# mims-harvard/G-Meta

Hardware: AMD Instinct MI355X
Metric: meta-tasks/sec (inner-loop fwd+bwd) at task_num=32 (higher is better)
Workload: dtype f32

## Files before the change

g-meta_amd/_lib.py:

```python
import ctypes as C
import os

HERE = os.path.dirname(os.path.abspath(__file__))
LIB_PATH = os.environ.get('GMETA_HIP_LIB') or os.path.join(HERE, 'libgmeta_hip.so')

GM_MAX_GCN = 4
(F_SUB_OFF, F_SET_SUB_OFF, F_PARENT, F_GRAPH, F_INDPTR, F_INDICES, F_INDPTR_T, F_INDICES_T, F_CENTRE, F_NORM,
 F_FEAT_ROW, F_NORM_SRC, F_NORM_CENTRE, F_EDGE_W, F_EDGE_W_T, F_HOP, F_NORM_E1, F_EDGE_CENTRE_T, F_OBS_CENTRE, F_OBS_E1) = range(20)
LINK_SYMMETRIC = 2
LINK_MASK_TARGET = 4
NEG_MODES = {'uniform': 0, 'two_hop': 1}
PAIR_MASK_TARGET = 1
PROP_SELF_LOOPS = 1
PROP_OPS = {'hadamard': 0, 'abs_diff': 1}
DIST_UNREACHED = 255


class Seed(C.Structure):
    _fields_ = [('graph', C.c_int32), ('i', C.c_int32), ('j', C.c_int32)]


class Model(C.Structure):
    _fields_ = [('n_gcn', C.c_int32), ('dims', C.c_int32 * (GM_MAX_GCN + 1)), ('n_out', C.c_int32), ('link_pred', C.c_int32)]

# ... 12 lines not shown
    'gm_store_weighted': (i32, [vp]),
    'gm_batch_weighted': (i32, [vp]),
    'gm_store_destroy': (None, [vp]),
    'gm_store_negative_pairs': (i32, [vp, i32, i64, u64, i32, vp, i64, vp, vp, vp]),
    'gm_store_has_edges': (i32, [vp, i32, vp, i64, vp, vp]),
    'gm_store_pair_scores': (i32, [vp, i32, vp, i64, i32, vp, vp]),
    'gm_store_pair_walks': (i32, [vp, i32, vp, i64, i32, vp, vp]),
    'gm_store_rooted_pagerank': (i32, [vp, i32, vp, i64, C.c_float, i32, vp, vp]),
    'gm_store_pair_pagerank': (i32, [vp, i32, vp, i64, i32, C.c_float, i32, vp, vp]),
    'gm_store_pagerank_candidates': (i32, [vp, i32, vp, i64, i32, C.c_float, i32, vp, vp, vp, vp]),
    'gm_store_node_distances': (i32, [vp, i32, vp, i64, i32, vp, vp]),
    'gm_store_pair_distance': (i32, [vp, i32, vp, i64, i32, i32, vp, vp]),
    'gm_store_pair_distance_profile': (i32, [vp, i32, vp, i64, i32, i32, vp, vp]),
    'gm_store_sketch_build': (i32, [vp, i32, i32, i32, i32, u64, vp, vp]),
    'gm_sketch_dims': (i32, [vp, vp, vp, vp, vp, vp]),
    'gm_sketch_registers': (i32, [vp, i32, vp, i64, vp, vp, vp]),
    'gm_sketch_pair_counts': (i32, [vp, vp, i64, vp, vp, vp]),
    'gm_sketch_destroy': (None, [vp]),
    'gm_store_propagate_build': (i32, [vp, i32, i32, i32, vp, vp]),
    'gm_prop_dims': (i32, [vp, vp, vp, vp, vp, vp]),
    'gm_prop_rows': (i32, [vp, i32, vp, i64, vp, vp]),
    'gm_prop_pair_features': (i32, [vp, vp, i64, i32, vp, vp]),
    'gm_prop_destroy': (None, [vp]),
    'gm_store_neighbour_degrees': (i32, [vp, i32, vp, vp]),
    'gm_store_pair_candidates': (i32, [vp, i32, vp, i64, i32, i32, vp, vp, vp, vp]),
    'gm_extract': (C.c_int, [vp, vp, i32, vp, i32, i32, i32, u64, i32, vp, vp]),
    'gm_extract_pair': (C.c_int, [vp, vp, i32, vp, i32, vp, i32, vp, i32, i32, i32, u64, i32, vp, vp, vp]),
    'gm_batch_from_nodes': (C.c_int, [vp, vp, i32, vp, i32, vp, vp, i32, vp, vp]),
    'gm_set_hop_labels': (None, [i32]),
    'gm_get_hop_labels': (i32, []),
    'gm_batch_hop_labels': (i32, [vp]),
    'gm_batch_mask_target': (i32, [vp]),
    'gm_batch_concat': (C.c_int, [vp, i32, vp, vp]),
    'gm_batch_destroy': (None, [vp]),
    'gm_batch_prepare_cone': (C.c_int, [vp, i32, vp]),
    'gm_batch_prepare_cone_pair': (C.c_int, [vp, vp, i32, vp]),
    'gm_batch_cone_dims': (C.c_int, [vp, i32, vp, vp, vp]),
    'gm_batch_cone_read': (C.c_int, [vp, i32, i32, i32, vp, i64]),
    'gm_batch_dims': (C.c_int, [vp, vp, vp, vp, vp, vp]),
    'gm_batch_read': (C.c_int, [vp, i32, vp, i64]),
    'gm_batch_device_ptr': (C.c_int, [vp, i32, vp]),
    'gm_batch_source_rows': (C.c_int, [vp, vp]),
    'gm_batch_e1_source_rows': (C.c_int, [vp, vp]),
    'gm_gather_features': (C.c_int, [vp, vp, vp]),
    'gm_aggregate': (C.c_int, [vp, i32, i32, vp, i32, vp, vp, vp, vp]),
    'gm_aggregate_bytes': (i64, [vp, i32]),
    'gm_model_param_count': (i64, [vp]),
    'gm_gcn_ws_bytes': (i64, [vp, vp]),
    'gm_gcn_forward': (C.c_int, [vp, vp, vp, i64, vp, vp, vp, vp, i64, vp]),
    'gm_gcn_backward': (C.c_int, [vp, vp, vp, i64, vp, vp, vp, vp, i64, vp, i64, vp]),
    'gm_dense_update': (C.c_int, [vp, vp, i32, vp, i64, i32, vp, i32, vp]),
    'gm_dense_gemm': (C.c_int, [vp, vp, i64, i32, vp, i64, i32, i32, vp, i64, vp, vp, vp, i64, i32, vp, vp, vp, vp, vp, i32, vp, vp]),
    'gm_dense_fused_gemm': (C.c_int, [vp, i32, vp, i64, i32, vp, i64, vp, i64, vp, i64, i32, vp, i64, vp, vp, vp, i64, i32, vp, vp, vp, i32, vp, vp]),
    'gm_dense_wgrad_fused': (C.c_int, [vp, i32, vp, i64, i32, vp, i64, vp, i64, i32, vp, vp, vp, i64, vp, i64, i32, vp]),
    'gm_dense_aggregate': (C.c_int, [vp, i32, i32, vp, i64, i32, i32, vp, vp, i32, vp, i64, i32, vp, vp, vp, i32, vp, i64, i32, i32, i32, i32, i32, vp, vp, vp]),
    'gm_dense_agg_info': (C.c_int, [vp, i32, vp]),
    'gm_dense_obs_lists': (C.c_int, [vp, vp, vp]),
    'gm_dense_fuse_counts': (C.c_int, [vp, vp]),
    'gm_dense_agg_table': (C.c_int, [vp, i32, i32, vp, i64, vp]),
    'gm_dense_dz_centre': (C.c_int, [vp, vp, i32, vp, i64, i32, vp, vp]),
    'gm_dense_wgrad_centre': (C.c_int, [vp, vp, i32, vp, i32, vp, i64, vp, i64, vp]),
    'gm_dense_agg_centre_t': (C.c_int, [vp, vp, i32, vp, vp, i32, vp]),
    'gm_dense_wgrad_e1': (C.c_int, [vp, vp, i32, vp, i32, vp, i64, vp, i64, vp]),
    'gm_dense_wgrad': (C.c_int, [vp, vp, i64, i32, vp, i64, i32, vp, vp, i64, vp, i64, vp, i64, i32, vp, vp, i64, C.c_float, vp, vp, vp, vp]),
    'gm_proto_loss_spt': (C.c_int, [vp, vp, i32, vp, i32, vp, vp, vp, vp, vp]),
    'gm_proto_loss_qry': (C.c_int, [vp, vp, i32, vp, vp, i32, vp, vp, vp, vp, vp]),
    'gm_dense_head_loss': (C.c_int, [vp, vp, i32, i32, i32, i32, vp, i64, i64, i64, vp, vp, i32, i32, vp, i32, vp, vp, vp, vp, vp, vp, vp, vp, i32, vp, i64, vp, vp,
                                     vp, vp, i64, C.c_float, vp, i32, vp, vp]),
    'gm_set_ragged_classes': (None, [i32]),
    'gm_get_ragged_classes': (i32, []),
    'gm_set_readout': (None, [i32]),
    'gm_get_readout': (i32, []),
    'gm_meta_ws_bytes': (i64, [vp, vp, vp, vp]),
    'gm_meta_out_floats': (i64, [vp, vp, vp]),
    'gm_meta_step': (C.c_int, [vp, vp, vp, vp, vp, vp, vp, vp, i64, vp, i64, vp]),
    'gm_adapt_ws_bytes': (i64, [vp, vp, vp]),
    'gm_meta_adapt': (C.c_int, [vp, vp, vp, vp, vp, vp, i64, vp, i32, vp, i64, vp]),
    'gm_predict_ws_bytes': (i64, [vp, vp, vp]),
    'gm_proto_predict': (C.c_int, [vp, vp, vp, vp, i64, vp, vp, i32, vp, vp, vp, vp, i64, vp]),
    'gm_meta_finish': (C.c_int, [vp, i64, i32, vp, vp, vp]),
    'gm_meta_finish_adam': (C.c_int, [vp, i64, i32, vp, vp, vp, vp, vp, i32, C.c_float, C.c_float, C.c_float, C.c_float, vp, vp, vp]),
    'gm_set_gemm_mode': (None, [i32]),
    'gm_get_gemm_mode': (i32, []),
    'gm_get_split_pieces': (i32, []),
    'gm_set_split_pieces': (None, [i32]),
    'gm_set_tuning': (C.c_int, [C.c_char_p, i32]),
    'gm_get_tuning': (i32, [C.c_char_p]),
    'gm_tuning_epoch': (i32, []),
    'gm_set_fuse_agg': (None, [i32]),
    'gm_get_fuse_agg': (i32, []),
    'gm_profile_enable': (None, [i32]),
    'gm_profile_aggregate': (C.c_int, [vp, vp, vp]),
    'gm_profile_read': (C.c_int, [i32, vp, vp, vp]),
    'gm_profile_read_launches': (C.c_int, [i32, vp, vp, i32]),
}
PROBE_PROTOTYPES = {
    'gm_debug_stamp': (C.c_int, [vp, vp]),
    'gm_stream_debug': (C.c_int, [i32, vp, i32]),
    'gm_head_loss_debug': (C.c_int, [i32, vp]),
}

LATER_EXPORTS = {'gm_dense_obs_lists'}

_lib = None


def lib():
    global _lib
    if _lib is None:
        if not os.path.exists(LIB_PATH):
            raise RuntimeError('gmeta_amd: %s is missing -- run `python -c "import __graft_entry__ as g; g.build()"` '
                               '(hipcc --offload-arch=gfx950).  There is no CPU fallback.' % LIB_PATH)
        l = C.CDLL(LIB_PATH)
        for name, (res, args) in PROTOTYPES.items():
            if name in LATER_EXPORTS and os.environ.get('GMETA_HIP_LIB') and not hasattr(l, name):
                continue
            fn = getattr(l, name)
            fn.restype, fn.argtypes = res, args
        for name, (res, args) in PROBE_PROTOTYPES.items():
            if hasattr(l, name):
                fn = getattr(l, name)
                fn.restype, fn.argtypes = res, args
        _lib = l
    return _lib


def check(rc, what=''):
    if rc != 0:
        msg = lib().gm_last_error().decode('utf-8', 'replace')
        exc = ValueError if rc == -1 else RuntimeError
        raise exc('%s failed (code %d): %s' % (what or 'libgmeta_hip', rc, msg))


def require_gpu():
    import torch
    if not torch.cuda.is_available():
        raise RuntimeError('gmeta_amd needs an AMD GPU (gfx950); torch.cuda.is_available() is False and there is no CPU fallback')


def stream_ptr():
    import torch
    return C.c_void_p(torch.cuda.current_stream().cuda_stream)


def ptr(t):
    if t is None:
        return C.c_void_p(0)
    if hasattr(t, 'data_ptr'):
        return C.c_void_p(t.data_ptr())
    return C.c_void_p(t.ctypes.data)


READOUT_CENTRE, READOUT_MEAN = 0, 1
READOUTS = {'centre': READOUT_CENTRE, 'mean': READOUT_MEAN}

# ... 56 lines not shown
```

g-meta_amd/csrc/common.hip:

```cpp
#include <stdarg.h>
#include <stdlib.h>
#include <atomic>
#include <chrono>
#include <map>
#include <mutex>
#include <set>
#include <utility>
#include "gm_internal.h"

static thread_local char g_err[512] = "";

void gm_set_error(const char* fmt, ...) {
    va_list ap;
    va_start(ap, fmt);
    vsnprintf(g_err, sizeof(g_err), fmt, ap);
    va_end(ap);
}

extern "C" const char* gm_last_error(void) { return g_err; }
extern "C" int gm_version(void) { return 100; }

static void pool_keep_memory() {
    static thread_local int done_for = -1;
    int dev = 0;
// ... 261 lines not shown
    if (total_ms) *total_ms = tot;
    if (launches) *launches = c.launches;
    if (work) *work = c.work;
    return GM_OK;
}
extern "C" int gm_profile_read_launches(int32_t category, double* ms, int64_t* work, int32_t cap) {
    GM_REQUIRE(category >= 0 && category < GM_PROF_CATS && ms && work && cap >= 0, GM_EINVAL, "profile_read_launches: bad arguments");
    ProfCat& c = g_prof[category];
    int n = 0;
    for (size_t k = 0; k + 1 < c.used + 1 && k < c.used && n < cap; k += 2, ++n) {
        GM_HIP(hipEventSynchronize(c.ev[k + 1]));
        float t = 0;
        GM_HIP(hipEventElapsedTime(&t, c.ev[k], c.ev[k + 1]));
        ms[n] = t; work[n] = k / 2 < c.works.size() ? c.works[k / 2] : 0;
    }
    return n;
}
extern "C" int gm_profile_aggregate(double* total_ms, int64_t* launches, int64_t* algorithmic_bytes) {
    return gm_profile_read(GM_PROF_AGG, total_ms, launches, algorithmic_bytes);
}

#ifdef GM_PROBES
__global__ void k_debug_stamp(unsigned long long* out) { *out = wall_clock64(); }
extern "C" int gm_debug_stamp(void* out, void* stream) {
    GM_REQUIRE(out, GM_EINVAL, "debug_stamp: NULL argument");
    hipLaunchKernelGGL(k_debug_stamp, dim3(1), dim3(1), 0, (hipStream_t)stream, (unsigned long long*)out);
    GM_HIP(hipGetLastError());
    return GM_OK;
}
#endif

static gm_knobs g_knobs;
static std::once_flag g_knobs_once;
const gm_knobs& gm_knob() {
    gm_knobs& k = g_knobs;
    std::call_once(g_knobs_once, [] {
        gm_knobs& k = g_knobs;
        auto env = [](const char* name, int dflt) { const char* e = getenv(name); return e ? atoi(e) : dflt; };
        k.timing = env("GM_TIMING", 0);
        const char* gm = getenv("GM_GEMM_MODE");
        k.gemm_mode = (gm && (!strcmp(gm, "split") || !strcmp(gm, "1"))) ? 1 : (gm && (!strcmp(gm, "f32") || !strcmp(gm, "0"))) ? 0 : -1;
        k.gemm_split_min_tiles = env("GM_GEMM_SPLIT_MIN_TILES", -1);
        k.centre_store = env("GM_CENTRE_STORE", 2);
        k.dead_rows = env("GM_DEAD_ROWS", 4);
        k.fuse_agg = env("GM_FUSE_AGG", 1);
        k.fuse_diff = env("GM_FUSE_DIFF", 2);
        k.extract_pref16 = env("GM_EXTRACT_PREF16", 1);
        k.head_stage = env("GM_HEAD_STAGE", 1);
        k.head_threads = env("GM_HEAD_THREADS", 0);
        k.query_streams = env("GM_QUERY_STREAMS", 0);
        k.agg_mid_list = env("GM_AGG_MID_LIST", 1);
        k.agg_mid_win = env("GM_AGG_MID_WIN", 0);
        k.agg_obs_list = env("GM_AGG_OBS_LIST", 1);
        k.split_pieces = env("GM_SPLIT_PIECES", 3);
        k.split16_min_rows = env("GM_SPLIT16_MIN_ROWS", 65536);
        k.wgrad_split_min_chunks = env("GM_WGRAD_SPLIT_MIN_CHUNKS", -1);
        k.agg_stream = env("GM_AGG_STREAM", 1);
        k.agg_stream_min_rows = env("GM_AGG_STREAM_MIN_ROWS", 100000);
        k.neg_round = env("GM_NEG_ROUND", 0);
        k.pair_lanes = env("GM_PAIR_LANES", 0);
        k.cand_round = env("GM_CAND_ROUND", 0);
        k.cand_bitmap = env("GM_CAND_BITMAP", 0);
        k.walk_chunk = env("GM_WALK_CHUNK", 0);
        k.walk_lanes = env("GM_WALK_LANES", 0);
        k.ppr_chunk = env("GM_PPR_CHUNK", 0);
        k.ppr_cols = env("GM_PPR_COLS", 0);
        k.dist_chunk = env("GM_DIST_CHUNK", 0);
        k.dist_cols = env("GM_DIST_COLS", 0);
        k.dist_plane_kib = env("GM_DIST_PLANE_KIB", 0);
        k.sketch_chunk = env("GM_SKETCH_CHUNK", 0);
        k.sketch_mib = env("GM_SKETCH_MIB", 0);
        k.prop_chunk = env("GM_PROP_CHUNK", 0);
        k.prop_mib = env("GM_PROP_MIB", 0);
    });
    return k;
}

static std::atomic<int> g_tuning_epoch{0};
extern "C" int32_t gm_tuning_epoch(void) { return g_tuning_epoch.load(std::memory_order_relaxed); }
static int gm_knobs::* gm_find_knob(const char* name) {
    (void)gm_knob();
    static const struct { const char* name; int gm_knobs::*field; } tab[] = {
        {"GM_GEMM_SPLIT_MIN_TILES", &gm_knobs::gemm_split_min_tiles}, {"GM_CENTRE_STORE", &gm_knobs::centre_store}, {"GM_DEAD_ROWS", &gm_knobs::dead_rows},
        {"GM_HEAD_STAGE", &gm_knobs::head_stage}, {"GM_HEAD_THREADS", &gm_knobs::head_threads}, {"GM_QUERY_STREAMS", &gm_knobs::query_streams}, {"GM_AGG_MID_LIST", &gm_knobs::agg_mid_list}, {"GM_AGG_MID_WIN", &gm_knobs::agg_mid_win}, {"GM_AGG_OBS_LIST", &gm_knobs::agg_obs_list}, {"GM_AGG_STREAM", &gm_knobs::agg_stream}, {"GM_AGG_STREAM_MIN_ROWS", &gm_knobs::agg_stream_min_rows},
        {"GM_SPLIT16_MIN_ROWS", &gm_knobs::split16_min_rows}, {"GM_WGRAD_SPLIT_MIN_CHUNKS", &gm_knobs::wgrad_split_min_chunks}, {"GM_TIMING", &gm_knobs::timing},
        {"GM_FUSE_DIFF", &gm_knobs::fuse_diff}, {"GM_EXTRACT_PREF16", &gm_knobs::extract_pref16},
        {"neg_round", &gm_knobs::neg_round}, {"GM_NEG_ROUND", &gm_knobs::neg_round},
        {"pair_lanes", &gm_knobs::pair_lanes}, {"GM_PAIR_LANES", &gm_knobs::pair_lanes},
        {"cand_round", &gm_knobs::cand_round}, {"GM_CAND_ROUND", &gm_knobs::cand_round},
        {"cand_bitmap", &gm_knobs::cand_bitmap}, {"GM_CAND_BITMAP", &gm_knobs::cand_bitmap},
        {"walk_chunk", &gm_knobs::walk_chunk}, {"GM_WALK_CHUNK", &gm_knobs::walk_chunk},
        {"walk_lanes", &gm_knobs::walk_lanes}, {"GM_WALK_LANES", &gm_knobs::walk_lanes},
        {"ppr_chunk", &gm_knobs::ppr_chunk}, {"GM_PPR_CHUNK", &gm_knobs::ppr_chunk},
        {"ppr_cols", &gm_knobs::ppr_cols}, {"GM_PPR_COLS", &gm_knobs::ppr_cols},
        {"dist_chunk", &gm_knobs::dist_chunk}, {"GM_DIST_CHUNK", &gm_knobs::dist_chunk},
        {"dist_cols", &gm_knobs::dist_cols}, {"GM_DIST_COLS", &gm_knobs::dist_cols},
        {"dist_plane_kib", &gm_knobs::dist_plane_kib}, {"GM_DIST_PLANE_KIB", &gm_knobs::dist_plane_kib},
        {"sketch_chunk", &gm_knobs::sketch_chunk}, {"GM_SKETCH_CHUNK", &gm_knobs::sketch_chunk},
        {"sketch_mib", &gm_knobs::sketch_mib}, {"GM_SKETCH_MIB", &gm_knobs::sketch_mib},
        {"prop_chunk", &gm_knobs::prop_chunk}, {"GM_PROP_CHUNK", &gm_knobs::prop_chunk},
        {"prop_mib", &gm_knobs::prop_mib}, {"GM_PROP_MIB", &gm_knobs::prop_mib},
    };
    for (const auto& e : tab)
        if (!strcmp(name, e.name)) return e.field;
    return nullptr;
}
extern "C" int gm_set_tuning(const char* name, int32_t value) {
    GM_REQUIRE(name, GM_EINVAL, "set_tuning: NULL name");
    int gm_knobs::* f = gm_find_knob(name);
    GM_REQUIRE(f, GM_EINVAL, "set_tuning: unknown or start-up-only knob %s", name);
    g_knobs.*f = value; g_tuning_epoch.fetch_add(1, std::memory_order_relaxed);
    return GM_OK;
}
extern "C" int32_t gm_get_tuning(const char* name) {
    int gm_knobs::* f = name ? gm_find_knob(name) : nullptr;
    return f ? g_knobs.*f : 0;
}

int gm_heavy_deg() { return 64; }
int gm_heavy_deg_for(int64_t rows, int64_t edges) {
    return edges <= 8 * rows ? 32 : 64;
}

static std::mutex g_dev_mu;

int gm_num_cus() {
    static std::map<int, int> cus;
    int dev = 0;
    if (hipGetDevice(&dev) != hipSuccess) { (void)hipGetLastError(); return 256; }
    std::lock_guard<std::mutex> lk(g_dev_mu);
    auto it = cus.find(dev);
    if (it != cus.end()) return it->second;
    int n = 0;
    if (hipDeviceGetAttribute(&n, hipDeviceAttributeMultiprocessorCount, dev) != hipSuccess || n <= 0) { (void)hipGetLastError(); n = 256; }
    cus[dev] = n;
    return n;
}
// ... 12 lines not shown
```

g-meta_amd/csrc/dense_exports.hip:

```cpp
#include <algorithm>
#include "gm_internal.h"

static int set_row_amax(const gm_batch* b, const float* x, int64_t ldx, int cols, unsigned* slots, hipStream_t st) {
    int rc = GM_OK;
    for (int t0 = 0; rc == GM_OK && t0 < b->sets; t0 += 8) {
        const int segs = std::min(8, b->sets - t0);
        int64_t xo[8], xn[8];
        for (int i = 0; i < segs; ++i) {
            const int64_t r0 = b->h_set_row_off[t0 + i], nr = b->h_set_row_off[t0 + i + 1] - r0;
            xo[i] = r0 * ldx; xn[i] = nr > 0 ? (nr - 1) * ldx + cols : 0;
        }
        rc = gm_amax_segs(x, xo, xn, segs, slots + (int64_t)t0 * GM_BOUND_PAD, GM_BOUND_PAD, st);
    }
    return rc;
}

extern "C" int gm_dense_update(const gm_batch_t* b, const float* x, int32_t K, const float* W, int64_t w_stride, int32_t N, float* out, int32_t mode,
                               void* stream) {
    GM_REQUIRE(b && x && W && out && K >= 1 && N >= 1, GM_EINVAL, "dense_update: bad arguments");
    hipStream_t st = (hipStream_t)stream;
    gm_gemm_args g{};
    g.A = x; g.lda = K; g.B = W; g.b_stride = w_stride; g.C = out; g.ldc = N; g.K = K; g.N = N;
    g.tiles = b->d_tiles; g.n_tiles = b->n_tiles; g.rows = b->rows;
    uint16_t* planes = nullptr; unsigned* slots = nullptr;
// ... 13 lines not shown
            g.np = 2; g.a_bound = gm_no_bound(); g.a_bound.amax = slots; g.b_bound = wb;
        }
        if (rc == GM_OK) rc = gm_split_weights(W, w_stride, 0, K, N, 0, sets, planes, st, mode == 2 ? 2 : 3, wb);
        if (rc != GM_OK) { gm_dev_free(planes, st); if (slots) gm_dev_free(slots, st); return rc; }
        g.Bsplit = planes; g.bsplit_stride = w_stride ? (int64_t)3 * K * N : 0;
    }
    const int rc = gm_launch_gemm_nn(g, st);
    if (planes) gm_dev_free(planes, st);
    if (slots) gm_dev_free(slots, st);
    gm_batch_mark_use(b, st);
    return rc;
}

extern "C" int gm_dense_gemm(const gm_batch_t* b, const float* x, int64_t ldx, int32_t K, const float* W, int64_t w_stride, int32_t trans_w, int32_t N,
                             float* out, int64_t ldc, const float* s, const float* s_keep, const float* bias, int64_t bias_stride, int32_t relu,
                             uint8_t* relu_bits, const float* mask_h, const uint8_t* mask_b, float* zero_out, uint32_t* amax_out, int32_t mode,
                             int32_t* launched, void* stream) {
    GM_REQUIRE(b && x && W && out && K >= 1 && N >= 1 && ldx >= K && ldc >= N && mode >= -1 && mode <= 2 && !(mask_h && mask_b), GM_EINVAL,
               "dense_gemm: bad arguments");
    GM_REQUIRE(!amax_out || mode == 2, GM_EINVAL, "dense_gemm: amax_out is an output of the two-piece kernels (mode 2)");
    hipStream_t st = (hipStream_t)stream;
    const int sets = b->sets;
    gm_gemm_args g{};
    g.A = x; g.lda = ldx; g.B = W; g.b_stride = w_stride; g.transB = trans_w ? 1 : 0; g.C = out; g.ldc = ldc; g.K = K; g.N = N;
    g.row_scale = s; g.row_scale_keep = s_keep; g.n_keep = b->rows; g.bias = bias; g.bias_stride = bias_stride; g.relu = relu ? 1 : 0;
    g.relu_bits = relu_bits; g.mask_h = mask_h; g.mask_b = mask_b; g.zero_out = zero_out;
    g.tiles = b->d_tiles; g.n_tiles = b->n_tiles; g.rows = b->rows; g.launched = launched;
    uint16_t* planes = nullptr; unsigned* slots = nullptr;
    int rc = GM_OK;
    if (mode == 1 || mode == 2 || (mode < 0 && gm_gemm_split_ok(b->n_tiles, K, N))) {
        GM_REQUIRE(!mask_h && !mask_b, GM_EINVAL, "dense_gemm: the split kernels take no relu' mask");
        GM_REQUIRE((N == 256 || N == 128) && K % 16 == 0 && K >= 32, GM_EINVAL, "dense_gemm: the split kernels need N = 128 or 256 and K a multiple of 16 (>= 32)");
        const int wsets = w_stride ? sets : 1;
        rc = gm_alloc(&planes, (size_t)wsets * 3 * K * N, st);
        gm_bound wb = gm_no_bound();
        if (rc == GM_OK && mode == 2) {
            rc = gm_alloc(&slots, (size_t)(sets + wsets) * GM_BOUND_PAD, st);
            if (rc == GM_OK && hipMemsetAsync(slots, 0, sizeof(unsigned) * (sets + wsets) * GM_BOUND_PAD, st) != hipSuccess) { gm_set_error("dense_gemm: memset failed"); rc = GM_EHIP; }
            if (rc == GM_OK) rc = set_row_amax(b, x, ldx, K, slots, st);
            if (rc == GM_OK) rc = gm_amax(W, w_stride, 0, (int64_t)K * N, wsets, slots + (int64_t)sets * GM_BOUND_PAD, GM_BOUND_PAD, st);
            wb.amax = slots + (int64_t)sets * GM_BOUND_PAD; wb.stride = w_stride ? GM_BOUND_PAD : 0;
            g.np = 2; g.a_bound = gm_no_bound(); g.a_bound.amax = slots; g.a_bound.stride = GM_BOUND_PAD; g.b_bound = wb; g.amax_out = amax_out;
        }
        if (rc == GM_OK) rc = gm_split_weights(W, w_stride, 0, K, N, trans_w ? 1 : 0, wsets, planes, st, mode == 2 ? 2 : 3, wb);
        g.Bsplit = planes; g.bsplit_stride = w_stride ? (int64_t)3 * K * N : 0;
    }
    if (rc == GM_OK) rc = gm_launch_gemm_nn(g, st);
    if (planes) gm_dev_free(planes, st);
    if (slots) gm_dev_free(slots, st);
    gm_batch_mark_use(b, st);
    return rc;
}

extern "C" int gm_dense_fused_gemm(const gm_batch_t* b, int32_t table, const float* x, int64_t ldx, int32_t K, const float* zside, int64_t ldz,
                                   const float* zfull, int64_t ldzf, const float* W, int64_t w_stride, int32_t N, float* out, int64_t ldc, const float* s,
                                   const float* s_keep, const float* bias, int64_t bias_stride, int32_t relu, uint8_t* relu_bits, float* zero_out,
                                   uint32_t* amax_out, int32_t mode, int32_t* launched, void* stream) {
    GM_REQUIRE(b && W && out && zside && K >= 1 && N >= 1 && ldz >= K && ldc >= N && (mode == 1 || mode == 2) && (table == 0 || table == 1), GM_EINVAL,
               "dense_fused_gemm: bad arguments");
    GM_REQUIRE(b->d_fuse2 && b->d_fuse2_feat, GM_EINVAL, "dense_fused_gemm: the batch carries no source tables");
    GM_REQUIRE(table == 1 || (x && ldx >= K), GM_EINVAL, "dense_fused_gemm: table 0 needs x and ldx >= K");
    GM_REQUIRE(table == 0 || (b->feat && (K == b->feat_dim || K == b->feat_ld)), GM_EINVAL, "dense_fused_gemm: table 1 needs K == feat_dim (%d)", b->feat_dim);
    GM_REQUIRE(!amax_out || mode == 2, GM_EINVAL, "dense_fused_gemm: amax_out is an output of the two-piece kernels (mode 2)");
    GM_REQUIRE(mode != 2 || (zfull && ldzf >= K), GM_EINVAL, "dense_fused_gemm: mode 2 takes its A bounds over a fully aggregated Z (zfull)");
    GM_REQUIRE((N == 256 || N == 128) && K % 16 == 0 && K >= 32, GM_EINVAL, "dense_fused_gemm: the split kernels need N = 128 or 256 and K a multiple of 16 (>= 32)");
    hipStream_t st = (hipStream_t)stream;
    const int sets = b->sets, wsets = w_stride ? sets : 1;
    gm_gemm_args g{};
    g.B = W; g.b_stride = w_stride; g.C = out; g.ldc = ldc; g.K = K; g.N = N;
    g.row_scale = s; g.row_scale_keep = s_keep; g.n_keep = b->rows; g.bias = bias; g.bias_stride = bias_stride; g.relu = relu ? 1 : 0;
    g.relu_bits = relu_bits; g.zero_out = zero_out;
    g.tiles = b->d_tiles; g.n_tiles = b->n_tiles; g.rows = b->rows; g.launched = launched;
    g.zside = zside; g.ldz = ldz;
    if (table == 1) { g.A = b->feat; g.lda = b->feat_ld; g.fuse2 = b->d_fuse2_feat; }
    else { g.A = x; g.lda = ldx; g.fuse2 = b->d_fuse2; }
    uint16_t* planes = nullptr; unsigned* slots = nullptr;
    int rc = gm_alloc(&planes, (size_t)wsets * 3 * K * N, st);
    gm_bound wb = gm_no_bound();
    if (rc == GM_OK && mode == 2) {
        rc = gm_alloc(&slots, (size_t)(sets + wsets) * GM_BOUND_PAD, st);
        if (rc == GM_OK && hipMemsetAsync(slots, 0, sizeof(unsigned) * (sets + wsets) * GM_BOUND_PAD, st) != hipSuccess) { gm_set_error("dense_fused_gemm: memset failed"); rc = GM_EHIP; }
        if (rc == GM_OK) rc = set_row_amax(b, zfull, ldzf, K, slots, st);
        if (rc == GM_OK) rc = gm_amax(W, w_stride, 0, (int64_t)K * N, wsets, slots + (int64_t)sets * GM_BOUND_PAD, GM_BOUND_PAD, st);
        wb.amax = slots + (int64_t)sets * GM_BOUND_PAD; wb.stride = w_stride ? GM_BOUND_PAD : 0;
        g.np = 2; g.a_bound = gm_no_bound(); g.a_bound.amax = slots; g.a_bound.stride = GM_BOUND_PAD; g.b_bound = wb; g.amax_out = amax_out;
    }
    if (rc == GM_OK) rc = gm_split_weights(W, w_stride, 0, K, N, 0, wsets, planes, st, mode == 2 ? 2 : 3, wb);
    g.Bsplit = planes; g.bsplit_stride = w_stride ? (int64_t)3 * K * N : 0;
    if (rc == GM_OK) rc = gm_launch_gemm_nn(g, st);
    if (planes) gm_dev_free(planes, st);
    if (slots) gm_dev_free(slots, st);
    gm_batch_mark_use(b, st);
    return rc;
}

extern "C" int gm_dense_dz_centre(const gm_batch_t* b, const float* dQ, int32_t K, const float* W, int64_t w_stride, int32_t N, float* T, void* stream) {
    GM_REQUIRE(b && dQ && W && T && b->d_dq_tab, GM_EINVAL, "dense_dz_centre: bad arguments");
    GM_REQUIRE((N == 256 || N == 128) && K % 16 == 0 && K >= 64, GM_EINVAL, "dense_dz_centre: the fused split kernel needs N = 128 or 256 and K a multiple of 16 (>= 64)");
    hipStream_t st = (hipStream_t)stream;
    const int wsets = w_stride ? b->sets : 1;
    uint16_t* planes = nullptr;
    GM_TRY(gm_alloc(&planes, (size_t)wsets * 3 * K * N, st));
    gm_gemm_args g{};
    g.A = dQ; g.lda = K; g.B = W; g.b_stride = w_stride; g.transB = 1; g.C = T; g.ldc = N; g.K = K; g.N = N;
    g.row_scale = b->d_norm; g.tiles = b->d_tiles; g.n_tiles = b->n_tiles; g.rows = b->rows;
    g.fuse2 = b->d_dq_tab; g.zside = dQ; g.ldz = K;
    int rc = gm_split_weights(W, w_stride, 0, K, N, 1, wsets, planes, st, 3, gm_no_bound());
    g.Bsplit = planes; g.bsplit_stride = w_stride ? (int64_t)3 * K * N : 0; g.np = 3;
    if (rc == GM_OK) rc = gm_launch_gemm_nn(g, st);
    gm_dev_free(planes, st);
    gm_batch_mark_use(b, st);
    return rc;
}
static int dense_wgrad_keep(const gm_batch_t* b, const float* keep, const float* x, int32_t Kx, const float* dQ, int32_t N, float* dW, int64_t dw_stride, float* db,
                            int64_t db_stride, void* stream) {
    GM_REQUIRE(b && x && dQ && dW && db && keep, GM_EINVAL, "dense_wgrad_centre / _e1: bad arguments");
    const int64_t KN = (int64_t)Kx * N;
    GM_REQUIRE(b->sets == 1 || (dw_stride >= KN && db_stride >= N), GM_EINVAL, "dense_wgrad_centre / _e1: per-set outputs overlap");
    hipStream_t st = (hipStream_t)stream;
    gm_wgrad_args w{};
    w.A = x; w.lda = Kx; w.K = Kx; w.G = dQ; w.ldg = N; w.N = N; w.a_scale = b->d_norm; w.g_keep = keep;
    w.chunks = b->d_chunks; w.n_chunks = b->n_chunks; w.set_chunk_off = b->d_set_chunk_off; w.sets = b->sets; w.rows = b->rows;
    w.dW = dW; w.dw_stride = dw_stride; w.db = db; w.db_stride = db_stride; w.pick = GM_WGRAD_PICK_SPLIT;
    int rc = gm_alloc(&w.partial, (size_t)std::max(1, b->n_chunks) * (size_t)(KN + N), st);
    if (rc == GM_OK) rc = gm_launch_wgrad(w, st);
    if (w.partial) gm_dev_free(w.partial, st);
    gm_batch_mark_use(b, st);
    return rc;
}
extern "C" int gm_dense_wgrad_centre(const gm_batch_t* b, const float* x, int32_t Kx, const float* dQ, int32_t N, float* dW, int64_t dw_stride, float* db,
                                     int64_t db_stride, void* stream) {
    return dense_wgrad_keep(b, b ? b->d_norm_c : nullptr, x, Kx, dQ, N, dW, dw_stride, db, db_stride, stream);
}

extern "C" int gm_dense_agg_centre_t(const gm_batch_t* b, float* T, int32_t width, const uint8_t* mask_b, float* out, int32_t keep, void* stream) {
    GM_REQUIRE(b && T && out && width >= 4 && width % 4 == 0, GM_EINVAL, "dense_agg_centre_t: bad arguments");
    GM_REQUIRE(!keep || (b->d_ect && b->d_norm_e1), GM_EINVAL, "dense_agg_centre_t: the batch carries no centre-edge tables");
    hipStream_t st = (hipStream_t)stream;
    gm_agg_args a{};
    a.indptr = b->d_indptr_t; a.indices = b->d_indices_t;
    a.heavy = b->d_heavy[1]; a.n_heavy = b->n_heavy[1]; a.heavy_deg = b->heavy_deg;
    a.sched = b->d_sched[1]; a.sched_len = b->sched_len[1]; a.sched_win = b->sched_win;
    GM_TRY(gm_agg_hub(a, b, 1, st));
    if (b->weighted) a.e_w = b->d_ew[1];
    a.rows = b->rows; a.x = T; a.ldx = width; a.s_out = b->d_norm; a.mask_b = mask_b; a.out = out; a.width = width;
    if (keep) {
// ... 139 lines not shown
        if (list_sched) {
            GM_REQUIRE(hubs == 2 && !transposed && b->d_sched_mid && n_list == b->n_mid && list_win == b->mid_win, GM_EINVAL,
                       "dense_aggregate: the list schedule goes with the batch's own list (%d rows, windows of %d) and its hub tables", b->n_mid, b->mid_win);
            a.sched = b->d_sched_mid; a.sched_len = b->sched_len_mid; a.sched_win = b->mid_win;
        } else { a.sched = nullptr; a.sched_len = 0; }
    } else if (list_sched >= 2 && list_sched <= 4) {
        const gm_batch::obs_list& ol = b->obs[list_sched - 2];
        GM_REQUIRE(ol.rows && (list_sched == 4) == (transposed != 0), GM_EINVAL, "dense_aggregate: the batch holds no list %d of this orientation", list_sched - 2);
        GM_REQUIRE(ol.cap >= 1 || ol.sched, GM_EINVAL, "dense_aggregate: list %d is empty and the orientation has no hub rows: nothing to launch", list_sched - 2);
        GM_REQUIRE(b->n_heavy[o] == 0 || (hubs == 2 && ol.sched), GM_EINVAL, "dense_aggregate: list %d has no schedule for the orientation's hub rows", list_sched - 2);
        a.rowlist = ol.rows; a.n_list = ol.cap; a.n_list_dev = ol.len; a.list_win = ol.win;
        a.sched = ol.sched; a.sched_len = ol.sched ? ol.sched_len : 0; a.sched_win = ol.win;
    } else GM_REQUIRE(!list_sched, GM_EINVAL, "dense_aggregate: a list schedule without a row list");
    if (stream_ok && a.e_w && a.e_w == b->d_enorm[o]) GM_TRY(gm_agg_stream_args(a, b, o, gather, st));
    const int rc = gm_launch_aggregate(a, st);
    gm_batch_mark_use(b, st);
    return rc;
}

extern "C" int gm_dense_agg_info(const gm_batch_t* b, int32_t transposed, int64_t* info) {
    GM_REQUIRE(b && info, GM_EINVAL, "dense_agg_info: bad arguments");
    const int o = transposed ? 1 : 0;
    const int64_t v[16] = {b->heavy_deg, b->n_heavy[o], b->sched_win, b->hub_part[o], b->hub_parts[o], b->d_sched[o] ? 1 : 0, b->d_mid ? b->n_mid : 0, b->mid_win,
                           b->d_sched_mid ? 1 : 0, b->d_sseg[o] ? b->stream_nseg[o] : 0, b->stream_nwg[o], b->stream_hubwg[o], b->weighted ? 1 : 0, b->feat_dim, b->feat_ld, 0};
    std::copy(v, v + 16, info);
    return GM_OK;
}
extern "C" int gm_dense_obs_lists(const gm_batch_t* b, int64_t* info, void* stream) {
    GM_REQUIRE(b && info, GM_EINVAL, "dense_obs_lists: bad arguments");
    for (int k = 0; k < 3; ++k) {
        const gm_batch::obs_list& ol = b->obs[k];
        if (ol.n < 0) {
            int32_t h = 0;
            if (ol.rows && ol.len) { GM_HIP(hipMemcpyAsync(&h, ol.len, 4, hipMemcpyDeviceToHost, (hipStream_t)stream)); GM_HIP(hipStreamSynchronize((hipStream_t)stream)); }
            ol.n = h;
        }
        info[4 * k] = ol.n; info[4 * k + 1] = ol.cap; info[4 * k + 2] = ol.win; info[4 * k + 3] = ol.take + (ol.sched ? 4 : 0);
    }
    for (int k = 0; k < 2; ++k) {
        int64_t w[3] = {-1, -1, -1};
        if (b->d_obs[k] && b->rows > 0) GM_TRY(gm_batch_fwd_counts(b, k, (hipStream_t)stream, w));
        info[12 + k] = w[0];
    }
    info[14] = gm_batch_e1_rows(b, (hipStream_t)stream); info[15] = 0;
    gm_batch_mark_use(b, (hipStream_t)stream);
    return GM_OK;
}
extern "C" int gm_dense_fuse_counts(const gm_batch_t* b, int64_t* counts) {
    GM_REQUIRE(b && counts, GM_EINVAL, "dense_fuse_counts: bad arguments");
    counts[0] = b->unfused_rows; counts[1] = b->unfused_edges;
    return GM_OK;
}
extern "C" int gm_dense_agg_table(const gm_batch_t* b, int32_t which, int32_t transposed, void* dst, int64_t n, void* stream) {
    GM_REQUIRE(b && dst && n >= 0 && which >= 0 && which <= 12, GM_EINVAL, "dense_agg_table: bad arguments");
    if (which >= 10) {
        const gm_batch::obs_list& ol = b->obs[which - 10];
        GM_REQUIRE(ol.rows && n <= ol.cap, GM_EINVAL, "dense_agg_table: table %d holds %lld entries", which, (long long)(ol.rows ? ol.cap : 0));
        if (n) GM_HIP(hipMemcpyAsync(dst, ol.rows, 4 * (size_t)n, hipMemcpyDeviceToDevice, (hipStream_t)stream));
        gm_batch_mark_use(b, (hipStream_t)stream);
        return GM_OK;
    }
    const int o = transposed ? 1 : 0;
    const void* src = which == 0 ? (const void*)b->d_enorm[o] : which == 1 ? (const void*)b->d_efeat : which == 2 ? (const void*)b->d_mid : which == 3 ? (const void*)b->d_heavy[o]
                    : which == 4 ? (const void*)b->d_fuse2 : which == 5 ? (const void*)b->d_fuse2_feat : which == 6 ? (const void*)b->d_dq_tab
                    : which == 7 ? (const void*)b->d_fwd_tab[0] : which == 8 ? (const void*)b->d_fwd_tab[1] : (const void*)b->d_fwd_tab_feat;
    const int64_t have = which <= 1 ? b->edges : which == 2 ? b->n_mid : which == 3 ? b->n_heavy[o] : b->rows;
    GM_REQUIRE(src && n <= have, GM_EINVAL, "dense_agg_table: table %d holds %lld entries", which, (long long)(src ? have : 0));
    if (n) GM_HIP(hipMemcpyAsync(dst, src, (which >= 4 ? 16 : 4) * (size_t)n, hipMemcpyDeviceToDevice, (hipStream_t)stream));
    gm_batch_mark_use(b, (hipStream_t)stream);
    return GM_OK;
}
```

g-meta_amd/csrc/extract.hip:

```cpp
#include <algorithm>
#include <initializer_list>
#include <stdlib.h>
#include <string.h>
#include <memory>
#include <mutex>
#include <type_traits>
#include "gm_internal.h"
#include "gm_devutil.h"

#define EX_BLOCK 512
#define EX_WAVES (EX_BLOCK / GM_WAVE)

__device__ __forceinline__ int lane_id() { return __builtin_amdgcn_mbcnt_hi(~0u, __builtin_amdgcn_mbcnt_lo(~0u, 0u)); }
__device__ __forceinline__ int wave_sum(int v) {
#pragma unroll
    for (int o = 32; o > 0; o >>= 1) v += __shfl_xor(v, o, 64);
    return v;
}
template <bool G> __device__ __forceinline__ bool bit_test(const uint32_t* bm, int v) { return (wld<G>(&bm[v >> 5]) >> (v & 31)) & 1u; }
__device__ __forceinline__ void bit_set(uint32_t* bm, int v) { atomicOr(&bm[v >> 5], 1u << (v & 31)); }
template <bool G, typename PT> __device__ __forceinline__ int pref_ld(const PT* p) {
    if constexpr (sizeof(PT) == 4) return (int)wld<G>(reinterpret_cast<const uint32_t*>(p)); else return (int)*p;
}
template <bool G, typename PT> __device__ __forceinline__ int bit_rank(const uint32_t* bm, const PT* pref, int v) {
// ... 650 lines not shown
    if (blockIdx.x == 0 && threadIdx.x == 0) *n_rows = 0;
    for (int64_t k = blockIdx.x * (int64_t)blockDim.x + threadIdx.x; k < n; k += (int64_t)gridDim.x * blockDim.x) {
        if (k < rows) norm_e1[k] = __uint_as_float(__float_as_uint(norm[k]) | 0x80000000u);
        if (k < edges) { const int v = indices_t[k]; ect[k] = (__float_as_uint(norm_c[v]) >> 31) ? (int32_t)(rows + (k & (GM_ZERO_ROWS - 1))) : v; }
    }
}
__global__ void k_e1_rows(const int32_t* e_row, int n_e1, float* norm_e1, int32_t* n_rows) {
    const int k = blockIdx.x * blockDim.x + threadIdx.x;
    if (k >= n_e1) return;
    const unsigned old = atomicAnd(reinterpret_cast<unsigned*>(norm_e1) + e_row[k], 0x7fffffffu);
    if (old >> 31) atomicAdd(n_rows, 1);
}
int64_t gm_batch_e1_rows(const gm_batch* b, hipStream_t s) {
    if (b->n_e1_rows >= 0) return b->n_e1_rows;
    const int64_t fallback = std::min<int64_t>(b->n_e1, b->rows);
    if (!b->d_n_e1_rows) return fallback;
    int32_t h = 0;
    if (hipMemcpyAsync(&h, b->d_n_e1_rows, 4, hipMemcpyDeviceToHost, s) != hipSuccess || hipStreamSynchronize(s) != hipSuccess) { (void)hipGetLastError(); return fallback; }
    return b->n_e1_rows = h;
}
__global__ void k_e1_kept_edges(const int32_t* indptr_t, const float* norm_e1, int64_t rows, unsigned long long* out) {
    unsigned long long c = 0;
    for (int64_t r = blockIdx.x * (int64_t)blockDim.x + threadIdx.x; r < rows; r += (int64_t)gridDim.x * blockDim.x)
        if (!(__float_as_uint(norm_e1[r]) >> 31)) c += (unsigned long long)(indptr_t[r + 1] - indptr_t[r]);
#pragma unroll
    for (int off = 32; off >= 1; off >>= 1) c += __shfl_down(c, off, 64);
    if ((threadIdx.x & 63) == 0 && c) atomicAdd(out, c);
}
int64_t gm_batch_e1_edges(const gm_batch* b, hipStream_t s) {
    if (b->n_e1_edges >= 0) return b->n_e1_edges;
    const int64_t fallback = b->edges;
    if (!b->d_norm_e1 || !b->d_indptr_t || b->rows <= 0) return fallback;
    unsigned long long* cnt = nullptr; unsigned long long h = 0;
    if (gm_alloc(&cnt, 1, s) != GM_OK) return fallback;
    bool ok = hipMemsetAsync(cnt, 0, 8, s) == hipSuccess;
    if (ok) {
        hipLaunchKernelGGL(k_e1_kept_edges, dim3((int)std::min<int64_t>(512, (b->rows + 255) / 256)), dim3(256), 0, s, b->d_indptr_t, b->d_norm_e1, (int64_t)b->rows, cnt);
        ok = hipMemcpyAsync(&h, cnt, 8, hipMemcpyDeviceToHost, s) == hipSuccess && hipStreamSynchronize(s) == hipSuccess;
    }
    if (!ok) (void)hipGetLastError();
    gm_dev_free(cnt, s);
    return ok ? (b->n_e1_edges = (int64_t)h) : fallback;
}
__global__ void k_fwd_tables(const int4* f2, const int4* f2_feat, const float* norm_c, const float* norm_e1, int64_t rows, int4* tab_c, int4* tab_e1, int4* tab_e1_feat,
                             float* obs_c, float* obs_e1) {
    auto pick = [](const bool on, const int4 t) { return make_int4(on ? t.x : GM_FUSE_ZERO, on ? t.y : GM_FUSE_ZERO, on ? t.z : 0, on ? t.w : 0); };
    for (int64_t r = blockIdx.x * (int64_t)blockDim.x + threadIdx.x; r < rows; r += (int64_t)gridDim.x * blockDim.x) {
        const bool c = !(__float_as_uint(norm_c[r]) >> 31), e = !(__float_as_uint(norm_e1[r]) >> 31);
        const int4 t = f2[r], tf = f2_feat[r];
        tab_c[r] = pick(c, t); tab_e1[r] = pick(e, t); tab_e1_feat[r] = pick(e, tf);
        obs_c[r] = c ? 1.f : -1.f; obs_e1[r] = e ? 1.f : -1.f;
    }
}
__global__ void k_fwd_count(const int32_t* indptr, const int32_t* indices, const float* obs, int64_t rows, int maxdeg, uint32_t* bits, unsigned long long* out) {
    unsigned long long nr = 0, ne = 0;
    for (int64_t r = blockIdx.x * (int64_t)blockDim.x + threadIdx.x; r < rows; r += (int64_t)gridDim.x * blockDim.x) {
        const int p = indptr[r], d = indptr[r + 1] - p;
        if (d <= maxdeg || (__float_as_uint(obs[r]) >> 31)) continue;
        ++nr; ne += (unsigned long long)d;
        for (int e = p; e < p + d; ++e) { const int u = indices[e]; atomicOr(&bits[u >> 5], 1u << (u & 31)); }
    }
#pragma unroll
    for (int off = 32; off >= 1; off >>= 1) { nr += __shfl_down(nr, off, 64); ne += __shfl_down(ne, off, 64); }
    if ((threadIdx.x & 63) == 0 && nr) { atomicAdd(out, nr); atomicAdd(out + 1, ne); }
}
int gm_batch_fwd_counts(const gm_batch* b, int which, hipStream_t s, int64_t* out) {
    GM_REQUIRE(b && out && (which == 0 || which == 1), GM_EINVAL, "batch_fwd_counts: bad arguments");
    int64_t* have = b->fwd_cnt[which];
    if (have[0] < 0) {
        GM_REQUIRE(b->d_obs[which] && b->rows > 0, GM_EINVAL, "batch_fwd_counts: the batch carries no forward-only tables");
        const int64_t words = (b->rows + 31) / 32;
        uint32_t* bits = nullptr; unsigned long long* cnt = nullptr; unsigned long long h[3] = {0, 0, 0};
        int rc = gm_alloc(&bits, (size_t)words, s);
        if (rc == GM_OK) rc = gm_alloc(&cnt, 3, s);
        bool ok = rc == GM_OK && hipMemsetAsync(bits, 0, 4 * (size_t)words, s) == hipSuccess && hipMemsetAsync(cnt, 0, 24, s) == hipSuccess;
        if (ok) {
            hipLaunchKernelGGL(k_fwd_count, dim3((int)std::min<int64_t>(2048, (b->rows + 255) / 256)), dim3(256), 0, s, b->d_indptr, b->d_indices, b->d_obs[which], (int64_t)b->rows,
                               GM_FUSE_MAXDEG, bits, cnt);
            hipLaunchKernelGGL(k_count_bits, dim3((int)std::min<int64_t>(512, (words + 255) / 256)), dim3(256), 0, s, bits, words, cnt + 2);
            ok = hipMemcpyAsync(h, cnt, 24, hipMemcpyDeviceToHost, s) == hipSuccess && hipStreamSynchronize(s) == hipSuccess;
        }
        if (bits) gm_dev_free(bits, s);
        if (cnt) gm_dev_free(cnt, s);
        if (!ok) { (void)hipGetLastError(); gm_set_error("batch_fwd_counts: counting failed"); return GM_EHIP; }
        have[1] = (int64_t)h[1]; have[2] = (int64_t)h[2]; have[0] = (int64_t)h[0];
    }
    out[0] = have[0]; out[1] = have[1]; out[2] = have[2];
    return GM_OK;
}
__global__ void k_copy_add(int32_t* dst, const int32_t* src, int64_t n, int32_t add) {
    for (int64_t k = blockIdx.x * (int64_t)blockDim.x + threadIdx.x; k < n; k += (int64_t)gridDim.x * blockDim.x) dst[k] = src[k] + add;
}
__global__ void k_gather_rows(const float* feat, int64_t ld, const int32_t* feat_row, float* out, int64_t rows, int F) {
    const int64_t total = rows * F;
    for (int64_t k = blockIdx.x * (int64_t)blockDim.x + threadIdx.x; k < total; k += (int64_t)gridDim.x * blockDim.x) {
        const int64_t r = k / F; const int f = (int)(k - r * F);
        out[k] = feat[(int64_t)feat_row[r] * ld + f];
    }
}

#define GM_HOP_LDS_ROWS 2048
#define GM_HOP_BLOCK 256
template <bool LDS>
__device__ __forceinline__ void hop_bfs(int8_t* dist, int64_t stride, int n, int root, int r0, const int32_t* indptr, const int32_t* indices, int D) {
    auto get = [&](int v) -> int { return LDS ? (int)dist[v] : (int)((volatile int8_t*)dist)[(int64_t)v * stride]; };
    auto put = [&](int v, int d) { if (LDS) dist[v] = (int8_t)d; else ((volatile int8_t*)dist)[(int64_t)v * stride] = (int8_t)d; };
// ... 234 lines not shown
        const int nb = (int)((b->rows + MID_BLOCK - 1) / MID_BLOCK);
        int32_t* d_bcnt = nullptr;
        GM_TRY(gm_alloc(&d_bcnt, (size_t)nb, s));
        hipLaunchKernelGGL(k_mid_count, dim3(nb), dim3(MID_BLOCK), 0, s, indptr, flag, (int64_t)b->rows, lo, hi, d_bcnt);
        hipLaunchKernelGGL(k_mid_scan, dim3(1), dim3(1024), 0, s, d_bcnt, nb, total, (int)n_cap);
        hipLaunchKernelGGL(k_mid_scatter, dim3(nb), dim3(MID_BLOCK), 0, s, indptr, flag, (int64_t)b->rows, lo, hi, d_bcnt, list, (int)n_cap);
        GM_HIP(hipGetLastError());
        gm_dev_free(d_bcnt, s);
        return (int)GM_OK;
    };
    auto list_window = [](int64_t n) { int win = 64; while (win > 2 && n / win < 16384) win >>= 1; return gm_knob().agg_mid_win > 0 ? gm_knob().agg_mid_win : win; };
    auto list_schedule = [&](int o, int64_t n, int win, int32_t** d_sched, int32_t* len, const uint8_t* keep = nullptr) {
        std::vector<int32_t> pos(heavy_h[o].size());
        for (size_t k = 0; k < pos.size(); ++k) pos[k] = (int32_t)std::min<int64_t>(std::max<int64_t>(n, 1) - 1, (int64_t)heavy_h[o][k] * n / b->rows);
        return gm_agg_schedule_flat(b, n, win, pos.data(), (int)pos.size(), tab_h[o], d_sched, len, s, &sg, keep);
    };
    if (b->d_fuse2 && gm_knob().agg_mid_list) {
        const int64_t n_mid = b->unfused_rows - (int64_t)b->n_heavy[0];
        if (n_mid > 0 && n_mid < b->rows && h_cnt[0] <= cap) {
            GM_TRY(gm_balloc(b, &b->d_mid, (size_t)n_mid, s));
            GM_TRY(compact(b->d_indptr, nullptr, GM_FUSE_MAXDEG + 1, b->heavy_deg, b->d_mid, n_mid, nullptr));
            b->n_mid = (int32_t)n_mid;
            b->mid_win = list_window(n_mid);
            if (b->n_heavy[0] > 0 && b->d_sched[0]) GM_TRY(list_schedule(0, n_mid, b->mid_win, &b->d_sched_mid, &b->sched_len_mid));
        }
    }
    tm.lap("mid-list");
    std::vector<int32_t> eoff(b->n_c + 1, 0);
    for (int k = 0; k < b->n_c; ++k) eoff[k + 1] = eoff[k] + h_cdeg[k];
    b->n_e1 = eoff[b->n_c];
    int32_t* d_eoff = nullptr;
    GM_TRY(gm_alloc(&d_eoff, eoff.size(), s));
    GM_TRY(sg.upload(d_eoff, eoff));
    GM_TRY(gm_balloc(b, &b->d_e1_row, b->n_e1, s)); GM_TRY(gm_balloc(b, &b->d_e1_par, b->n_e1, s)); GM_TRY(gm_balloc(b, &b->d_e1_norm, b->n_e1, s));
    if (b->weighted) GM_TRY(gm_balloc(b, &b->d_e1_coef, b->n_e1, s));
    auto centre_edges = [&](auto kern, auto... w) {
        hipLaunchKernelGGL(kern, dim3(b->n_c), dim3(64), 0, s, b->d_crow, d_eoff, b->n_c, b->d_indptr, b->d_indices, b->d_norm, b->d_e1_row, b->d_e1_par, b->d_e1_norm, w...);
    };
    if (b->weighted) centre_edges(k_centre_edges<CentreW>, CentreW{b->d_ew[0], b->d_e1_coef}); else centre_edges(k_centre_edges<>);
    GM_HIP(hipGetLastError());
    if (b->rows > 0 && b->d_norm_c) {
        GM_TRY(gm_balloc(b, &b->d_ect, (size_t)b->edges, s)); GM_TRY(gm_balloc(b, &b->d_norm_e1, (size_t)b->rows, s)); GM_TRY(gm_balloc(b, &b->d_n_e1_rows, 1, s));
        hipLaunchKernelGGL(k_e1_tables, dim3(grid_for(std::max<int64_t>(b->edges, b->rows), 4096)), dim3(256), 0, s, b->d_indices_t, (int64_t)b->edges, b->d_norm, b->d_norm_c, (int64_t)b->rows, b->d_ect, b->d_norm_e1, b->d_n_e1_rows);
        if (b->n_e1 > 0) hipLaunchKernelGGL(k_e1_rows, dim3((b->n_e1 + 255) / 256), dim3(256), 0, s, b->d_e1_row, b->n_e1, b->d_norm_e1, b->d_n_e1_rows);
        GM_HIP(hipGetLastError());
        if (b->d_fuse2 && b->d_fuse2_feat) {
            int4 *tc = nullptr, *te = nullptr, *tf = nullptr;
            GM_TRY(gm_balloc(b, &tc, (size_t)b->rows, s)); GM_TRY(gm_balloc(b, &te, (size_t)b->rows, s)); GM_TRY(gm_balloc(b, &tf, (size_t)b->rows, s));
            GM_TRY(gm_balloc(b, &b->d_obs[0], (size_t)b->rows, s)); GM_TRY(gm_balloc(b, &b->d_obs[1], (size_t)b->rows, s));
            hipLaunchKernelGGL(k_fwd_tables, dim3(grid_for(b->rows, 4096)), dim3(256), 0, s, (const int4*)b->d_fuse2, (const int4*)b->d_fuse2_feat, b->d_norm_c, b->d_norm_e1, (int64_t)b->rows,
                               tc, te, tf, b->d_obs[0], b->d_obs[1]);
            GM_HIP(hipGetLastError());
            b->d_fwd_tab[0] = tc; b->d_fwd_tab[1] = te; b->d_fwd_tab_feat = tf;
        }
        if (gm_knob().agg_mid_list && h_cnt[0] <= cap && h_cnt[1] <= cap) {
            const int64_t walked_fwd = b->d_mid ? b->n_mid : b->rows;
            auto finish = [&](int k, int o, int64_t n, int64_t walked, const uint8_t* hub_keep) {
                gm_batch::obs_list& ol = b->obs[k];
                ol.cap = (int32_t)n; ol.win = list_window(n);
                if (2 * n > walked || (b->n_heavy[o] > 0 && !b->d_sched[o])) return (int)GM_OK;
                if (b->n_heavy[o] > 0) GM_TRY(list_schedule(o, n, ol.win, &ol.sched, &ol.sched_len, hub_keep));
                ol.take = 1;
                return (int)GM_OK;
            };
            if (b->d_obs[0]) {
                std::vector<int32_t> lst, hubs_c;
                for (int k = 0; k < b->n_c; ++k) {
                    const int32_t row = b->h_sub_off[k / nc] + h_centre[k];
                    if (h_cdeg[k] > b->heavy_deg) hubs_c.push_back(row); else if (h_cdeg[k] > GM_FUSE_MAXDEG) lst.push_back(row);
                }
                std::sort(lst.begin(), lst.end()); lst.erase(std::unique(lst.begin(), lst.end()), lst.end());
                std::sort(hubs_c.begin(), hubs_c.end());
                const bool hub_centre = !hubs_c.empty();
                std::vector<uint8_t> hub_keep(heavy_h[0].size());
                for (size_t k = 0; k < hub_keep.size(); ++k) hub_keep[k] = std::binary_search(hubs_c.begin(), hubs_c.end(), heavy_h[0][k]) ? 1 : 0;
                gm_batch::obs_list& ol = b->obs[0];
                ol.n = (int64_t)lst.size();
                if (lst.empty() && !hub_centre) ol.take = 2;
                else {
                    GM_TRY(gm_balloc(b, &ol.rows, lst.size(), s));
                    if (!lst.empty()) GM_TRY(sg.upload(ol.rows, lst));
                    GM_TRY(finish(0, 0, (int64_t)lst.size(), walked_fwd, hub_keep.data()));
                }
            }
            GM_TRY(gm_balloc(b, &b->obs[1].len, 2, s)); b->obs[2].len = b->obs[1].len + 1;
            GM_HIP(hipMemsetAsync(b->obs[1].len, 0, 8, s));
            if (b->d_obs[1]) {
                const int64_t n_range = b->unfused_rows - (int64_t)b->n_heavy[0], bound = std::min<int64_t>(b->n_e1, n_range);
                if (b->n_e1 == 0 || b->unfused_rows == 0) { b->obs[1].take = 2; b->obs[1].n = 0; }
                else {
                    GM_TRY(gm_balloc(b, &b->obs[1].rows, (size_t)bound, s));
                    if (bound > 0) GM_TRY(compact(b->d_indptr, b->d_obs[1], GM_FUSE_MAXDEG + 1, b->heavy_deg, b->obs[1].rows, bound, b->obs[1].len));
                    GM_TRY(finish(1, 0, bound, walked_fwd, nullptr));
                }
            }
            {
                const int64_t bound = std::min<int64_t>(b->n_e1, b->rows);
                if (b->n_e1 == 0) { b->obs[2].take = 2; b->obs[2].n = 0; }
                else {
                    GM_TRY(gm_balloc(b, &b->obs[2].rows, (size_t)bound, s));
                    GM_TRY(compact(b->d_indptr_t, b->d_norm_e1, 0, INT32_MAX, b->obs[2].rows, bound, b->obs[2].len));
                    GM_TRY(finish(2, 1, bound, b->rows, nullptr));
                }
            }
        }
    }
// ... 348 lines not shown
```

g-meta_amd/csrc/gemm.hip:

```cpp
#include <algorithm>
#include <stdlib.h>
#include "gm_internal.h"
#include <atomic>
#include <mutex>
#include "gemm_split.h"

typedef float f32x16 __attribute__((ext_vector_type(16)));

#define BK 16
#ifndef GM_GEMM_MODE_DEFAULT
#define GM_GEMM_MODE_DEFAULT 1
#endif
#define AS_LD 20

struct GemmK {
    const float* A; int64_t lda; const float* B; int64_t b_stride; int transB; float* C; int64_t ldc; int K, N;
    const float* row_scale; const float* bias; int64_t bias_stride; const float* mask_h; int relu;
    const uint8_t* mask_b; uint8_t* relu_bits;
    const int32_t* tiles; int n_tiles; int n_col_tiles; int a_vec, b_vec, c_vec; int nt_store;
    float* zero_out;
};

struct GemmTile { int set, row0, nrows, n0; };
__device__ __forceinline__ GemmTile gemm_tile(const GemmK& g, int BN) {
// ... 379 lines not shown
    hipLaunchKernelGGL(kernel, grid, block, lds, s, k);
    return GM_OK;
}
template <bool GATHER, int NP>
static int launch_gemm_split(const gm_gemm_args& a, const SplitGemmK& k, int grid, bool half_tiles, hipStream_t s) {
    const dim3 blk(1024);
    if (a.N == 128) return launch_kernel(k_gemm_split_p<GATHER, 1, 2, NP>, dim3(grid), blk, 0, s, k, a.launched, GM_GEMM_ID_SPLIT(GATHER, 1, 2, NP));
    if constexpr (!GATHER)
        if (half_tiles) return launch_kernel(k_gemm_split_p<false, 1, 4, NP>, dim3(2 * a.n_tiles), blk, 0, s, k, a.launched, GM_GEMM_ID_SPLIT(false, 1, 4, NP));
    return launch_kernel(k_gemm_split_p<GATHER, 2, 4, NP>, dim3(grid), blk, 0, s, k, a.launched, GM_GEMM_ID_SPLIT(GATHER, 2, 4, NP));
}
template <int WC>
static int launch_gemm_exact(const gm_gemm_args& a, const GemmK& g, bool vec, hipStream_t s) {
    const dim3 grid(g.n_tiles * g.n_col_tiles), blk(128 * WC);
    const int id = GM_GEMM_ID_NN(WC, vec, a.transB ? 1 : 0);
    if (vec && a.transB) return launch_kernel(k_gemm_nn<WC, true, true>, grid, blk, 0, s, g, a.launched, id);
    if (vec) return launch_kernel(k_gemm_nn<WC, true, false>, grid, blk, 0, s, g, a.launched, id);
    if (a.transB) return launch_kernel(k_gemm_nn<WC, false, true>, grid, blk, 0, s, g, a.launched, id);
    return launch_kernel(k_gemm_nn<WC, false, false>, grid, blk, 0, s, g, a.launched, id);
}

static int launch_gemm_nn(const gm_gemm_args& a, hipStream_t s);
int gm_launch_gemm_nn(const gm_gemm_args& a, hipStream_t s) {
    if (a.n_tiles <= 0) return GM_OK;
    const int cat = a.Bsplit ? (a.np == 2 ? GM_PROF_GEMM_SPLIT16 : GM_PROF_GEMM_SPLIT) : GM_PROF_GEMM;
    gm_prof_begin(cat, s, 2 * a.rows * a.K * a.N);
    if (a.Bsplit) gm_prof_note(GM_PROF_GEMM_SPLIT_BYTES, 4 * a.rows * (int64_t)a.K + 4 * (a.row_scale_keep ? a.n_keep : a.rows) * (int64_t)a.N);
    gm_prof_note(GM_PROF_GEMM_BYTES, 4 * a.rows * (int64_t)a.K + 4 * ((a.Bsplit && a.row_scale_keep) ? a.n_keep : a.rows) * (int64_t)a.N);
    const int rc = launch_gemm_nn(a, s);
    gm_prof_end(cat, s);
    return rc;
}
static int launch_gemm_nn(const gm_gemm_args& a, hipStream_t s) {
    if (a.Bsplit) {
        const bool ok = split_dims_ok(a.K, a.N) && !a.mask_h && !a.mask_b && (a.lda % 4 == 0) && (((uintptr_t)a.A & 15) == 0) &&
                        (a.ldc % 4 == 0) && (((uintptr_t)a.C & 15) == 0) && (!a.bias || a.bias_stride % 4 == 0);
        GM_REQUIRE(ok, GM_EINVAL, "gemm: launch not eligible for the split-bf16 kernel (N=%d K=%d)", a.N, a.K);
        GM_REQUIRE(!a.zero_out || a.ldc == a.N, GM_EINVAL, "gemm: the split kernels zero-fill a [rows, N] buffer only (ldc=%lld N=%d)", (long long)a.ldc, a.N);
        SplitGemmK k{};
        k.A = a.A; k.lda = a.lda; k.Bt = a.Bsplit; k.bt_stride = a.bsplit_stride; k.C = a.C; k.ldc = a.ldc; k.K = a.K; k.N = a.N;
        k.row_scale = a.row_scale_keep ? a.row_scale_keep : a.row_scale; k.keep_signed = a.row_scale_keep ? 1 : 0; k.bias = a.bias; k.bias_stride = a.bias_stride; k.relu = a.relu; k.relu_bits = a.relu_bits;
        k.tiles = a.tiles; k.n_tiles = a.n_tiles; k.n_col_tiles = 1; k.nt_store = 1; k.zero_out = a.zero_out;
        const bool f16 = a.np == 2;
        GM_REQUIRE(!f16 || (a.a_bound.amax && a.b_bound.amax), GM_EINVAL, "gemm: the two-piece split kernel needs bounds for both operands");
        k.a_bound = f16 ? a.a_bound : gm_no_bound(); k.b_bound = f16 ? a.b_bound : gm_no_bound(); k.amax_out = a.amax_out;
        const int cus = gm_num_cus();
        const int grid_cap = a.n_tiles > 2 * cus && a.n_tiles <= 6 * cus && cus >= 128 ? cus - 2 * GM_NXCD : cus;
        if (a.fuse2) {
            GM_REQUIRE(a.K / 16 >= PF_DA && a.zside && (a.ldz % 4 == 0) && (((uintptr_t)a.zside & 15) == 0), GM_EINVAL, "gemm: fused aggregate needs K >= %d and an aligned side buffer", 16 * PF_DA);
            GM_REQUIRE(a.K <= 4096, GM_EINVAL, "gemm: fused aggregate supports K <= 4096");
            k.f2 = reinterpret_cast<const int4*>(a.fuse2); k.zside = a.zside; k.ldz = a.ldz; k.zrow = gm_zero_row(s);
            GM_REQUIRE(k.zrow, GM_EHIP, "gemm: zero row allocation failed");
            const int mult_f = a.n_tiles >= 16 * grid_cap ? 2 : 3;
            const int grid = std::min(a.n_tiles, mult_f * grid_cap);
            GM_TRY(f16 ? (launch_gemm_split<true, 2>(a, k, grid, false, s)) : (launch_gemm_split<true, 3>(a, k, grid, false, s)));
        } else {
            const int grid = std::min(a.n_tiles, grid_cap);
            const bool half_tiles = 2 * a.n_tiles <= grid_cap;
            GM_TRY(f16 ? (launch_gemm_split<false, 2>(a, k, grid, half_tiles, s)) : (launch_gemm_split<false, 3>(a, k, grid, half_tiles, s)));
        }
        GM_HIP(hipGetLastError());
        return GM_OK;
    }
    GemmK g{a.A, a.lda, a.B, a.b_stride, a.transB, a.C, a.ldc, a.K, a.N, a.row_scale, a.bias, a.bias_stride, a.mask_h, a.relu,
            a.mask_b, a.relu_bits, a.tiles, a.n_tiles, 0, 0, 0, 0, 0, nullptr};
    g.a_vec = (a.K % 4 == 0) && (a.lda % 4 == 0) && (((uintptr_t)a.A & 15) == 0);
    g.b_vec = (((uintptr_t)a.B & 15) == 0) && (a.b_stride % 4 == 0) && ((a.transB ? a.K : a.N) % 4 == 0);
    g.c_vec = (a.N % 4 == 0) && (a.ldc % 4 == 0) && (((uintptr_t)a.C & 15) == 0) && (!a.mask_h || (((uintptr_t)a.mask_h & 15) == 0));
    const bool vec = g.a_vec && g.b_vec && a.K >= 4 && a.N >= 4;
    GM_REQUIRE(!(a.mask_b || a.relu_bits) || g.c_vec, GM_EINVAL, "gemm: packed relu masks need 16-byte aligned C with N %% 4 == 0");
    int bn = a.N > 128 ? 256 : a.N > 64 ? 128 : 64;
    while (bn > 64 && (int64_t)a.n_tiles * ((a.N + bn - 1) / bn) < 512) bn >>= 1;
    if (bn == 256 && a.n_tiles < 1536) bn = 128;
    g.n_col_tiles = (a.N + bn - 1) / bn;
    const bool bias_al = !a.bias || ((((uintptr_t)a.bias & 15) == 0) && (a.bias_stride % 4 == 0));
    g.nt_store = 1;
    const bool dma = vec && !a.transB && !a.mask_b && g.c_vec && bias_al && a.K % BK == 0 && a.K >= 2 * BK && a.N % bn == 0;
    if (a.zero_out) {
        if (dma && a.N == a.ldc) g.zero_out = a.zero_out;
        else GM_HIP(hipMemsetAsync(a.zero_out, 0, sizeof(float) * (size_t)a.rows * a.ldc, s));
    }
    if (dma) {
        const dim3 grid(g.n_tiles * g.n_col_tiles);
        if (bn == 256) GM_TRY(launch_kernel(k_gemm_glds<2, 4, 2>, grid, dim3(512), 0, s, g, a.launched, GM_GEMM_ID_GLDS4));
        else if (bn == 128) GM_TRY(launch_kernel(k_gemm_glds<2, 2, 2>, grid, dim3(256), 0, s, g, a.launched, GM_GEMM_ID_GLDS2));
        else if ((int64_t)g.n_tiles * g.n_col_tiles <= 4 * gm_num_cus()) GM_TRY(launch_kernel(k_gemm_glds<4, 2, 1>, grid, dim3(512), 0, s, g, a.launched, GM_GEMM_ID_GLDS_SMALL));
        else GM_TRY(launch_kernel(k_gemm_glds<2, 1, 2>, grid, dim3(128), 0, s, g, a.launched, GM_GEMM_ID_GLDS1));
    } else if (bn == 256) GM_TRY(launch_gemm_exact<4>(a, g, vec, s));
    else if (bn == 128) GM_TRY(launch_gemm_exact<2>(a, g, vec, s));
    else GM_TRY(launch_gemm_exact<1>(a, g, vec, s));
    GM_HIP(hipGetLastError());
    return GM_OK;
}

#define WG_THREADS 1024
#define WG_WAVES 16
#define WG_MAXT 4

struct WgradK {
    const float* A; int64_t lda; int K; const int32_t* a_row;
    const float* G; int64_t ldg; int N; const float* Gb; int64_t ldgb;
    const float* a_scale; const int32_t* chunks; int n_chunks; float* partial; int RK; int TK, TN; int vec;
    gm_bound a_bound, g_bound;
    const int4* f2; const float* gx; int64_t ldgx; const float* zrow;
};

#define WG_PF 2
// ... 700 lines not shown
```

g-meta_amd/csrc/gemm_split.h:

```cpp
#pragma once
#include <hip/hip_runtime.h>
#include <stdint.h>
#include "gm_bound.h"

typedef __bf16 gm_bf16x8 __attribute__((ext_vector_type(8)));
typedef _Float16 gm_f16x8 __attribute__((ext_vector_type(8)));
typedef float gm_f32x16 __attribute__((ext_vector_type(16)));

#define GS_BM 128
#define GS_BARRIER() do { asm volatile("s_waitcnt lgkmcnt(0)" ::: "memory"); __builtin_amdgcn_s_barrier(); } while (0)

struct GsTile { int set, row0, nrows; };
__device__ __forceinline__ GsTile gs_tile(const int32_t* tiles, int lt) {
    const uint64_t p = (uint64_t)(uintptr_t)(tiles + (int64_t)lt * 3);
    const unsigned lo = __builtin_amdgcn_readfirstlane((unsigned)p), hi = __builtin_amdgcn_readfirstlane((unsigned)(p >> 32));
    const uint64_t sp = ((uint64_t)hi << 32) | lo;
    int a, b, c;
    asm volatile("s_load_dword %0, %3, 0x0\n\ts_load_dword %1, %3, 0x4\n\ts_load_dword %2, %3, 0x8\n\ts_waitcnt lgkmcnt(0)"
                 : "=&s"(a), "=&s"(b), "=&s"(c) : "s"(sp) : "memory");
    return GsTile{a, b, c};
}

__device__ __forceinline__ unsigned gs_sload(const void* q) {
    const uint64_t p = (uint64_t)(uintptr_t)q;
    const unsigned lo = __builtin_amdgcn_readfirstlane((unsigned)p), hi = __builtin_amdgcn_readfirstlane((unsigned)(p >> 32));
    const uint64_t sp = ((uint64_t)hi << 32) | lo;
    unsigned a;
    asm volatile("s_load_dword %0, %1, 0x0\n\ts_waitcnt lgkmcnt(0)" : "=&s"(a) : "s"(sp) : "memory");
    return a;
}

struct SplitGemmK {
    const float* A; int64_t lda;
    const uint16_t* Bt; int64_t bt_stride;
    float* C; int64_t ldc; int K, N;
    const float* row_scale; const float* bias; int64_t bias_stride; const float* mask_h; int relu;
    const uint8_t* mask_b; uint8_t* relu_bits;
    const int32_t* tiles; int n_tiles; int n_col_tiles; int nt_store;
    unsigned long long* dbg;
    int dephase;
    float* zero_out;
    const int4* f2; const float* zside; int64_t ldz; const float* zrow;
    gm_bound a_bound, b_bound; unsigned* amax_out;
    int keep_signed;
};
#define GM_SPLIT_FUSE_SELF 0x40000000
#define GM_SPLIT_FUSE_ZERO 0x20000000

__device__ __forceinline__ void gs_split4(const float4 v, uint2& h, uint2& m, uint2& l) {
    const float x[4] = {v.x, v.y, v.z, v.w};
    uint32_t xh[4], xm[4], xl[4];
#pragma unroll
    for (int i = 0; i < 4; ++i) {
        const uint32_t b = __float_as_uint(x[i]);
        xh[i] = b & 0xffff0000u;
        const float r1 = x[i] - __uint_as_float(xh[i]);
        const uint32_t b1 = __float_as_uint(r1);
        xm[i] = b1 & 0xffff0000u;
        const float r2 = r1 - __uint_as_float(xm[i]);
        xl[i] = __float_as_uint(r2);
    }
    h.x = __builtin_amdgcn_perm(xh[1], xh[0], 0x07060302u); h.y = __builtin_amdgcn_perm(xh[3], xh[2], 0x07060302u);
    m.x = __builtin_amdgcn_perm(xm[1], xm[0], 0x07060302u); m.y = __builtin_amdgcn_perm(xm[3], xm[2], 0x07060302u);
    l.x = __builtin_amdgcn_perm(xl[1], xl[0], 0x07060302u); l.y = __builtin_amdgcn_perm(xl[3], xl[2], 0x07060302u);
}

__device__ __forceinline__ float gs_scale_of(float bound) {
    const unsigned e = (__float_as_uint(bound) >> 23) & 0xffu;
    if (e == 0u || e == 0xffu) return 1.f;
    int se = 15 - ((int)e - 126);
    se = se < -40 ? -40 : (se > 40 ? 40 : se);
    return __uint_as_float((unsigned)(se + 127) << 23);
}
__device__ __forceinline__ float gs_bound_scale(const gm_bound& b, int set) {
    if (!b.amax) return 1.f;
    const float gain = b.gain ? __uint_as_float(gs_sload(b.gain)) : 1.f;
    return gs_scale_of(__uint_as_float(gs_sload(b.amax + (int64_t)set * b.stride)) * gain * b.hgain);
}
__device__ __forceinline__ float gs_bound_scale_v(const gm_bound& b, int set) {
    if (!b.amax) return 1.f;
    const float gain = b.gain ? b.gain[0] : 1.f;
    return gs_scale_of(__uint_as_float(b.amax[(int64_t)set * b.stride]) * gain * b.hgain);
}
__device__ __forceinline__ void gs_note_max(unsigned* slot, unsigned bits) {
    if (bits == 0u) return;
    if (__hip_atomic_load(slot, __ATOMIC_RELAXED, __HIP_MEMORY_SCOPE_AGENT) < bits) atomicMax(slot, bits);
}
__device__ __forceinline__ void gs_split4_f16(const float4 v, const float s, uint2& h, uint2& m) {
    const float x[4] = {v.x * s, v.y * s, v.z * s, v.w * s};
    _Float16 xh[4], xm[4];
#pragma unroll
    for (int i = 0; i < 4; ++i) { xh[i] = (_Float16)x[i]; xm[i] = (_Float16)(x[i] - (float)xh[i]); }
// ... 37 lines not shown
        O[0 * plane + at] = (uint16_t)(bh >> 16);
        O[1 * plane + at] = (uint16_t)(bm >> 16);
        O[2 * plane + at] = (uint16_t)(__float_as_uint(r2) >> 16);
    }
}


__global__ __launch_bounds__(256) void k_amax(const float* x, int64_t stride, int64_t off, int64_t n, unsigned* out, int64_t out_stride) {
    const float* p = x + (int64_t)blockIdx.y * stride + off;
    float m = 0.f;
    for (int64_t i = blockIdx.x * (int64_t)blockDim.x + threadIdx.x; i < n; i += (int64_t)gridDim.x * blockDim.x) m = fmaxf(m, fabsf(p[i]));
#pragma unroll
    for (int o = 32; o >= 1; o >>= 1) m = fmaxf(m, __shfl_xor(m, o));
    if ((threadIdx.x & 63) == 0) gs_note_max(out + (int64_t)blockIdx.y * out_stride, __float_as_uint(m));
}

struct AmaxSegs { int64_t off[8]; int64_t n[8]; };
__global__ __launch_bounds__(256) void k_amax_segs(const float* x, AmaxSegs sg, unsigned* out, int64_t out_stride) {
    const float* p = x + sg.off[blockIdx.y]; const int64_t n = sg.n[blockIdx.y];
    float m = 0.f;
    for (int64_t i = blockIdx.x * (int64_t)blockDim.x + threadIdx.x; i < n; i += (int64_t)gridDim.x * blockDim.x) m = fmaxf(m, fabsf(p[i]));
#pragma unroll
    for (int o = 32; o >= 1; o >>= 1) m = fmaxf(m, __shfl_xor(m, o));
    if ((threadIdx.x & 63) == 0) gs_note_max(out + (int64_t)blockIdx.y * out_stride, __float_as_uint(m));
}

template <int CTRL> __device__ __forceinline__ float gs_dpp(float x) {
    return __int_as_float(__builtin_amdgcn_mov_dpp(__float_as_int(x), CTRL, 0xf, 0xf, true));
}
__device__ __forceinline__ void gs_quad_transpose(float& a0, float& a1, float& a2, float& a3, const bool odd1, const bool odd2) {
    const float p1 = gs_dpp<0xB1>(a1), q0 = gs_dpp<0xB1>(a0), p3 = gs_dpp<0xB1>(a3), q2 = gs_dpp<0xB1>(a2);
    const float b0 = odd1 ? p1 : a0, b1 = odd1 ? a1 : q0, b2 = odd1 ? p3 : a2, b3 = odd1 ? a3 : q2;
    const float r2 = gs_dpp<0x4E>(b2), s0 = gs_dpp<0x4E>(b0), r3 = gs_dpp<0x4E>(b3), s1 = gs_dpp<0x4E>(b1);
    a0 = odd2 ? r2 : b0; a2 = odd2 ? b2 : s0;
    a1 = odd2 ? r3 : b1; a3 = odd2 ? b3 : s1;
}

#ifndef PF_DA
#define PF_DA 4
#endif
template <bool GATHER, int MI, int WC = 4, int NP = 3>
__global__ __launch_bounds__(1024) void k_gemm_split_p(SplitGemmK g) {
    constexpr int BK = 16, BN = 64 * WC, BM = 32 * MI * (8 / WC), SPLIT = GS_BM / BM;
    static_assert((WC == 4 || WC == 2) && (BM == 128 || BM == 64), "wave grid");
    constexpr int A_OCT = BM * 16, B_OCT = BN * 16, A_PLANE = 2 * A_OCT, B_PLANE = 2 * B_OCT;
    constexpr int A_ST = NP * A_PLANE, B_ST = NP * B_PLANE, NB = 3;
    static_assert(NP == 2 || NP == 3, "pieces per operand");
    constexpr int OFF_B = 2 * A_ST;
    constexpr int E_WAVE = 0;
    constexpr int OFF_E = OFF_B + NB * B_ST, OFF_SC = OFF_E + 8 * E_WAVE, OFF_BIAS = OFF_SC + 2 * GS_BM * 4;
    constexpr int A_PER = (BM * BK / 4) / 256;
    constexpr int B_PPW = (NP * 2 * (BN / 64)) / 4;
    constexpr int OFF_MAX = OFF_BIAS + 2 * BN * 4;
    __shared__ __attribute__((aligned(16))) char smem[OFF_MAX + 16];
    const int tid = threadIdx.x, lane = tid & 63, wave = __builtin_amdgcn_readfirstlane(tid >> 6);
    const int nchunks = g.K / BK;
    const int G = gridDim.x, b = blockIdx.x;
    const int nb = g.n_tiles * SPLIT, q8 = nb / 8, r8 = nb % 8;
    auto logical = [&](int t) -> int { const int x = t % 8, i = t / 8; return (x < r8 ? x * (q8 + 1) : r8 * (q8 + 1) + (x - r8) * q8) + i; };
    const int ntb = b < nb ? (nb - b + G - 1) / G : 0;
    auto tile_of = [&](int w) -> GsTile {
        const int lt = logical(w);
        if constexpr (SPLIT == 1) return gs_tile(g.tiles, lt);
        else { GsTile t = gs_tile(g.tiles, lt >> 1); const int h = (lt & 1) * 64; t.row0 += h; t.nrows = max(0, min(64, t.nrows - h)); return t; }
    };
    auto a_scale_of = [&](int set) -> float {
        if constexpr (NP == 3) return 1.f;
        else return gs_bound_scale(g.a_bound, set);
    };
    auto b_scale_of = [&](int set) -> float {
        if constexpr (NP == 3) return 1.f;
        else return gs_bound_scale(g.b_bound, set);
    };
    const int total = ntb * nchunks;
    const unsigned lds_base = (unsigned)(uintptr_t)((__attribute__((address_space(3))) char*)smem);
    float* scales = reinterpret_cast<float*>(smem + OFF_SC);
    float* biasl = reinterpret_cast<float*>(smem + OFF_BIAS);
    if (total == 0) return;
    if (NP == 2 && tid < 2) reinterpret_cast<unsigned*>(smem + OFF_MAX)[tid] = 0u;
    if (wave >= 12) {
        __builtin_amdgcn_s_setprio(2);
        const int fw = wave - 12;
        unsigned boff[B_PPW]; int bdst[B_PPW];
#pragma unroll
        for (int p = 0; p < B_PPW; ++p) {
            const int piece = fw * B_PPW + p, cb = piece % (BN / 64), po = piece / (BN / 64), oct = po % 2, plane = po / 2;
            boff[p] = (unsigned)(((int64_t)plane * g.N * g.K + ((int64_t)oct * g.N + cb * 64 + lane) * 8) * 2);
            bdst[p] = OFF_B + plane * B_PLANE + oct * B_OCT + cb * 1024;
        }
        const int64_t b_chunk_bytes = (int64_t)BK * g.N * 2;
        int ib_c = 0, ib_ti = 0;
        uint64_t ib_base = (uint64_t)(uintptr_t)(g.Bt + (int64_t)tile_of(b).set * g.bt_stride);
        int ib_st = 0;
        auto issue_b = [&](int gc) {
            if (ib_c == nchunks) { ib_c = 0; ++ib_ti; ib_base = (uint64_t)(uintptr_t)(g.Bt + (int64_t)tile_of(b + ib_ti * G).set * g.bt_stride); }
            const uint64_t base = ib_base + (uint64_t)(ib_c * b_chunk_bytes);
            ++ib_c;
            const unsigned blo = __builtin_amdgcn_readfirstlane((unsigned)base), bhi = __builtin_amdgcn_readfirstlane((unsigned)(base >> 32));
            const uint64_t sbase = ((uint64_t)bhi << 32) | blo;
#pragma unroll
            for (int p = 0; p < B_PPW; ++p) {
                const unsigned dst = __builtin_amdgcn_readfirstlane(lds_base + (unsigned)(ib_st * B_ST + bdst[p]));
                unsigned keep;
                asm volatile("s_mov_b32 %0, m0\n\ts_mov_b32 m0, %3\n\ts_nop 0\n\tglobal_load_lds_dwordx4 %1, %2\n\ts_mov_b32 m0, %0"
                             : "=&s"(keep) : "v"(boff[p]), "s"(sbase), "s"(dst) : "memory");
            }
            ib_st = ib_st + 1 == NB ? 0 : ib_st + 1;
            (void)gc;
        };
        issue_b(0);
        if (total > 1) { issue_b(1); asm volatile("s_waitcnt vmcnt(%0)" :: "n"(B_PPW) : "memory"); }
        else asm volatile("s_waitcnt vmcnt(0)" ::: "memory");
        GS_BARRIER();
        for (int gc = 0; gc < total; ++gc) {
            if (gc + 2 < total) { issue_b(gc + 2); asm volatile("s_waitcnt vmcnt(%0)" :: "n"(B_PPW) : "memory"); }
            else asm volatile("s_waitcnt vmcnt(0)" ::: "memory");
            GS_BARRIER();
        }
    } else if (wave >= 8) {
        __builtin_amdgcn_s_setprio(3);
        const int ft = tid - 512;
        int rr[A_PER];
#pragma unroll
        for (int p = 0; p < A_PER; ++p) rr[p] = (ft + p * 256) >> 2;
        const int c4 = (ft & 3) * 4;
        int adst[A_PER];
#pragma unroll
        for (int p = 0; p < A_PER; ++p) adst[p] = (c4 >> 3) * A_OCT + rr[p] * 16 + (c4 & 7) * 2;
        typedef float f4v __attribute__((ext_vector_type(4)));
        typedef int i4v __attribute__((ext_vector_type(4)));
        constexpr int NJ = GATHER ? 2 : 1;
        f4v ra[PF_DA][A_PER][NJ];
        const bool fast_consts = nchunks >= PF_DA;
        int la_c = 0, la_ti = 0;
        const float* la_src[A_PER][NJ];
        float w_next[A_PER][2], w_cur[A_PER][2];
        i4v fq[A_PER];
#pragma unroll
        for (int p = 0; p < A_PER; ++p) { w_next[p][0] = w_cur[p][0] = 1.f; w_next[p][1] = w_cur[p][1] = 0.f; fq[p] = i4v{0, 0, 0, 0}; }
        float rc_sc = 1.f, rc_b = 0.f;
        float as_next = 1.f, as_cur = 1.f, inv_next = 1.f, inv_cur = 1.f;
        auto fq_prefetch = [&](int ti) {
            if (ti >= ntb) return;
            const GsTile t = tile_of(b + ti * G);
#pragma unroll
            for (int p = 0; p < A_PER; ++p) {
                const int4* q = g.f2 + t.row0 + min(rr[p], t.nrows - 1);
                asm volatile("global_load_dwordx4 %0, %1, off" : "=v"(fq[p]) : "v"(q) : "memory");
            }
        };
        auto la_tile = [&](int ti, bool consts) {
            const GsTile t = tile_of(b + ti * G);
            if constexpr (NP == 2) { as_next = a_scale_of(t.set); inv_next = (1.f / as_next) * (1.f / b_scale_of(t.set)); }
            if constexpr (GATHER) {
                if constexpr (A_PER == 2) asm volatile("" : "+v"(fq[0]), "+v"(fq[A_PER - 1]) :: "memory");
                else asm volatile("" : "+v"(fq[0]) :: "memory");
#pragma unroll
                for (int p = 0; p < A_PER; ++p) {
#pragma unroll
                    for (int j = 0; j < 2; ++j) {
                        const int u = j ? fq[p].y : fq[p].x;
                        const float* base = (u & GM_SPLIT_FUSE_ZERO) ? g.zrow : (u & GM_SPLIT_FUSE_SELF) ? g.zside + (int64_t)(u & ~GM_SPLIT_FUSE_SELF) * g.ldz : g.A + (int64_t)u * g.lda;
                        la_src[p][j] = base + c4;
                        w_next[p][j] = __int_as_float(j ? fq[p].w : fq[p].z);
                    }
                }
                fq_prefetch(ti + 1);
            } else {
#pragma unroll
                for (int p = 0; p < A_PER; ++p) la_src[p][0] = g.A + (int64_t)(t.row0 + min(rr[p], t.nrows - 1)) * g.lda + c4;
            }
            if (consts) {
                if (g.row_scale) { const float* q = g.row_scale + t.row0 + min(ft & (BM - 1), t.nrows - 1); asm volatile("global_load_dword %0, %1, off" : "=v"(rc_sc) : "v"(q) : "memory"); }
                if (g.bias) { const float* q = g.bias + (int64_t)t.set * g.bias_stride + min(ft, BN - 1); asm volatile("global_load_dword %0, %1, off" : "=v"(rc_b) : "v"(q) : "memory"); }
            }
        };
        if constexpr (GATHER) {
            fq_prefetch(0);
            if constexpr (A_PER == 2) asm volatile("s_waitcnt vmcnt(0)" : "+v"(fq[0]), "+v"(fq[A_PER - 1]) :: "memory");
            else asm volatile("s_waitcnt vmcnt(0)" : "+v"(fq[0]) :: "memory");
        }
        la_tile(0, false);
        as_cur = as_next; inv_cur = inv_next;
        if constexpr (GATHER) {
#pragma unroll
            for (int p = 0; p < A_PER; ++p) { w_cur[p][0] = w_next[p][0]; w_cur[p][1] = w_next[p][1]; }
        }
        auto load_a = [&](int slot) {
            if (la_c == nchunks) { la_c = 0; ++la_ti; la_tile(la_ti, fast_consts); }
#pragma unroll
            for (int p = 0; p < A_PER; ++p)
#pragma unroll
                for (int j = 0; j < NJ; ++j) {
                    const float* src = la_src[p][j] + la_c * BK;
                    asm volatile("global_load_dwordx4 %0, %1, off" : "=v"(ra[slot][p][j]) : "v"(src) : "memory");
                }
            ++la_c;
        };
        int sa_c = 0, sa_ti = 0;
        auto store_a = [&](int gc, int slot) {
            if (sa_c == nchunks) {
                sa_c = 0; ++sa_ti;
                as_cur = as_next; inv_cur = inv_next;
                if constexpr (NP == 2) { if (!fast_consts) as_cur = a_scale_of(tile_of(b + sa_ti * G).set); }
                if constexpr (GATHER) {
#pragma unroll
                    for (int p = 0; p < A_PER; ++p) { w_cur[p][0] = w_next[p][0]; w_cur[p][1] = w_next[p][1]; }
                }
            }
            if (sa_c == 0 && sa_ti > 0 && fast_consts) {
                asm volatile("" : "+v"(rc_sc), "+v"(rc_b) :: "memory");
                if (ft < BM) scales[(sa_ti & 1) * GS_BM + ft] = rc_sc * inv_cur;
                if (ft < BN) biasl[(sa_ti & 1) * BN + ft] = rc_b;
            }
            ++sa_c;
            char* As = smem + (gc & 1) * A_ST;
#pragma unroll
            for (int p = 0; p < A_PER; ++p) {
                uint2 h, m, l;
                f4v v = ra[slot][p][0];
                if constexpr (GATHER) {
                    const f4v v1 = ra[slot][p][NJ - 1];
                    const float w0 = w_cur[p][0], w1 = w_cur[p][1];
                    v.x = __fmaf_rn(v1.x, w1, __fmaf_rn(v.x, w0, 0.f)); v.y = __fmaf_rn(v1.y, w1, __fmaf_rn(v.y, w0, 0.f));
                    v.z = __fmaf_rn(v1.z, w1, __fmaf_rn(v.z, w0, 0.f)); v.w = __fmaf_rn(v1.w, w1, __fmaf_rn(v.w, w0, 0.f));
                }
                if constexpr (NP == 3) {
                    gs_split4(make_float4(v.x, v.y, v.z, v.w), h, m, l);
                    *reinterpret_cast<uint2*>(As + adst[p]) = h;
                    *reinterpret_cast<uint2*>(As + A_PLANE + adst[p]) = m;
                    *reinterpret_cast<uint2*>(As + 2 * A_PLANE + adst[p]) = l;
                } else {
                    gs_split4_f16(make_float4(v.x, v.y, v.z, v.w), as_cur, h, m);
                    *reinterpret_cast<uint2*>(As + adst[p]) = h;
                    *reinterpret_cast<uint2*>(As + A_PLANE + adst[p]) = m;
                }
            }
        };
        auto stage_tile_consts = [&](int ti) {
            const GsTile t = tile_of(b + ti * G);
            const int set = t.set, row0 = t.row0, nrows = t.nrows;
            float sc = 1.f;
            if (g.row_scale) sc = g.row_scale[row0 + min(ft & (BM - 1), nrows - 1)];
            float b0 = 0.f;
            if (g.bias) b0 = (g.bias + (int64_t)set * g.bias_stride)[min(ft, BN - 1)];
            if constexpr (NP == 2) sc *= (1.f / a_scale_of(set)) * (1.f / b_scale_of(set));
            if (ft < BM) scales[(ti & 1) * GS_BM + ft] = sc;
            if (ft < BN) biasl[(ti & 1) * BN + ft] = b0;
        };
        static_assert((A_PER == 1 || A_PER == 2) && PF_DA >= 2 && PF_DA <= 8, "wait macro is written for 1 or 2 rows per lane and chunk");
#define PF_WAIT_SLOT(NEWER, SLOT)                                                                                                              \
        do {                                                                                                                                   \
            if constexpr (GATHER && A_PER == 2) asm volatile("s_waitcnt vmcnt(%4)" : "+v"(ra[SLOT][0][0]), "+v"(ra[SLOT][A_PER - 1][0]), "+v"(ra[SLOT][0][NJ - 1]), "+v"(ra[SLOT][A_PER - 1][NJ - 1]) : "n"((NEWER) * 4) : "memory"); \
            else if constexpr (GATHER) asm volatile("s_waitcnt vmcnt(%2)" : "+v"(ra[SLOT][0][0]), "+v"(ra[SLOT][0][NJ - 1]) : "n"((NEWER) * 2) : "memory"); \
            else if constexpr (A_PER == 2) asm volatile("s_waitcnt vmcnt(%2)" : "+v"(ra[SLOT][0][0]), "+v"(ra[SLOT][A_PER - 1][0]) : "n"((NEWER) * 2) : "memory"); \
            else asm volatile("s_waitcnt vmcnt(%1)" : "+v"(ra[SLOT][0][0]) : "n"((NEWER) * 1) : "memory");                                 \
        } while (0)
        stage_tile_consts(0);
        asm volatile("s_waitcnt vmcnt(0)" ::: "memory");
#pragma unroll
        for (int d = 0; d < PF_DA; ++d) if (d < total) load_a(d);
        PF_WAIT_SLOT(0, 0);
        store_a(0, 0);
        GS_BARRIER();
        for (int g0 = 0; g0 < total; g0 += PF_DA) {
#pragma unroll
            for (int u = 0; u < PF_DA; ++u) {
                const int gc = g0 + u;
                if (gc < total) {
                    if (gc + 1 < total) {
                        const int newer = min(PF_DA - 2, total - 2 - gc);
                        const int SL = (u + 1) % PF_DA;
                        if (newer >= PF_DA - 2 && PF_DA >= 2) PF_WAIT_SLOT(PF_DA - 2, SL);
                        else if (newer == 1 && PF_DA > 3) PF_WAIT_SLOT(1, SL);
                        else if (newer == 2 && PF_DA > 4) PF_WAIT_SLOT(2, SL);
                        else PF_WAIT_SLOT(0, SL);
                        store_a(gc + 1, SL);
                        if (!fast_consts && sa_c == 1 && sa_ti > 0) { stage_tile_consts(sa_ti); asm volatile("s_waitcnt vmcnt(0)" ::: "memory"); }
                    }
                    if (gc + PF_DA < total) load_a(u);
                    GS_BARRIER();
                }
            }
        }
#undef PF_WAIT_SLOT
    } else {
        const int wr = wave / WC, wc = wave % WC, li = lane & 31, kh = lane >> 5;
        const int a_lane = kh * A_OCT + (wr * 32 * MI + li) * 16, b_lane = OFF_B + kh * B_OCT + (wc * 64 + li) * 16;
        int b_st = 0;
        GS_BARRIER();
        int gc = 0;
        float vmax = 0.f; int vmax_set = -1;
        auto vmax_note = [&](unsigned bits) {
            gs_note_max(g.amax_out + (int64_t)vmax_set * GM_BOUND_PAD, bits);
            if (g.b_bound.viol && bits > 0x58800000u && bits < 0x7f800000u) atomicOr(g.b_bound.viol, GM_VIOL_RANGE);
        };
        auto vmax_flush = [&]() {
#pragma unroll
            for (int o = 32; o >= 1; o >>= 1) vmax = fmaxf(vmax, __shfl_xor(vmax, o));
            if (lane == 0) {
                unsigned* mx = reinterpret_cast<unsigned*>(smem + OFF_MAX);
                atomicMax(mx, __float_as_uint(vmax));
                __builtin_amdgcn_fence(__ATOMIC_RELEASE, "workgroup");
                const unsigned ticket = atomicAdd(mx + 1, 1u);
                __builtin_amdgcn_fence(__ATOMIC_ACQUIRE, "workgroup");
                if (ticket == 7u) {
                    const unsigned all = atomicExch(mx, 0u);
                    mx[1] = 0u;
                    vmax_note(all);
                }
            }
            vmax = 0.f;
        };
        auto vmax_flush_last = [&]() {
#pragma unroll
            for (int o = 32; o >= 1; o >>= 1) vmax = fmaxf(vmax, __shfl_xor(vmax, o));
            if (lane == 0) vmax_note(__float_as_uint(vmax));
        };
        for (int ti = 0; ti < ntb; ++ti) {
            gm_f32x16 acc[MI][2];
#pragma unroll
            for (int i = 0; i < MI; ++i)
#pragma unroll
                for (int j = 0; j < 2; ++j)
#pragma unroll
                    for (int e = 0; e < 16; ++e) acc[i][j][e] = 0.f;
            for (int c = 0; c < nchunks; ++c, ++gc) {
                const char* S = smem + (gc & 1) * A_ST;
                const char* SB = smem + b_st * B_ST;
                b_st = b_st + 1 == NB ? 0 : b_st + 1;
                if constexpr (NP == 3) {
                    gm_bf16x8 af[MI][3], bf[2][3];
#pragma unroll
                    for (int i = 0; i < MI; ++i)
#pragma unroll
                        for (int p = 0; p < 3; ++p) af[i][p] = *reinterpret_cast<const gm_bf16x8*>(S + a_lane + p * A_PLANE + i * 512);
#pragma unroll
                    for (int j = 0; j < 2; ++j)
#pragma unroll
                        for (int p = 0; p < 3; ++p) bf[j][p] = *reinterpret_cast<const gm_bf16x8*>(SB + b_lane + p * B_PLANE + j * 512);
#define PF_PROD(PA, PB)                                                                                                  \
                    _Pragma("unroll") for (int i = 0; i < MI; ++i) _Pragma("unroll") for (int j = 0; j < 2; ++j)          \
                        acc[i][j] = __builtin_amdgcn_mfma_f32_32x32x16_bf16(af[i][PA], bf[j][PB], acc[i][j], 0, 0, 0);
                    PF_PROD(2, 0) PF_PROD(0, 2) PF_PROD(1, 1) PF_PROD(1, 0) PF_PROD(0, 1) PF_PROD(0, 0)
#undef PF_PROD
                } else {
                    gm_f16x8 af[MI][2], bf[2][2];
#pragma unroll
                    for (int i = 0; i < MI; ++i)
#pragma unroll
                        for (int p = 0; p < 2; ++p) af[i][p] = *reinterpret_cast<const gm_f16x8*>(S + a_lane + p * A_PLANE + i * 512);
#pragma unroll
                    for (int j = 0; j < 2; ++j)
#pragma unroll
                        for (int p = 0; p < 2; ++p) bf[j][p] = *reinterpret_cast<const gm_f16x8*>(SB + b_lane + p * B_PLANE + j * 512);
#define PF_PROD(PA, PB)                                                                                                  \
                    _Pragma("unroll") for (int i = 0; i < MI; ++i) _Pragma("unroll") for (int j = 0; j < 2; ++j)          \
                        acc[i][j] = __builtin_amdgcn_mfma_f32_32x32x16_f16(af[i][PA], bf[j][PB], acc[i][j], 0, 0, 0);
                    PF_PROD(1, 0) PF_PROD(0, 1) PF_PROD(0, 0)
#undef PF_PROD
                }
                GS_BARRIER();
            }
            const GsTile tl = tile_of(b + ti * G);
            const int row0 = tl.row0, nrows = tl.nrows;
            const float* sc_t = scales + (ti & 1) * GS_BM;
            const int t4 = li & 3, q4 = li >> 2;
            const bool odd1 = (li & 1) != 0, odd2 = (li & 2) != 0;
            float4 b4[2];
#pragma unroll
            for (int j = 0; j < 2; ++j) b4[j] = *reinterpret_cast<const float4*>(biasl + (ti & 1) * BN + wc * 64 + j * 32 + q4 * 4);
            if constexpr (NP == 2) { if (g.amax_out && tl.set != vmax_set) { if (vmax_set >= 0) vmax_flush(); vmax_set = tl.set; } }
            const bool keep_only = g.keep_signed && !g.relu_bits && !g.zero_out;
            if (keep_only && __ballot(!(__float_as_uint(sc_t[wr * 32 * MI + (lane & (32 * MI - 1))]) >> 31)) == 0ull) continue;
#pragma unroll
            for (int i = 0; i < MI; ++i) {
#pragma unroll
                for (int gq = 0; gq < 4; ++gq) {
                    const int rl = wr * 32 * MI + i * 32 + gq * 8 + kh * 4 + t4;
                    const float sc_raw = sc_t[rl];
                    const bool keep = !g.keep_signed || !(__float_as_uint(sc_raw) >> 31);
                    if (keep_only && __ballot(keep) == 0ull) continue;
                    const float sc = fabsf(sc_raw);
                    const int64_t row = row0 + rl;
#pragma unroll
                    for (int j = 0; j < 2; ++j) {
                        float a0 = acc[i][j][gq * 4 + 0], a1 = acc[i][j][gq * 4 + 1], a2 = acc[i][j][gq * 4 + 2], a3 = acc[i][j][gq * 4 + 3];
                        gs_quad_transpose(a0, a1, a2, a3, odd1, odd2);
                        float4 v;
                        v.x = a0 * sc + b4[j].x; v.y = a1 * sc + b4[j].y; v.z = a2 * sc + b4[j].z; v.w = a3 * sc + b4[j].w;
                        if (g.relu) { v.x = v.x < 0.f ? 0.f : v.x; v.y = v.y < 0.f ? 0.f : v.y; v.z = v.z < 0.f ? 0.f : v.z; v.w = v.w < 0.f ? 0.f : v.w; }
                        if (rl >= nrows || (keep_only && !keep)) continue;
                        const int col = wc * 64 + j * 32 + q4 * 4;
                        if constexpr (NP == 2) { if (g.amax_out) vmax = fmaxf(fmaxf(vmax, fmaxf(fabsf(v.x), fabsf(v.y))), fmaxf(fabsf(v.z), fabsf(v.w))); }
                        if (g.relu_bits) g.relu_bits[(row * g.ldc + col) >> 2] = (uint8_t)((v.x > 0.f) | ((v.y > 0.f) << 1) | ((v.z > 0.f) << 2) | ((v.w > 0.f) << 3));
                        if (!keep) {
                        } else if (g.nt_store) {
                            typedef float f4v __attribute__((ext_vector_type(4)));
                            f4v vv = {v.x, v.y, v.z, v.w};
                            __builtin_nontemporal_store(vv, reinterpret_cast<f4v*>(g.C + row * g.ldc + col));
                        } else {
                            *reinterpret_cast<float4*>(g.C + row * g.ldc + col) = v;
                        }
                        if (g.zero_out) {
                            typedef float f4z __attribute__((ext_vector_type(4)));
                            f4z z;
                            asm volatile("v_mov_b32 %0, 0\n\tv_mov_b32 %1, 0\n\tv_mov_b32 %2, 0\n\tv_mov_b32 %3, 0" : "=v"(z.x), "=v"(z.y), "=v"(z.z), "=v"(z.w));
                            *reinterpret_cast<f4z*>(g.zero_out + row * g.ldc + col) = z;
                        }
                    }
                }
            }
        }
        if constexpr (NP == 2) { if (g.amax_out && vmax_set >= 0) vmax_flush_last(); }
    }
}
```

g-meta_amd/csrc/gm_internal.h:

```cpp
#pragma once
#include <hip/hip_runtime.h>
#include "gm_bound.h"
#include <stdint.h>
#include <stdio.h>
#include <mutex>
#include <stdlib.h>
#include <string.h>
#include <vector>
#include <algorithm>
#include "../../include/gmeta_hip.h"

#define GM_WAVE 64
#define GM_NXCD 8

void gm_set_error(const char* fmt, ...);

#define GM_HIP(call)                                                                              \
    do {                                                                                          \
        hipError_t e__ = (call);                                                                  \
        if (e__ != hipSuccess) {                                                                  \
            gm_set_error("%s failed: %s (%s:%d)", #call, hipGetErrorString(e__), __FILE__, __LINE__); \
            return GM_EHIP;                                                                       \
        }                                                                                         \
    } while (0)
// ... 81 lines not shown
    int32_t* d_indices_t = nullptr;
    int32_t* d_centre = nullptr;
    std::vector<int32_t> h_centre;
    float* d_norm = nullptr;
    bool weighted = false;
    bool mask_target = false;
    float* d_ew[2] = {nullptr, nullptr};
    int32_t* d_sub_set = nullptr;
    int32_t* d_tiles = nullptr;
    int32_t n_tiles = 0;
    int32_t* d_chunks = nullptr;
    int32_t n_chunks = 0;
    int32_t* d_set_chunk_off = nullptr;
    int32_t* d_heavy[2] = {nullptr, nullptr};
    int32_t n_heavy[2] = {0, 0};
    int32_t heavy_deg = 64;
    int32_t* d_sched[2] = {nullptr, nullptr};
    int32_t sched_len[2] = {0, 0};
    int32_t sched_win = 0;
    int32_t* d_hub[2] = {nullptr, nullptr}; float* d_hub_scratch[2] = {nullptr, nullptr}; int32_t hub_part[2] = {0, 0};
    int32_t hub_words[2] = {0, 0}, hub_parts[2] = {0, 0};
    mutable int32_t* d_hub2[2] = {nullptr, nullptr}; mutable float* d_hub_scratch2[2] = {nullptr, nullptr};
    mutable hipStream_t hub_stream[4] = {nullptr, nullptr, nullptr, nullptr}; mutable bool hub_used[4] = {false, false, false, false}; mutable hipEvent_t hub_ev[4] = {nullptr, nullptr, nullptr, nullptr};
    float* d_enorm[2] = {nullptr, nullptr}; int32_t* d_efeat = nullptr;
    float* d_gain = nullptr;
    void* d_fuse2 = nullptr; void* d_fuse2_feat = nullptr;
    int64_t unfused_rows = 0, unfused_edges = 0;
    int32_t* d_mid = nullptr; int32_t n_mid = 0, mid_win = 0;
    int32_t* d_sptr[2] = {nullptr, nullptr}; int32_t* d_su[2] = {nullptr, nullptr}; int32_t* d_su_feat = nullptr; float* d_sw[2] = {nullptr, nullptr};
    int32_t* d_scum[2] = {nullptr, nullptr}; int2* d_sseg[2] = {nullptr, nullptr}; int32_t* d_sxord[2] = {nullptr, nullptr};
    int32_t stream_nseg[2] = {0, 0}, stream_nwg[2] = {0, 0}, stream_hubwg[2] = {0, 0}, stream_nparts[2] = {0, 0}, stream_enorm[2] = {0, 0};
    struct stream_pending { bool pending = false; bool has_tab = false; int n_parts = 0; std::vector<int32_t> hubs, deg, tab; };
    mutable stream_pending spend[2];
    int32_t* d_sched_mid = nullptr; int32_t sched_len_mid = 0;
    mutable int64_t unfused_src = -1;
    int32_t n_c = 0;
    int32_t* d_crow = nullptr;
    float* d_cnorm = nullptr;
    float* d_norm_c = nullptr;
    float* d_norm_src = nullptr;
    int64_t n_src = 0;
    void* d_dq_tab = nullptr;
    int32_t n_e1 = 0;
    int32_t* d_e1_row = nullptr;
    int32_t* d_e1_par = nullptr;
    int32_t* d_ect = nullptr;
    float* d_norm_e1 = nullptr;
    int32_t* d_n_e1_rows = nullptr;
    mutable int64_t n_e1_rows = -1;
    mutable int64_t n_e1_edges = -1;
    void* d_fwd_tab[2] = {nullptr, nullptr};
    void* d_fwd_tab_feat = nullptr;
    float* d_obs[2] = {nullptr, nullptr};
    struct obs_list { int32_t* rows = nullptr; int32_t* len = nullptr; int32_t cap = 0, win = 0, take = 0; int32_t* sched = nullptr; int32_t sched_len = 0; mutable int64_t n = -1; };
    obs_list obs[3];
    mutable int64_t fwd_cnt[2][3] = {{-1, -1, -1}, {-1, -1, -1}};
    float* d_e1_norm = nullptr;
    float* d_e1_coef = nullptr;
    int32_t* d_c_tiles = nullptr; int32_t n_c_tiles = 0;
    int32_t* d_c_chunks = nullptr; int32_t* d_c_set_chunk_off = nullptr; int32_t n_c_chunks = 0;
    int32_t* d_e1_chunks = nullptr; int32_t* d_e1_set_chunk_off = nullptr; int32_t n_e1_chunks = 0;
    mutable int32_t* d_ro_chunks = nullptr; mutable int32_t* d_ro_multi = nullptr; mutable int32_t n_ro_chunks = 0, n_ro_multi = 0;
    mutable hipStream_t ro_stream = nullptr; mutable hipEvent_t ro_ev = nullptr;
    mutable gm_cone* cone[GM_MAX_GCN + 1] = {};
    hipStream_t stream = nullptr;
    struct slab { char* base; size_t cap, used; };
    std::vector<slab> slabs;
    std::mutex slab_mu;
    mutable hipEvent_t used_ev = nullptr;
};
int gm_batch_gains(const gm_batch* b, hipStream_t s);
int gm_balloc_bytes(gm_batch* b, void** p, size_t bytes, hipStream_t s);
template <class T> static inline int gm_balloc(gm_batch* b, T** p, size_t n, hipStream_t s) { return gm_balloc_bytes(b, (void**)p, (n ? n : 1) * sizeof(T), s); }
void gm_batch_mark_use(const gm_batch* b, hipStream_t st);
int gm_batch_wait_build(const gm_batch* b, hipStream_t s);
static inline int gm_hop_feat_dim(const gm_store* st, int centres, int D) { return st->feat_dim + centres * (D + 2); }

struct gm_knobs {
    int timing;
    int extract_pref16;
    int gemm_mode;
    int gemm_split_min_tiles;
    int centre_store, dead_rows;
    int fuse_agg, head_stage;
    int fuse_diff;
    int agg_mid_win;
    int agg_obs_list;
    int agg_mid_list;
    int query_streams;
    int head_threads;
    int split16_min_rows;
    int split_pieces;
    int wgrad_split_min_chunks;
    int agg_stream;
    int agg_stream_min_rows;
    int neg_round;
    int pair_lanes;
    int cand_round;
    int walk_chunk;
    int walk_lanes;
    int ppr_chunk;
    int ppr_cols;
    int dist_chunk;
    int dist_cols;
    int dist_plane_kib;
    int cand_bitmap;
    int sketch_chunk;
    int sketch_mib;
    int prop_chunk;
    int prop_mib;
};
const gm_knobs& gm_knob();

int gm_nbr_index(const gm_store* s);
void gm_nbr_release(const gm_store* s);
int gm_pair_lanes(const gm_store* s, int32_t g, const char* what, int* lpp);
int gm_pair_scores_launch(const gm_store* s, int32_t g, int lpp, const int32_t* d_pairs, int64_t n, int mask, float* d_out, hipStream_t st);

#define GM_CAND_THREADS 256
#define GM_CAND_WAVES (GM_CAND_THREADS / GM_WAVE)
#define GM_CAND_MAX_K 1024

__device__ __forceinline__ unsigned long long gm_cand_key(uint32_t score_bits, int32_t w) {
    return ((unsigned long long)score_bits << 32) | (unsigned long long)(0xFFFFFFFFu - (uint32_t)w);
}

__device__ __forceinline__ int gm_cand_scan(int v, int* part, int* total) {
    const int lane = (int)threadIdx.x & (GM_WAVE - 1), wave = (int)threadIdx.x / GM_WAVE;
    int inc = v;
#pragma unroll
    for (int o = 1; o < GM_WAVE; o <<= 1) { const int t = __shfl_up(inc, o, GM_WAVE); if (lane >= o) inc += t; }
    __syncthreads();
    if (lane == GM_WAVE - 1) part[wave] = inc;
    __syncthreads();
    int base = 0, tot = 0;
#pragma unroll
    for (int w = 0; w < GM_CAND_WAVES; ++w) { const int p = part[w]; tot += p; if (w < wave) base += p; }
    *total = tot;
    return base + inc;
}
// ... 167 lines not shown
int gm_agg_stream_args(gm_agg_args& a, const gm_batch* b, int o, bool gather, hipStream_t s);
bool gm_stream_ok(const gm_agg_args& g);
bool gm_stream_batch_ok(const gm_batch* b, int o);
int gm_launch_stream(const gm_agg_args& g, int nt, hipStream_t s);
int gm_stream_tables(gm_batch* b, int o, const int32_t* hubs_host, const int32_t* deg_host, int n_hubs, int n_parts, const std::vector<int32_t>* part_tab, hipStream_t s,
                     gm_stager* sg);
#define GM_FUSE_SELF 0x40000000
#define GM_FUSE_ZERO 0x20000000
const float* gm_zero_row(hipStream_t s);
#ifndef GM_ZERO_ROWS
#define GM_ZERO_ROWS 1
#endif
#define GM_FUSE_MAXDEG 2
#define GM_AGG_HUB_LD 512
struct gm_agg_sched { int32_t* d_sched = nullptr; int32_t len = 0; int32_t* d_hub = nullptr; float* d_hub_scratch = nullptr; int32_t hub_part = 0; int32_t hub_words = 0, parts = 0;
                      std::vector<int32_t> tab; };
int gm_batch_hub_order(const gm_batch* b, int o, hipStream_t s, int set = 0);
int gm_batch_hub_alt(const gm_batch* b, hipStream_t s);
template <class A> inline int gm_agg_hub(A& a, const gm_batch* b, int o, hipStream_t s, int set = 0) {
    const bool alt = set == 1 && b->d_hub2[o];
    a.hub = alt ? b->d_hub2[o] : b->d_hub[o]; a.hub_scratch = alt ? b->d_hub_scratch2[o] : b->d_hub_scratch[o]; a.hub_part = b->hub_part[o];
    return a.hub ? gm_batch_hub_order(b, o, s, alt ? 1 : 0) : GM_OK;
}
int gm_agg_window(int64_t rows, int64_t edges);
struct gm_stager;
int gm_agg_schedule_flat(gm_batch* b, int64_t rows, int win, const int32_t* pos, int n_heavy, const std::vector<int32_t>& tab, int32_t** d_sched, int32_t* len, hipStream_t s, gm_stager* sg,
                         const uint8_t* keep = nullptr);
int gm_agg_schedule(gm_batch* b, int64_t rows, int win, const int32_t* heavy_host, const int32_t* heavy_deg_host, int n_heavy, gm_agg_sched* out, hipStream_t s, gm_stager* sg);
int gm_heavy_deg();
int gm_heavy_deg_for(int64_t rows, int64_t edges);
int gm_launch_aggregate(const gm_agg_args& a, hipStream_t s);

struct gm_gemm_args {
    const float* A; int64_t lda;
    const float* B; int64_t b_stride;
    int transB;
    float* C; int64_t ldc;
    int K, N;
    const float* row_scale;
    const float* row_scale_keep;
    int64_t n_keep;
    const float* bias; int64_t bias_stride;
    int relu;
    const float* mask_h;
    const uint8_t* mask_b;
    uint8_t* relu_bits;
    const uint16_t* Bsplit; int64_t bsplit_stride;
    const void* fuse2; const float* zside; int64_t ldz;
    int np; gm_bound a_bound, b_bound; unsigned* amax_out;
    float* zero_out;
    const int32_t* tiles;
    int n_tiles;
    int64_t rows;
    int* launched;
};
#define GM_GEMM_ID_GLDS4 1
#define GM_GEMM_ID_GLDS2 2
#define GM_GEMM_ID_GLDS1 3
#define GM_GEMM_ID_GLDS_SMALL 4
#define GM_GEMM_ID_NN(WC, VEC, TB) (10 + 4 * ((WC) == 4 ? 2 : (WC) == 2 ? 1 : 0) + 2 * (VEC) + (TB))
#define GM_GEMM_ID_SPLIT(GATHER, MI, WC, NP) (30 + 10 * (GATHER) + ((MI) == 2 ? 0 : (WC) == 4 ? 2 : 4) + ((NP) == 2))
#define GM_GEMM_BM 128
int gm_launch_gemm_nn(const gm_gemm_args& a, hipStream_t s);
int gm_gemm_mode();
bool gm_gemm_split_ok(int n_tiles, int K, int N);
int gm_split_weights(const float* params, int64_t pstride, int64_t w_off, int K, int N, int trans, int sets, uint16_t* out, hipStream_t s, int np = 3,
                     gm_bound bound = gm_no_bound());
int gm_amax(const float* x, int64_t stride, int64_t off, int64_t n, int sets, unsigned* out, int64_t out_stride, hipStream_t s);
int gm_amax_segs(const float* x, const int64_t* off, const int64_t* n, int segs, unsigned* out, int64_t out_stride, hipStream_t s);
int gm_split_np();

struct gm_wgrad_hold { int n = 0; int sets[GM_MAX_GCN] = {}; alignas(16) unsigned char slot[GM_MAX_GCN][256] = {}; };
struct gm_wgrad_args {
    const float* A; int64_t lda; int K;
    const int32_t* a_row;
    const float* G; int64_t ldg; int N;
    const float* Gb; int64_t ldgb;
    const float* a_scale;
    const int32_t* chunks;
    int n_chunks;
    const int32_t* set_chunk_off;
    int sets;
    float* partial;
    float* dW; int64_t dw_stride;
    float* db; int64_t db_stride;
    const float* sgd_cur; int64_t sgd_cur_stride; float* sgd_next; int64_t sgd_next_stride; float sgd_lr;
    int64_t w_off, b_off;
    int np; gm_bound a_bound, g_bound; int pl_np; gm_bound pl_bound;
    uint16_t* pl_fwd; uint16_t* pl_dz;
    float* wt_next;
    int64_t rows;
    const void* fuse2; const float* gx; int64_t ldgx;
    int64_t a_rows;
    const float* g_keep;
    gm_wgrad_hold* hold; int hold_this;
    int pick;
};
#define GM_WGRAD_PICK_EXACT 1
#define GM_WGRAD_PICK_SPLIT 2
#define GM_WGRAD_ROWS 1024
int gm_launch_wgrad(const gm_wgrad_args& a, hipStream_t s);
bool gm_wgrad_gather_ok(int n_chunks, int K, int N);

int gm_num_cus();
int gm_func_full_lds(const void* fn);
#define GM_WGRAD_EXTRA_ROUND_PCT 25
// ... 53 lines not shown
```

g-meta_amd/csrc/model.hip:

```cpp
#include <algorithm>
#include <atomic>
#include <map>
#include <stdlib.h>
#include "gm_internal.h"


__device__ __forceinline__ float wave_sumf(float v) {
#pragma unroll
    for (int o = 32; o > 0; o >>= 1) v += __shfl_xor(v, o, 64);
    return v;
}

struct HeadK {
    const float* H; int64_t ldh; int Hd;
    const int32_t* sub_off; const int32_t* centre; int nc; const int32_t* sub_set; const int32_t* set_sub_off;
    const float* params; int64_t pstride; int64_t wl_off, bl_off; int hc, C; int subs;
    int compact;
    unsigned* dq_amax;
    int subs_per_set;
};

__device__ __forceinline__ int64_t centre_row(const HeadK& k, int s, int which) {
    return k.compact ? (int64_t)s * k.nc + which : (int64_t)k.sub_off[s] + k.centre[s * k.nc + which];
}
// ... 518 lines not shown
    const unsigned vw = viol ? *viol : 0u;
    for (int64_t id = blockIdx.x * (int64_t)blockDim.x + threadIdx.x; id <= tot; id += (int64_t)gridDim.x * blockDim.x) {
        float s = 0.f;
        if (id == tot) { out[id] = (float)vw; continue; }
        if (id < P) { const int64_t src = id < cut ? id : id + shift; if (gq) for (int t = 0; t < T; ++t) s += gq[t * stride + src] + gp[t * stride + src]; }
        else if (id < P + K1) { for (int t = 0; t < T; ++t) s += lq[t * K1 + (id - P)]; if (vw && id == P + K1 - 1) s = __uint_as_float(0x7fc00000u); }
        else if (id < P + 2 * K1) { for (int t = 0; t < T; ++t) s += aq[t * K1 + (id - P - K1)]; }
        else if (id == P + 2 * K1) s = (float)T;
        else s = aq[id - P - 2 * K1 - 1];
        out[id] = s;
    }
}

struct Carver {
    char* base; int64_t used = 0, cap;
    Carver(void* p, int64_t c) : base((char*)p), cap(c) {}
    template <class T> T* take(int64_t n) {
        const int64_t bytes = ((n > 0 ? n : 1) * (int64_t)sizeof(T) + 255) / 256 * 256;
        T* r = base ? (T*)(base + used) : nullptr;
        used += bytes;
        return r;
    }
    bool ok() const { return !base || used <= cap; }
};

#define GM_W_HEADROOM 1024.f
struct PlaneDir {
    const float* fw0 = nullptr; int64_t TP = 0; int K = 0;
    uint16_t* base = nullptr; int64_t per_k = 0;
    int64_t off[GM_MAX_GCN][2] = {};
    bool valid[64][GM_MAX_GCN][2] = {};
    int index_of(const float* params) const {
        if (!base || !fw0 || params < fw0) return 0;
        const int64_t d = params - fw0;
        if (d % TP) return 0;
        const int64_t k = d / TP + 1;
        return (k >= 1 && k <= K && k < 64) ? (int)k : 0;
    }
    uint16_t* slot(int k, int l, int o) const { return (k && off[l][o] >= 0) ? base + (int64_t)(k - 1) * per_k + off[l][o] : nullptr; }
    uint16_t* lookup(const float* params, int l, int o) const { const int k = index_of(params); return (k && off[l][o] >= 0 && valid[k][l][o]) ? slot(k, l, o) : nullptr; }
    unsigned* wam = nullptr; const float* theta = nullptr;
    unsigned* viol = nullptr;
    bool w_bound(const float* params, int l, gm_bound& bd) const {
        bd = gm_no_bound();
        if (!wam || !(index_of(params) || params == theta)) return false;
        bd.amax = wam + (int64_t)l * GM_BOUND_PAD; bd.stride = 0; bd.gain = nullptr; bd.hgain = GM_W_HEADROOM; bd.viol = viol;
        return true;
    }
};

enum PassKind { PASS_PLAIN = 0, PASS_FWD_ONLY = 1, PASS_DIFF = 2 };
enum RowSet { ROWS_ALL, ROWS_SRC, ROWS_E1, ROWS_CENTRE };
enum DqFill { DQ_MEMSET, DQ_ZEROED, DQ_CENTRE };
struct LayerPlan { bool split, fuse; RowSet formed, stored; bool relu_bits; const gm_batch::obs_list* list; };
struct PassPlan { PassKind kind; LayerPlan layer[GM_MAX_GCN]; DqFill dq; bool t_centre, dq_e1; const gm_batch::obs_list* t_list; };

struct GcnCtx {
    const gm_batch* b; gm_layout L;
    PlaneDir* pd;
    bool is_support = false;
    PassPlan plan = {};
    bool t_zero = false;
    float* Z[GM_MAX_GCN]; float* H[GM_MAX_GCN]; float* X0; float* bufA; float* bufB; float* partial;
    float* partial_l[GM_MAX_GCN];
    gm_wgrad_hold hold;
    uint16_t* Wsplit;
    float* WTl[GM_MAX_GCN];
    const float* wt_of[GM_MAX_GCN]; int64_t wt_stride[GM_MAX_GCN];
    uint8_t* M[GM_MAX_GCN];
    float* cG2; float* cT2; float* cG1; float* partial_c;
    float* Pool; float* Gpool; float* ro_part;
    const float* x0_user; const int32_t* centre; int z1_valid;
    int zw[GM_MAX_GCN];
    const gm_cone* cone;
    SgdK sgd;
    int hub_set = 0;
    int np = 3; unsigned* am = nullptr; int am_passes = 0, am_pass = -1;
    const unsigned* feat_bound = nullptr;
    bool hv[GM_MAX_GCN] = {}, tv[GM_MAX_GCN] = {}; bool dqv = false;
    unsigned* am_slot(int i) const { return am + ((int64_t)am_pass * (2 * L.n_gcn + 1) + i) * b->sets * GM_BOUND_PAD; }
    unsigned* amH(int l) const { return am_slot(l); }
    unsigned* amT(int l) const { return am_slot(L.n_gcn + l); }
    unsigned* amdQ() const { return am_slot(2 * L.n_gcn); }
};
static bool in_bound(const GcnCtx& c, int l, gm_bound& bd) {
    bd = gm_no_bound();
    if (c.np != 2 || c.am_pass < 0 || !c.b->d_gain) return false;
    if (l == 0) {
        if (c.x0_user || !c.feat_bound) return false;
        bd.amax = c.feat_bound; bd.stride = 1;
    } else {
        if (!c.hv[l - 1]) return false;
        bd.amax = c.amH(l - 1); bd.stride = GM_BOUND_PAD;
    }
    bd.gain = c.b->d_gain; bd.hgain = 1.f;
    return true;
}
static bool dq_bound(const GcnCtx& c, int l, gm_bound& bd) {
    bd = gm_no_bound();
    if (c.np != 2 || c.am_pass < 0 || !c.b->d_gain) return false;
    if (l == c.L.n_gcn - 1) { if (!c.dqv) return false; bd.amax = c.amdQ(); bd.gain = nullptr; }
    else { if (!c.tv[l + 1]) return false; bd.amax = c.amT(l + 1); bd.gain = c.b->d_gain + 1; }
    bd.stride = GM_BOUND_PAD; bd.hgain = 1.f;
    return true;
}
static int weight_planes(GcnCtx& c, const float* params, int64_t pstride, int l, int o, hipStream_t st, gm_gemm_args& g) {
    const int fi = c.L.dims[l], fo = c.L.dims[l + 1];
    const bool want16 = o ? dq_bound(c, l, g.a_bound) : in_bound(c, l, g.a_bound);
// ... 76 lines not shown
    Carver cv(nullptr, 0);
    gcn_carve(c, cv);
    return cv.used + 256;
}

static int head_subs_per_set(const gm_batch* b) {
    int n = b->sets > 0 ? b->subs / b->sets : 0;
    for (int t = 0; t <= b->sets && n; ++t) if (b->h_set_sub_off[t] != t * n) n = 0;
    return n;
}
static HeadK make_head(const GcnCtx& c, const float* params, int64_t pstride) {
    const gm_layout& L = c.L; const gm_batch* b = c.b;
    HeadK k{};
    k.H = c.H[L.n_gcn - 1]; k.ldh = L.dims[L.n_gcn]; k.Hd = L.dims[L.n_gcn];
    k.sub_off = b->d_sub_off; k.centre = c.centre ? c.centre : b->d_centre; k.nc = b->centres; k.sub_set = b->d_sub_set;
    k.set_sub_off = b->d_set_sub_off; k.params = params; k.pstride = pstride; k.wl_off = L.wl_off; k.bl_off = L.bl_off;
    k.hc = L.hc; k.C = L.n_out; k.subs = b->subs; k.compact = c.cone ? 1 : 0;
    if (mean_readout(c)) { k.H = c.Pool; k.compact = 1; k.nc = 1; }
    k.dq_amax = (c.np == 2 && c.am_pass >= 0) ? c.amdQ() : nullptr;
    k.subs_per_set = head_subs_per_set(b);
    return k;
}
static int launch_head_fwd(const GcnCtx& c, const float* params, int64_t pstride, float* logits, hipStream_t st) {
    hipLaunchKernelGGL(k_head_fwd, dim3((c.b->subs + 3) / 4), dim3(256), 0, st, make_head(c, params, pstride), logits);
    GM_HIP(hipGetLastError());
    return GM_OK;
}
static int launch_head_bwd(GcnCtx& c, const float* params, int64_t pstride, const float* dlogits, float* dparams, int64_t dstride, float* dQ, float* Gc, hipStream_t st) {
    const HeadK k = make_head(c, params, pstride);
    hipLaunchKernelGGL(k_head_bwd, dim3(c.b->sets), dim3(256), 0, st, k, dlogits, dparams, dstride, dQ, Gc);
    GM_HIP(hipGetLastError());
    if (dQ && k.dq_amax) c.dqv = true;
    return GM_OK;
}

static int launch_agg(const gm_agg_args& a, int64_t bytes, int64_t strict_bytes, hipStream_t st) {
    gm_prof_agg_begin(st, bytes); gm_prof_note(GM_PROF_AGG_STRICT, strict_bytes);
    const int rc = gm_launch_aggregate(a, st);
    gm_prof_agg_end(st);
    return rc;
}
static int batch_agg(const GcnCtx& c, int dir, hipStream_t st, gm_agg_args& a) {
    const gm_batch* b = c.b;
    a = gm_agg_args{};
    if (dir == 0) { a.indptr = b->d_indptr; a.indices = b->d_indices; } else { a.indptr = b->d_indptr_t; a.indices = b->d_indices_t; }
    a.heavy = b->d_heavy[dir]; a.n_heavy = b->n_heavy[dir]; a.heavy_deg = b->heavy_deg;
    a.sched = b->d_sched[dir]; a.sched_len = b->sched_len[dir]; a.sched_win = b->sched_win;
    GM_TRY(gm_agg_hub(a, b, dir, st, c.hub_set));
    a.rows = b->rows;
    if (b->weighted) a.e_w = b->d_ew[dir];
    return GM_OK;
}

struct RowView { const float* keep; const float* sign; const void* tab; int obs; int64_t n; };
static RowView row_view(const gm_batch* b, RowSet rs, bool gather) {
    if (rs == ROWS_E1) return {b->d_norm_e1, b->d_obs[1], gather ? b->d_fwd_tab_feat : b->d_fwd_tab[1], 1, b->n_e1};
    if (rs == ROWS_CENTRE) return {b->d_norm_c, b->d_obs[0], b->d_fwd_tab[0], 0, b->n_c};
    return {rs == ROWS_SRC ? b->d_norm_src : nullptr, nullptr, gather ? b->d_fuse2_feat : b->d_fuse2, -1, rs == ROWS_SRC ? b->n_src : b->rows};
}
static int64_t rows_kept(const gm_batch* b, RowSet rs, hipStream_t st) { return rs != ROWS_E1 ? row_view(b, rs, false).n : gm_prof_enabled() ? gm_batch_e1_rows(b, st) : std::min<int64_t>(b->n_e1, b->rows); }

static int partial_agg_bytes(const gm_batch* b, RowSet formed, int fi, bool gather, hipStream_t st, int64_t* bytes, int64_t* strict) {
    const bool all = formed == ROWS_ALL;
    int64_t w[3] = {std::min<int64_t>(b->unfused_rows, row_view(b, formed, gather).n), b->unfused_edges, std::min<int64_t>(b->unfused_edges, b->rows)};
    if (gm_prof_enabled() && all) w[2] = gm_batch_unfused_sources(b, st);
    if (gm_prof_enabled() && !all) GM_TRY(gm_batch_fwd_counts(b, row_view(b, formed, gather).obs, st, w));
    const int64_t pb0 = 4 * (b->rows + 1) + (all ? 4 : 8) * b->unfused_rows + 4 * w[1] + 4 * w[0] * (int64_t)fi;
    *bytes = pb0 + 4 * w[2] * (int64_t)fi;
    *strict = pb0 + 4 * (gather ? std::min<int64_t>(w[2], b->feat_rows) : w[2]) * (int64_t)fi;
    gm_prof_note(GM_PROF_AGG_BOUND, pb0 + 4 * std::min<int64_t>(w[1], b->rows) * (int64_t)fi - *bytes);
    return GM_OK;
}
static int64_t t_centre_agg_bytes(const gm_batch* b, RowSet out, int fi, bool maskbits, hipStream_t st) {
    const int64_t n_out = rows_kept(b, out, st), e_out = (out == ROWS_E1 && gm_prof_enabled()) ? gm_batch_e1_edges(b, st) : b->edges;
    return 4 * (b->rows + 1) + 4 * b->rows + 4 * e_out + (maskbits ? n_out * (int64_t)fi / 4 : 0) + 4 * ((int64_t)b->n_c + n_out) * (int64_t)fi;
}

static bool dz_split_ok(const GcnCtx& c, int l) { return c.Wsplit && gm_gemm_split_ok(c.b->n_tiles, c.L.dims[l + 1], c.L.dims[l]); }
static bool dz_centre_ok(const GcnCtx& c, int l) { return dz_split_ok(c, l) && c.L.dims[l + 1] >= 64 && c.L.dims[l + 1] <= 4096 && c.b->d_dq_tab; }
static float* t_zero_rows(const GcnCtx& c) {
    const gm_layout& L = c.L; const int Lg = L.n_gcn;
    if (c.cone || Lg < 2 || !c.bufB || L.dims[Lg - 1] > L.dims[Lg]) return nullptr;
    for (int l = 0; l < Lg - 1; ++l) if (std::min(L.dims[l], L.dims[l + 1]) > L.dims[Lg - 1]) return nullptr;
    return c.bufB + c.b->rows * (int64_t)L.dims[Lg - 1];
}
static int dead_row_level(const GcnCtx& c) { return (gm_knob().centre_store == 0 || c.centre) ? 0 : gm_knob().dead_rows; }
static int t_zero_fill(GcnCtx& c, hipStream_t st) {
    float* z = t_zero_rows(c);
    c.t_zero = z && dead_row_level(c) >= 2 && dz_centre_ok(c, c.L.n_gcn - 1) && c.b->d_ect && c.b->d_norm_e1;
    if (c.t_zero) GM_HIP(hipMemsetAsync(z, 0, sizeof(float) * GM_ZERO_ROWS * c.L.dims[c.L.n_gcn - 1], st));
    return GM_OK;
}

int gm_gather_rows(const gm_batch* b, const int32_t* feat_row, int64_t n, int F, float* out, hipStream_t st);
static int cone_forward(GcnCtx& c, const float* params, int64_t pstride, float* logits, hipStream_t st, int reuse_z1, int skip_head);
static int cone_backward(GcnCtx& c, const float* params, int64_t pstride, const float* dlogits, float* dparams, int64_t dstride, hipStream_t st, int skip_head);

static std::atomic<int> g_fuse_agg_override{-1};
extern "C" void gm_set_fuse_agg(int32_t on) { g_fuse_agg_override.store(on < 0 ? -1 : (on ? 1 : 0), std::memory_order_relaxed); }
extern "C" int32_t gm_get_fuse_agg(void) { const int o = g_fuse_agg_override.load(std::memory_order_relaxed); return o >= 0 ? o : gm_knob().fuse_agg; }

static int plan_check(const GcnCtx& c, const PassPlan& p) {
    for (int l = 0; l < c.L.n_gcn; ++l) {
        GM_REQUIRE(p.layer[l].formed == ROWS_ALL || p.layer[l].fuse, GM_EINVAL, "plan: layer %d is formed on a row set but not fused: nothing reads it through the set's table", l);
        GM_REQUIRE(p.layer[l].formed != ROWS_CENTRE || (l == c.L.n_gcn - 1 && p.layer[l].stored == ROWS_CENTRE && (l > 0 || c.x0_user)), GM_EINVAL, "plan: layer %d is formed on the centre rows, but is not a last layer that stores them alone and reads no feature table", l);
    }
    GM_REQUIRE(!(p.kind == PASS_DIFF && p.layer[c.L.n_gcn - 1].formed == ROWS_CENTRE) || p.dq == DQ_CENTRE, GM_EINVAL, "plan: a restricted differentiated pass must leave dQ to its centre rows");
    GM_REQUIRE(!p.dq_e1 || p.t_centre, GM_EINVAL, "plan: dQ_{L-1} on the sources of the centres' in-edges needs T_L on its centre rows");
    return GM_OK;
}
static int plan_check(const GcnCtx& c, const PassPlan& p);
static int plan_pass(const GcnCtx& c, const float* params, int64_t pstride, PassKind kind, int reuse_z1, PassPlan* plan) {
    const gm_layout& L = c.L; const gm_batch* b = c.b;
    const int Lg = L.n_gcn, last = Lg - 1, level = dead_row_level(c), centre_store = gm_knob().centre_store;
    const bool mean = mean_readout(c);
    auto agg_first = [&](int l) { return L.dims[l] <= L.dims[l + 1]; };
    auto wgrad_tabled = [&](int l) { return gm_wgrad_gather_ok(b->n_chunks, L.dims[l], L.dims[l + 1]); };
    PassPlan p{}; p.kind = kind; p.dq = DQ_MEMSET;
    for (int l = 0; l < Lg; ++l) {
        LayerPlan& lp = p.layer[l]; const int fi = L.dims[l];
        lp.relu_bits = !agg_first(l) || kind != PASS_FWD_ONLY;
        if (!agg_first(l)) continue;
        lp.split = c.Wsplit && gm_gemm_split_ok(b->n_tiles, fi, L.dims[l + 1]) && ((uintptr_t)(params + L.b_off[l]) & 15) == 0 && pstride % 4 == 0;
        const bool gather = (l == 0 && !c.x0_user);
        const bool keeps_stream = gm_knob().fuse_diff == 2 && c.is_support && gm_knob().agg_stream && gm_stream_batch_ok(b, 0);
        const bool diff_ok = kind == PASS_DIFF && gm_knob().fuse_diff && !keeps_stream && c.np != 2 && !c.cone && wgrad_tabled(l);
        lp.fuse = (kind == PASS_FWD_ONLY || diff_ok) && gm_get_fuse_agg() && lp.split && !(l == 0 && reuse_z1) && fi >= 64 && fi % 4 == 0 && b->d_fuse2 && b->d_enorm[0] &&
                  (!gather || (b->feat_ld % 4 == 0 && b->feat_ld >= fi)) &&
                  2 * b->unfused_rows <= b->rows;
        if (l == last) { if (!mean && !c.centre && b->d_norm_c && (centre_store >= 2 || (centre_store == 1 && kind == PASS_FWD_ONLY))) lp.stored = ROWS_CENTRE; }
        else if (level >= 1 && lp.split && (kind == PASS_FWD_ONLY || (kind == PASS_DIFF && c.M[l])) && L.dims[l + 1] <= L.dims[l + 2] && b->d_norm_src) lp.stored = ROWS_SRC;
    }
    if (kind == PASS_DIFF && agg_first(last) && !mean)
        p.dq = (level >= 1 && p.layer[last].split && c.np != 2 && b->d_norm_c && (last == 0 || dz_centre_ok(c, last)) && wgrad_tabled(last)) ? DQ_CENTRE : DQ_ZEROED;
    p.t_centre = p.dq == DQ_CENTRE && c.t_zero && level >= 2;
    p.dq_e1 = p.t_centre && Lg == 2 && agg_first(0) && c.np != 2 && wgrad_tabled(0);
    const bool last_ok = !mean && c.np != 2 && b->d_norm_c && b->d_norm_e1 && b->d_fwd_tab[0] && b->d_obs[0] && agg_first(last) && p.layer[last].fuse;
    const bool below_ok = Lg >= 2 && agg_first(Lg - 2) && b->d_fwd_tab[1] && b->d_fwd_tab_feat && b->d_obs[1];
    const bool fwd3 = kind == PASS_FWD_ONLY && level >= 3 && centre_store >= 1 && last_ok && (Lg >= 2 || c.x0_user);
    const bool diff4 = kind == PASS_DIFF && level >= 4 && centre_store >= 2 && p.t_centre && !reuse_z1 && Lg >= 2 && last_ok;
    if (fwd3 || diff4) p.layer[last].formed = ROWS_CENTRE;
    if (below_ok && ((fwd3 && p.layer[Lg - 2].split) || (diff4 && p.dq_e1 && p.layer[0].fuse && c.M[0]))) {
        p.layer[Lg - 2].stored = ROWS_E1; if (p.layer[Lg - 2].fuse) p.layer[Lg - 2].formed = ROWS_E1; }
    if (gm_knob().agg_obs_list && c.hub_set == 0) {
        auto taken = [&](int k) { return b->obs[k].take ? &b->obs[k] : nullptr; };
        for (int l = 0; l < Lg; ++l)
            if (p.layer[l].fuse && p.layer[l].formed != ROWS_ALL) p.layer[l].list = taken(p.layer[l].formed == ROWS_CENTRE ? 0 : 1);
        if (p.dq_e1) p.t_list = taken(2);
    }
    *plan = p; return plan_check(c, p);
}
static void agg_take_list(gm_agg_args& a, const gm_batch::obs_list& ol) {
    a.rowlist = ol.rows; a.n_list = ol.cap; a.n_list_dev = ol.len; a.list_win = ol.win;
    a.sched = ol.sched; a.sched_len = ol.sched ? ol.sched_len : 0; a.sched_win = ol.win;
}

static int gcn_forward(GcnCtx& c, const float* params, int64_t pstride, float* logits, hipStream_t st, int reuse_z1, int skip_head = 0, PassKind kind = PASS_PLAIN) {
    if (c.cone) return cone_forward(c, params, pstride, logits, st, reuse_z1, skip_head);
    const gm_layout& L = c.L; const gm_batch* b = c.b;
    if (!c.x0_user) GM_TRY(gm_check_feat_dim(b, L.dims[0], "forward"));
    GM_REQUIRE((L.link != 0) == (b->centres == 2), GM_EINVAL, "forward: link_pred model needs a 2-centre batch and vice versa");
    const float* xin = c.x0_user;
    GM_TRY(plan_pass(c, params, pstride, kind, reuse_z1, &c.plan));
    const PassPlan& plan = c.plan; const bool mean = mean_readout(c);
    if (mean) GM_TRY(readout_tables(b, st));
    if (c.np == 2) {
        ++c.am_pass;
        GM_REQUIRE(c.am_pass < c.am_passes, GM_EINVAL, "forward: more passes than bound slots (%d)", c.am_passes);
        for (int l = 0; l < GM_MAX_GCN; ++l) c.hv[l] = c.tv[l] = false;
        c.dqv = false;
    }
    for (int l = 0; l < L.n_gcn; ++l) {
        const int fi = L.dims[l], fo = L.dims[l + 1];
        const bool gather = (l == 0 && !c.x0_user);
        const LayerPlan& lp = plan.layer[l]; uint8_t* relu_bits = lp.relu_bits ? c.M[l] : nullptr;
        if (fi > fo) {
            const float* A = xin; int64_t lda = fi;
            if (gather) { GM_TRY(gm_gather_rows(b, b->d_feat_row, b->rows, fi, c.X0, st)); A = c.X0; }
            gm_gemm_args g{}; g.A = A; g.lda = lda; g.B = params + L.w_off[l]; g.b_stride = pstride; g.C = c.Z[l]; g.ldc = fo; g.K = fi; g.N = fo;
            g.row_scale = b->d_norm; g.tiles = b->d_tiles; g.n_tiles = b->n_tiles; g.rows = b->rows;
            GM_TRY(gm_launch_gemm_nn(g, st));
            gm_agg_args a; GM_TRY(batch_agg(c, 0, st, a));
            a.x = c.Z[l]; a.ldx = fo; a.s_out = b->d_norm;
            a.bias = params + L.b_off[l]; a.bias_stride = pstride; a.set_row_off = b->d_set_row_off; a.n_sets = b->sets; a.relu = 1;
            a.out = c.H[l]; a.width = fo; a.relu_bits = relu_bits;
            GM_TRY(launch_agg(a, gm_aggregate_bytes(b, fo), gm_aggregate_bytes(b, fo), st));
        } else {
            const float* x = gather ? b->feat : xin; const int64_t ldx = gather ? b->feat_ld : fi;
            if (!(l == 0 && reuse_z1 && c.z1_valid)) {
                gm_agg_args a; GM_TRY(batch_agg(c, 0, st, a));
                a.s_in = b->d_norm; a.e_w = b->d_enorm[0]; a.out = c.Z[l]; a.width = fi;
                a.x = x; a.ldx = ldx; if (gather) { a.x_row = b->d_feat_row; a.x_idx = b->d_efeat; }
                if (lp.fuse) {
                    a.skip_on = 1; a.skip_lo = 0; a.skip_hi = GM_FUSE_MAXDEG;
                    if (b->d_mid && c.hub_set == 0 && gm_knob().agg_mid_list && (b->n_heavy[0] == 0 || b->d_sched_mid)) {
                        a.rowlist = b->d_mid; a.n_list = b->n_mid; a.list_win = b->mid_win;
                        if (b->n_heavy[0] > 0) { a.sched = b->d_sched_mid; a.sched_len = b->sched_len_mid; a.sched_win = b->mid_win; }
                        else { a.sched = nullptr; a.sched_len = 0; }
                    }
                    if (lp.formed != ROWS_ALL) { a.s_out = row_view(b, lp.formed, gather).sign; a.keep_signed = 1; }
                    if (lp.list && lp.list->take == 1) agg_take_list(a, *lp.list);
                    if (!(lp.list && lp.list->take == 2)) {
                        int64_t pb, pbs;
                        GM_TRY(partial_agg_bytes(b, lp.formed, fi, gather, st, &pb, &pbs));
                        GM_TRY(launch_agg(a, pb, pbs, st));
                    }
                } else {
                    if (a.e_w) GM_TRY(gm_agg_stream_args(a, b, 0, gather, st));
                    int64_t strict = gm_aggregate_bytes(b, fi);
                    if (gather) strict += 4 * b->rows - 4 * b->rows * (int64_t)fi + std::min<int64_t>(4 * b->rows * (int64_t)fi, 4 * b->feat_rows * (int64_t)fi);
                    GM_TRY(launch_agg(a, gm_aggregate_bytes(b, fi), strict, st));
                    if (l == 0) c.z1_valid = 1;
                }
            }
            gm_gemm_args g{}; g.A = c.Z[l]; g.lda = fi; g.B = params + L.w_off[l]; g.b_stride = pstride; g.C = c.H[l]; g.ldc = fo; g.K = fi; g.N = fo;
            g.row_scale = b->d_norm; g.bias = params + L.b_off[l]; g.bias_stride = pstride; g.relu = 1; g.tiles = b->d_tiles; g.n_tiles = b->n_tiles; g.rows = b->rows;
            g.relu_bits = relu_bits;
            if (lp.stored != ROWS_ALL) { g.row_scale_keep = row_view(b, lp.stored, false).keep; g.n_keep = rows_kept(b, lp.stored, st); }
            if (lp.split) {
                GM_TRY(weight_planes(c, params, pstride, l, 0, st, g));
                GM_REQUIRE(!(l == L.n_gcn - 1 && plan.dq == DQ_CENTRE) || g.np == 3, GM_EINVAL, "forward: dQ is left to its centre rows, which needs the three-piece kernels");
            }
            if (l == L.n_gcn - 1 && plan.dq == DQ_ZEROED) g.zero_out = c.bufA;
            if (lp.fuse) { g.A = x; g.lda = ldx; g.zside = c.Z[l]; g.ldz = fi; g.fuse2 = row_view(b, lp.formed, gather).tab; }
            GM_TRY(gm_launch_gemm_nn(g, st));
        }
        xin = c.H[l];
    }
    if (mean) GM_TRY(readout_fwd(c, st));
    return skip_head ? GM_OK : launch_head_fwd(c, params, pstride, logits, st);
}

static int gcn_backward_sparse(GcnCtx& c, const float* params, int64_t pstride, const float* dlogits, float* dparams, int64_t dstride, hipStream_t st, int skip_head);
static bool sparse_bwd_ok(const gm_layout& L);

static int gcn_backward(GcnCtx& c, const float* params, int64_t pstride, const float* dlogits, float* dparams, int64_t dstride, hipStream_t st, int sparse = 0,
                        int skip_head = 0) {
    if (c.cone) return cone_backward(c, params, pstride, dlogits, dparams, dstride, st, skip_head);
    if (sparse && sparse_bwd_ok(c.L)) return gcn_backward_sparse(c, params, pstride, dlogits, dparams, dstride, st, skip_head);
    const gm_layout& L = c.L; const gm_batch* b = c.b; const int Lg = L.n_gcn;
    float* dQ = c.bufA; float* T = c.bufB;
    c.hold.n = 0;
    const PassPlan& plan = c.plan;
    const bool dq_centre = skip_head && plan.dq == DQ_CENTRE;
    const bool t_centre = dq_centre && plan.t_centre, dq_e1 = t_centre && plan.dq_e1;
    const bool dq_filled = !skip_head && !mean_readout(c);
    if (!skip_head && mean_readout(c)) {
        GM_TRY(launch_head_bwd(c, params, pstride, dlogits, dparams, dstride, nullptr, c.Gpool, st));
        GM_TRY(readout_bwd(c, st));
    } else if (!skip_head) {
        GM_HIP(hipMemsetAsync(dQ, 0, sizeof(float) * b->rows * L.dims[Lg], st));
        GM_TRY(launch_head_bwd(c, params, pstride, dlogits, dparams, dstride, dQ, nullptr, st));
    }
    for (int l = Lg - 1; l >= 0; --l) {
        const int fi = L.dims[l], fo = L.dims[l + 1];
        const float* Xprev = l > 0 ? c.H[l - 1] : (c.x0_user ? c.x0_user : c.X0);
        const float* maskprev = l > 0 ? c.H[l - 1] : nullptr;
        const uint8_t* maskbits = l > 0 ? c.M[l - 1] : nullptr;
        if (maskbits) maskprev = nullptr;
        gm_wgrad_args w{}; w.chunks = b->d_chunks; w.n_chunks = b->n_chunks; w.set_chunk_off = b->d_set_chunk_off; w.sets = b->sets; w.rows = b->rows;
        w.partial = c.partial; w.dW = dparams + L.w_off[l]; w.dw_stride = dstride; w.db = dparams + L.b_off[l]; w.db_stride = dstride;
        w.a_scale = b->d_norm; w.K = fi; w.N = fo;
        wgrad_sgd(w, c, l);
        w.hold = &c.hold; w.hold_this = l > 0 ? 1 : 0;
        if (l > 0) w.partial = c.partial_l[l];
        if (fi > fo) {
            gm_agg_args a; GM_TRY(batch_agg(c, 1, st, a));
            a.x = dQ; a.ldx = fo; a.s_in = b->d_norm; a.e_w = b->d_enorm[1]; a.out = T; a.width = fo;
            GM_TRY(launch_agg(a, gm_aggregate_bytes(b, fo), gm_aggregate_bytes(b, fo), st));
            w.A = Xprev; w.lda = fi; w.G = T; w.ldg = fo; w.Gb = dQ; w.ldgb = fo;
            GM_TRY(gm_launch_wgrad(w, st));
            if (l > 0) {
                gm_gemm_args g{}; g.A = T; g.lda = fo; g.B = params + L.w_off[l]; g.b_stride = pstride; g.transB = 1; g.C = dQ; g.ldc = fi; g.K = fo; g.N = fi;
                g.row_scale = b->d_norm; g.mask_h = maskprev; g.mask_b = maskbits; g.tiles = b->d_tiles; g.n_tiles = b->n_tiles; g.rows = b->rows;
                GM_TRY(gm_launch_gemm_nn(g, st));
            }
        } else {
            w.A = c.Z[l]; w.lda = fi; w.G = dQ; w.ldg = fo;
            const RowSet g_rows = (dq_centre && l == Lg - 1) ? ROWS_CENTRE : (dq_e1 && l == Lg - 2) ? ROWS_E1 : ROWS_ALL;
            w.g_keep = row_view(b, g_rows, false).keep;
            const RowSet z_rows = plan.layer[l].formed;
            if (plan.layer[l].fuse) {
                const bool gather = l == 0 && !c.x0_user;
                w.fuse2 = row_view(b, z_rows, gather).tab;
                w.gx = gather ? b->feat : (l > 0 ? c.H[l - 1] : c.x0_user); w.ldgx = gather ? b->feat_ld : fi;
            }
            if (z_rows != ROWS_ALL) {
                GM_REQUIRE(w.g_keep || dq_filled, GM_EINVAL, "backward: layer %d was formed on its observable rows only, but its weight gradient got neither flagged rows of G (g_keep) nor a dQ this call zero-filled", l);
                if (gm_prof_enabled()) w.a_rows = rows_kept(b, z_rows, st);
            }
            if (l > 0) {
                gm_gemm_args g{}; g.A = dQ; g.lda = fo; g.C = T; g.ldc = fi; g.K = fo; g.N = fi;
                g.row_scale = b->d_norm; g.tiles = b->d_tiles; g.n_tiles = b->n_tiles; g.rows = b->rows;
                const bool use_split = dz_split_ok(c, l);
                const bool use_wt = !use_split && c.WTl[l] && fi % 64 == 0 && fo % 16 == 0;
                if (use_split) {
                    GM_TRY(weight_planes(c, params, pstride, l, 1, st, g));
                    g.B = params + L.w_off[l]; g.b_stride = pstride; g.transB = 1;
                    if (dq_centre && l == Lg - 1) { g.fuse2 = b->d_dq_tab; g.zside = dQ; g.ldz = fo; }
                    if (t_centre && l == Lg - 1) { g.row_scale_keep = row_view(b, ROWS_CENTRE, false).keep; g.n_keep = rows_kept(b, ROWS_CENTRE, st); }
                } else if (use_wt) {
                    if (!(c.wt_of[l] == params && c.wt_stride[l] == pstride)) {
                        const int nt = pstride ? b->sets : 1;
                        hipLaunchKernelGGL(k_transpose_w, dim3((fo + 31) / 32, (fi + 31) / 32, nt), dim3(256), 0, st, params, pstride, L.w_off[l], fi, fo, c.WTl[l]);
                        GM_HIP(hipGetLastError());
                        c.wt_of[l] = params; c.wt_stride[l] = pstride;
                    }
                    g.B = c.WTl[l]; g.b_stride = pstride ? (int64_t)fi * fo : 0; g.transB = 0;
                } else { g.B = params + L.w_off[l]; g.b_stride = pstride; g.transB = 1; }
                GM_TRY(gm_launch_gemm_nn(g, st));
                if (use_wt && c.sgd.next) { w.wt_next = c.WTl[l]; }
            }
            int kn = 0;
            if (c.pd && c.sgd.next && (kn = c.pd->index_of(c.sgd.next)) != 0) { w.pl_fwd = c.pd->slot(kn, l, 0); w.pl_dz = c.pd->slot(kn, l, 1); }
            if (c.np == 2) {
                gm_bound ab, gb;
                if (in_bound(c, l, ab) && dq_bound(c, l, gb)) { w.np = 2; w.a_bound = ab; w.g_bound = gb; }
                if (kn) {
                    if (c.pd->w_bound(c.sgd.next, l, w.pl_bound)) w.pl_np = 2; else { w.pl_fwd = nullptr; w.pl_dz = nullptr; }
                }
            }
            GM_TRY(gm_launch_wgrad(w, st));
            if (kn) { c.pd->valid[kn][l][0] = w.pl_fwd != nullptr; c.pd->valid[kn][l][1] = w.pl_dz != nullptr; }
            if (w.wt_next) { c.wt_of[l] = c.sgd.next; c.wt_stride[l] = c.sgd.next_stride; }
            if (l > 0) {
                gm_agg_args a; GM_TRY(batch_agg(c, 1, st, a));
                a.x = T; a.ldx = fi; a.s_out = b->d_norm; a.mask_h = maskprev; a.mask_b = maskbits;
                a.out = dQ; a.width = fi;
                int64_t by = gm_aggregate_bytes(b, fi);
                if (t_centre && l == Lg - 1) {
                    a.x_idx = b->d_ect;
                    const RowSet out = dq_e1 ? ROWS_E1 : ROWS_ALL;
                    if (dq_e1) { a.s_out = row_view(b, out, false).keep; a.keep_signed = 1; }
                    if (dq_e1 && plan.t_list && plan.t_list->take == 1) agg_take_list(a, *plan.t_list);
                    by = t_centre_agg_bytes(b, out, fi, maskbits != nullptr, st);
                }
                if (!(t_centre && l == Lg - 1 && dq_e1 && plan.t_list && plan.t_list->take == 2)) GM_TRY(launch_agg(a, by, by, st));
            }
        }
    }
    return GM_OK;
}

static bool sparse_bwd_ok(const gm_layout& L) {
    if (L.n_gcn > 2 || L.readout == GM_READOUT_MEAN) return false;
    for (int l = 0; l < L.n_gcn; ++l) if (L.dims[l] > L.dims[l + 1]) return false;
    return true;
}

static int gcn_backward_sparse(GcnCtx& c, const float* params, int64_t pstride, const float* dlogits, float* dparams, int64_t dstride, hipStream_t st, int skip_head) {
    const gm_layout& L = c.L; const gm_batch* b = c.b;
    const int Lg = L.n_gcn, fiL = L.dims[Lg - 1], foL = L.dims[Lg];
    if (!skip_head) GM_TRY(launch_head_bwd(c, params, pstride, dlogits, dparams, dstride, nullptr, c.cG2, st));
// ... 1211 lines not shown
```

include/gmeta_hip.h:

```cpp
#ifndef GMETA_HIP_H
#define GMETA_HIP_H
#include <stdint.h>
#ifdef __cplusplus
extern "C" {
#endif

#define GM_OK 0
#define GM_EINVAL (-1)
#define GM_ENOMEM (-2)
#define GM_EHIP (-3)
#define GM_ERANGE (-4)
#define GM_MAX_GCN 4

typedef struct gm_store gm_store_t;
typedef struct gm_batch gm_batch_t;

typedef struct gm_seed { int32_t graph, i, j; } gm_seed_t;

typedef struct gm_model {
    int32_t n_gcn;
    int32_t dims[GM_MAX_GCN + 1];
    int32_t n_out;
    int32_t link_pred;
} gm_model_t;
// ... 94 lines not shown
enum gm_field {
    GM_F_SUB_OFF = 0,
    GM_F_SET_SUB_OFF,
    GM_F_PARENT,
    GM_F_GRAPH,
    GM_F_INDPTR,
    GM_F_INDICES,
    GM_F_INDPTR_T,
    GM_F_INDICES_T,
    GM_F_CENTRE,
    GM_F_NORM,
    GM_F_FEAT_ROW,
    GM_F_NORM_SRC,
    GM_F_NORM_CENTRE,
    GM_F_EDGE_W,
    GM_F_EDGE_W_T = 14,
    GM_F_HOP = 15,
    GM_F_NORM_E1 = 16,
    GM_F_EDGE_CENTRE_T = 17,
    GM_F_OBS_CENTRE = 18,
    GM_F_OBS_E1 = 19
};
int32_t gm_batch_weighted(const gm_batch_t* b);
int gm_batch_read(const gm_batch_t* b, int32_t field, void* host_dst, int64_t bytes);
int gm_batch_device_ptr(const gm_batch_t* b, int32_t field, void** dptr);
int gm_batch_source_rows(const gm_batch_t* b, int64_t* n_rows);
int gm_batch_e1_source_rows(const gm_batch_t* b, int64_t* n_rows);

int gm_gather_features(const gm_batch_t* b, float* x_out, void* stream);

int gm_aggregate(const gm_batch_t* b, int32_t transposed, int32_t gather, const float* x, int32_t width,
                 const float* s_in, const float* s_out, float* out, void* stream);
int64_t gm_aggregate_bytes(const gm_batch_t* b, int32_t width);

int64_t gm_model_param_count(const gm_model_t* m);
int64_t gm_gcn_ws_bytes(const gm_batch_t* b, const gm_model_t* m);
int gm_gcn_forward(const gm_batch_t* b, const gm_model_t* m, const float* params, int64_t param_stride,
                   const float* x0, const int32_t* centre_local, float* logits, void* ws, int64_t ws_bytes,
                   void* stream);
int gm_gcn_backward(const gm_batch_t* b, const gm_model_t* m, const float* params, int64_t param_stride,
                    const float* x0, const int32_t* centre_local, const float* dlogits, float* dparams,
                    int64_t dparam_stride, void* ws, int64_t ws_bytes, void* stream);

int gm_dense_update(const gm_batch_t* b, const float* x, int32_t K, const float* W, int64_t w_stride, int32_t N, float* out, int32_t mode,
                    void* stream);
int gm_dense_gemm(const gm_batch_t* b, const float* x, int64_t ldx, int32_t K, const float* W, int64_t w_stride, int32_t trans_w, int32_t N,
                  float* out, int64_t ldc, const float* s, const float* s_keep, const float* bias, int64_t bias_stride, int32_t relu,
                  uint8_t* relu_bits, const float* mask_h, const uint8_t* mask_b, float* zero_out, uint32_t* amax_out, int32_t mode,
                  int32_t* launched, void* stream);
int gm_dense_fused_gemm(const gm_batch_t* b, int32_t table, const float* x, int64_t ldx, int32_t K, const float* zside, int64_t ldz, const float* zfull,
                        int64_t ldzf, const float* W, int64_t w_stride, int32_t N, float* out, int64_t ldc, const float* s, const float* s_keep,
                        const float* bias, int64_t bias_stride, int32_t relu, uint8_t* relu_bits, float* zero_out, uint32_t* amax_out, int32_t mode,
                        int32_t* launched, void* stream);
int gm_dense_aggregate(const gm_batch_t* b, int32_t transposed, int32_t x_src, const float* x, int64_t ldx, int32_t width, int32_t scale_src,
                       const float* s_in, const float* s_out, int32_t keep_signed, const float* bias, int64_t bias_stride, int32_t relu,
                       uint8_t* relu_bits, const float* mask_h, const uint8_t* mask_b, int32_t hubs, const int32_t* rowlist, int64_t n_list,
                       int32_t list_win, int32_t list_sched, int32_t skip_lo, int32_t skip_hi, int32_t stream_ok, float* out, int32_t* launched,
                       void* stream);
int gm_dense_obs_lists(const gm_batch_t* b, int64_t* info, void* stream);
int gm_dense_agg_info(const gm_batch_t* b, int32_t transposed, int64_t* info);
int gm_dense_fuse_counts(const gm_batch_t* b, int64_t* counts);
int gm_dense_agg_table(const gm_batch_t* b, int32_t which, int32_t transposed, void* dst, int64_t n, void* stream);
int gm_dense_dz_centre(const gm_batch_t* b, const float* dQ, int32_t K, const float* W, int64_t w_stride, int32_t N, float* T, void* stream);
int gm_dense_wgrad_centre(const gm_batch_t* b, const float* x, int32_t Kx, const float* dQ, int32_t N, float* dW, int64_t dw_stride, float* db,
                          int64_t db_stride, void* stream);
int gm_dense_agg_centre_t(const gm_batch_t* b, float* T, int32_t width, const uint8_t* mask_b, float* out, int32_t keep, void* stream);
int gm_dense_wgrad_e1(const gm_batch_t* b, const float* x, int32_t Kx, const float* dQ, int32_t N, float* dW, int64_t dw_stride, float* db,
                      int64_t db_stride, void* stream);
int gm_dense_wgrad(const gm_batch_t* b, const float* x, int64_t ldx, int32_t K, const float* g, int64_t ldg, int32_t N, const float* s,
                   const float* gb, int64_t ldgb, float* dW, int64_t dw_stride, float* db, int64_t db_stride, int32_t mode,
                   const float* cur, float* next, int64_t p_stride, float lr, float* wt, uint16_t* pl_fwd, uint16_t* pl_dz, void* stream);
int gm_dense_wgrad_fused(const gm_batch_t* b, int32_t table, const float* A, int64_t lda, int32_t K, const float* gx, int64_t ldgx, const float* g,
                         int64_t ldg, int32_t N, const float* s, const float* g_keep, float* dW, int64_t dw_stride, float* db, int64_t db_stride,
                         int32_t mode, void* stream);

int gm_proto_loss_spt(const gm_batch_t* b, const float* logits, int32_t n_out, const int32_t* y, int32_t n_support,
                      float* loss, float* acc, float* protos, float* dlogits, void* stream);
int gm_proto_loss_qry(const gm_batch_t* b, const float* logits, int32_t n_out, const int32_t* y, const float* protos,
                      int32_t c_task, float* loss, float* acc, float* dlogits, float* dprotos, void* stream);
void gm_set_ragged_classes(int32_t on);
int32_t gm_get_ragged_classes(void);
int gm_dense_head_loss(const gm_batch_t* b, const float* H, int32_t Hd, int32_t nc, int32_t compact, int32_t C, const float* params,
                       int64_t param_stride, int64_t wl_off, int64_t bl_off, const int32_t* centre_local, const int32_t* y, int32_t mode,
                       int32_t n_support, const float* protos, int32_t c_task, const int32_t* spt_labels, const int32_t* spt_counts, float* logits,
                       float* dlogits, float* dprotos, float* protos_out, float* loss, float* acc, int32_t bwd, float* dparams,
                       int64_t dparam_stride, float* dQ, float* Gc, const float* sgd_cur, float* sgd_next, int64_t sgd_stride, float sgd_lr,
                       uint32_t* dq_amax, int32_t path, int32_t* launched, void* stream);

#define GM_READOUT_CENTRE 0
#define GM_READOUT_MEAN 1
void gm_set_readout(int32_t mode);
int32_t gm_get_readout(void);

int64_t gm_meta_ws_bytes(const gm_batch_t* spt, const gm_batch_t* qry, const gm_model_t* m, const gm_hparams_t* hp);
int64_t gm_meta_out_floats(const gm_batch_t* spt, const gm_model_t* m, const gm_hparams_t* hp);
int gm_meta_step(const gm_batch_t* spt, const gm_batch_t* qry, const int32_t* y_spt, const int32_t* y_qry,
                 const gm_model_t* m, const gm_hparams_t* hp, const float* theta, float* out, int64_t out_floats,
                 void* ws, int64_t ws_bytes, void* stream);

int64_t gm_adapt_ws_bytes(const gm_batch_t* spt, const gm_model_t* m, const gm_hparams_t* hp);
int gm_meta_adapt(const gm_batch_t* spt, const int32_t* y_spt, const gm_model_t* m, const gm_hparams_t* hp, const float* theta, float* fw_out,
                  int64_t fw_stride, float* protos_out, int32_t c_task, void* ws, int64_t ws_bytes, void* stream);
int64_t gm_predict_ws_bytes(const gm_batch_t* qry, const gm_model_t* m, const gm_hparams_t* hp);
int gm_proto_predict(const gm_batch_t* qry, const gm_model_t* m, const gm_hparams_t* hp, const float* params, int64_t param_stride,
                     const float* protos, const int32_t* n_classes, int32_t c_task, float* logits_out, float* logp_out, int32_t* pred_out,
                     void* ws, int64_t ws_bytes, void* stream);
// ... 26 lines not shown
```

Measured before the change: 1931.

## Skip loads for GEMM tiles with no kept centre or e1 rows

A new kernel builds per-tile liveness flags for the centre and e1 row sets. Forward-only fused split GEMMs, and the centre-transposed backward GEMM, compact each block's tile list to live tiles in LDS, so producer and consumer waves skip A/B staging and epilogues for dead tiles. Dead tiles still get dummy zero MFMA chunks, which keeps some compute cost and adds a liveness pass plus list-building overhead. A test export, gm_dense_fused_gemm_rows, with a grid override is also added.

```diff
diff --git a/g-meta_amd/_lib.py b/g-meta_amd/_lib.py
--- a/g-meta_amd/_lib.py
+++ b/g-meta_amd/_lib.py
@@ -88,6 +88,7 @@
     'gm_dense_update': (C.c_int, [vp, vp, i32, vp, i64, i32, vp, i32, vp]),
     'gm_dense_gemm': (C.c_int, [vp, vp, i64, i32, vp, i64, i32, i32, vp, i64, vp, vp, vp, i64, i32, vp, vp, vp, vp, vp, i32, vp, vp]),
     'gm_dense_fused_gemm': (C.c_int, [vp, i32, vp, i64, i32, vp, i64, vp, i64, vp, i64, i32, vp, i64, vp, vp, vp, i64, i32, vp, vp, vp, i32, vp, vp]),
+    'gm_dense_fused_gemm_rows': (C.c_int, [vp, i32, i32, i32, i32, i32, vp, i64, i32, vp, i64, vp, i64, vp, i64, i32, vp, i64, vp, i64, i32, vp, vp, vp, i32, vp, vp]),
     'gm_dense_wgrad_fused': (C.c_int, [vp, i32, vp, i64, i32, vp, i64, vp, i64, i32, vp, vp, vp, i64, vp, i64, i32, vp]),
     'gm_dense_aggregate': (C.c_int, [vp, i32, i32, vp, i64, i32, i32, vp, vp, i32, vp, i64, i32, vp, vp, vp, i32, vp, i64, i32, i32, i32, i32, i32, vp, vp, vp]),
     'gm_dense_agg_info': (C.c_int, [vp, i32, vp]),
@@ -136,7 +137,7 @@
     'gm_head_loss_debug': (C.c_int, [i32, vp]),
 }
 
-LATER_EXPORTS = {'gm_dense_obs_lists'}
+LATER_EXPORTS = {'gm_dense_obs_lists', 'gm_dense_fused_gemm_rows'}
 
 _lib = None
 
diff --git a/g-meta_amd/csrc/common.hip b/g-meta_amd/csrc/common.hip
--- a/g-meta_amd/csrc/common.hip
+++ b/g-meta_amd/csrc/common.hip
@@ -337,6 +337,7 @@
         k.agg_mid_list = env("GM_AGG_MID_LIST", 1);
         k.agg_mid_win = env("GM_AGG_MID_WIN", 0);
         k.agg_obs_list = env("GM_AGG_OBS_LIST", 1);
+        k.dead_tiles = env("GM_DEAD_TILES", 1);
         k.split_pieces = env("GM_SPLIT_PIECES", 3);
         k.split16_min_rows = env("GM_SPLIT16_MIN_ROWS", 65536);
         k.wgrad_split_min_chunks = env("GM_WGRAD_SPLIT_MIN_CHUNKS", -1);
@@ -367,7 +368,7 @@
     (void)gm_knob();
     static const struct { const char* name; int gm_knobs::*field; } tab[] = {
         {"GM_GEMM_SPLIT_MIN_TILES", &gm_knobs::gemm_split_min_tiles}, {"GM_CENTRE_STORE", &gm_knobs::centre_store}, {"GM_DEAD_ROWS", &gm_knobs::dead_rows},
-        {"GM_HEAD_STAGE", &gm_knobs::head_stage}, {"GM_HEAD_THREADS", &gm_knobs::head_threads}, {"GM_QUERY_STREAMS", &gm_knobs::query_streams}, {"GM_AGG_MID_LIST", &gm_knobs::agg_mid_list}, {"GM_AGG_MID_WIN", &gm_knobs::agg_mid_win}, {"GM_AGG_OBS_LIST", &gm_knobs::agg_obs_list}, {"GM_AGG_STREAM", &gm_knobs::agg_stream}, {"GM_AGG_STREAM_MIN_ROWS", &gm_knobs::agg_stream_min_rows},
+        {"GM_HEAD_STAGE", &gm_knobs::head_stage}, {"GM_HEAD_THREADS", &gm_knobs::head_threads}, {"GM_QUERY_STREAMS", &gm_knobs::query_streams}, {"GM_AGG_MID_LIST", &gm_knobs::agg_mid_list}, {"GM_AGG_MID_WIN", &gm_knobs::agg_mid_win}, {"GM_AGG_OBS_LIST", &gm_knobs::agg_obs_list}, {"GM_DEAD_TILES", &gm_knobs::dead_tiles}, {"GM_AGG_STREAM", &gm_knobs::agg_stream}, {"GM_AGG_STREAM_MIN_ROWS", &gm_knobs::agg_stream_min_rows},
         {"GM_SPLIT16_MIN_ROWS", &gm_knobs::split16_min_rows}, {"GM_WGRAD_SPLIT_MIN_CHUNKS", &gm_knobs::wgrad_split_min_chunks}, {"GM_TIMING", &gm_knobs::timing},
         {"GM_FUSE_DIFF", &gm_knobs::fuse_diff}, {"GM_EXTRACT_PREF16", &gm_knobs::extract_pref16},
         {"neg_round", &gm_knobs::neg_round}, {"GM_NEG_ROUND", &gm_knobs::neg_round},
diff --git a/g-meta_amd/csrc/dense_exports.hip b/g-meta_amd/csrc/dense_exports.hip
--- a/g-meta_amd/csrc/dense_exports.hip
+++ b/g-meta_amd/csrc/dense_exports.hip
@@ -89,10 +89,10 @@
     return rc;
 }
 
-extern "C" int gm_dense_fused_gemm(const gm_batch_t* b, int32_t table, const float* x, int64_t ldx, int32_t K, const float* zside, int64_t ldz,
-                                   const float* zfull, int64_t ldzf, const float* W, int64_t w_stride, int32_t N, float* out, int64_t ldc, const float* s,
-                                   const float* s_keep, const float* bias, int64_t bias_stride, int32_t relu, uint8_t* relu_bits, float* zero_out,
-                                   uint32_t* amax_out, int32_t mode, int32_t* launched, void* stream) {
+static int dense_fused_gemm(const gm_batch_t* b, int32_t rowset, int32_t live_on, int32_t grid, int32_t table, const float* x, int64_t ldx, int32_t K, const float* zside, int64_t ldz,
+                            const float* zfull, int64_t ldzf, const float* W, int64_t w_stride, int32_t N, float* out, int64_t ldc, const float* s,
+                            const float* s_keep, const float* bias, int64_t bias_stride, int32_t relu, uint8_t* relu_bits, float* zero_out,
+                            uint32_t* amax_out, int32_t mode, int32_t* launched, void* stream) {
     GM_REQUIRE(b && W && out && zside && K >= 1 && N >= 1 && ldz >= K && ldc >= N && (mode == 1 || mode == 2) && (table == 0 || table == 1), GM_EINVAL,
                "dense_fused_gemm: bad arguments");
     GM_REQUIRE(b->d_fuse2 && b->d_fuse2_feat, GM_EINVAL, "dense_fused_gemm: the batch carries no source tables");
@@ -111,6 +111,13 @@
     g.zside = zside; g.ldz = ldz;
     if (table == 1) { g.A = b->feat; g.lda = b->feat_ld; g.fuse2 = b->d_fuse2_feat; }
     else { g.A = x; g.lda = ldx; g.fuse2 = b->d_fuse2; }
+    if (rowset >= 0) {
+        GM_REQUIRE(rowset <= 1 && !(rowset == 0 && table == 1) && grid >= 0, GM_EINVAL, "dense_fused_gemm_rows: bad row set");
+        GM_REQUIRE(b->d_fwd_tab[0] && b->d_fwd_tab[1] && b->d_fwd_tab_feat && b->d_tile_live[0] && b->d_tile_live[1], GM_EINVAL, "dense_fused_gemm_rows: the batch carries no row-set tables");
+        g.fuse2 = rowset == 0 ? b->d_fwd_tab[0] : table == 1 ? b->d_fwd_tab_feat : b->d_fwd_tab[1];
+        if (live_on) g.tile_live = b->d_tile_live[rowset];
+        g.grid_test = grid;
+    }
     uint16_t* planes = nullptr; unsigned* slots = nullptr;
     int rc = gm_alloc(&planes, (size_t)wsets * 3 * K * N, st);
     gm_bound wb = gm_no_bound();
@@ -129,6 +136,22 @@
     if (slots) gm_dev_free(slots, st);
     gm_batch_mark_use(b, st);
     return rc;
+}
+
+extern "C" int gm_dense_fused_gemm(const gm_batch_t* b, int32_t table, const float* x, int64_t ldx, int32_t K, const float* zside, int64_t ldz,
+                                   const float* zfull, int64_t ldzf, const float* W, int64_t w_stride, int32_t N, float* out, int64_t ldc, const float* s,
+                                   const float* s_keep, const float* bias, int64_t bias_stride, int32_t relu, uint8_t* relu_bits, float* zero_out,
+                                   uint32_t* amax_out, int32_t mode, int32_t* launched, void* stream) {
+    return dense_fused_gemm(b, -1, 0, 0, table, x, ldx, K, zside, ldz, zfull, ldzf, W, w_stride, N, out, ldc, s, s_keep, bias, bias_stride, relu, relu_bits, zero_out, amax_out,
+                            mode, launched, stream);
+}
+extern "C" int gm_dense_fused_gemm_rows(const gm_batch_t* b, int32_t rowset, int32_t keep, int32_t live_on, int32_t grid, int32_t table, const float* x, int64_t ldx, int32_t K,
+                                        const float* zside, int64_t ldz, const float* zfull, int64_t ldzf, const float* W, int64_t w_stride, int32_t N, float* out, int64_t ldc,
+                                        const float* bias, int64_t bias_stride, int32_t relu, uint8_t* relu_bits, float* zero_out, uint32_t* amax_out, int32_t mode,
+                                        int32_t* launched, void* stream) {
+    GM_REQUIRE(b && (rowset == 0 || rowset == 1) && b->d_norm_c && b->d_norm_e1, GM_EINVAL, "dense_fused_gemm_rows: bad arguments");
+    return dense_fused_gemm(b, rowset, live_on, grid, table, x, ldx, K, zside, ldz, zfull, ldzf, W, w_stride, N, out, ldc, b->d_norm, keep ? (rowset == 0 ? b->d_norm_c : b->d_norm_e1) : nullptr,
+                            bias, bias_stride, relu, relu_bits, zero_out, amax_out, mode, launched, stream);
 }
 
 extern "C" int gm_dense_dz_centre(const gm_batch_t* b, const float* dQ, int32_t K, const float* W, int64_t w_stride, int32_t N, float* T, void* stream) {
@@ -374,7 +397,14 @@
     return GM_OK;
 }
 extern "C" int gm_dense_agg_table(const gm_batch_t* b, int32_t which, int32_t transposed, void* dst, int64_t n, void* stream) {
-    GM_REQUIRE(b && dst && n >= 0 && which >= 0 && which <= 12, GM_EINVAL, "dense_agg_table: bad arguments");
+    GM_REQUIRE(b && dst && n >= 0 && which >= 0 && which <= 14, GM_EINVAL, "dense_agg_table: bad arguments");
+    if (which >= 13) {
+        const int32_t* fl = b->d_tile_live[which - 13];
+        GM_REQUIRE(fl && n <= b->n_tiles, GM_EINVAL, "dense_agg_table: table %d holds %lld entries", which, (long long)(fl ? b->n_tiles : 0));
+        if (n) GM_HIP(hipMemcpyAsync(dst, fl, 4 * (size_t)n, hipMemcpyDeviceToDevice, (hipStream_t)stream));
+        gm_batch_mark_use(b, (hipStream_t)stream);
+        return GM_OK;
+    }
     if (which >= 10) {
         const gm_batch::obs_list& ol = b->obs[which - 10];
         GM_REQUIRE(ol.rows && n <= ol.cap, GM_EINVAL, "dense_agg_table: table %d holds %lld entries", which, (long long)(ol.rows ? ol.cap : 0));
diff --git a/g-meta_amd/csrc/extract.hip b/g-meta_amd/csrc/extract.hip
--- a/g-meta_amd/csrc/extract.hip
+++ b/g-meta_amd/csrc/extract.hip
@@ -726,6 +726,15 @@
         obs_c[r] = c ? 1.f : -1.f; obs_e1[r] = e ? 1.f : -1.f;
     }
 }
+__global__ __launch_bounds__(GM_GEMM_BM) void k_tile_live(const int32_t* tiles, int n_tiles, const float* norm_c, const float* norm_e1, int32_t* live_c, int32_t* live_e1) {
+    const int t = blockIdx.x;
+    if (t >= n_tiles) return;
+    const int row0 = tiles[3 * t + 1], nrows = tiles[3 * t + 2], r = threadIdx.x;
+    const bool in = r < nrows;
+    const int c = in && !(__float_as_uint(norm_c[(int64_t)row0 + r]) >> 31), e = in && !(__float_as_uint(norm_e1[(int64_t)row0 + r]) >> 31);
+    const int any_c = __syncthreads_or(c), any_e = __syncthreads_or(e);
+    if (r == 0) { live_c[t] = any_c ? 1 : 0; live_e1[t] = any_e ? 1 : 0; }
+}
 __global__ void k_fwd_count(const int32_t* indptr, const int32_t* indices, const float* obs, int64_t rows, int maxdeg, uint32_t* bits, unsigned long long* out) {
     unsigned long long nr = 0, ne = 0;
     for (int64_t r = blockIdx.x * (int64_t)blockDim.x + threadIdx.x; r < rows; r += (int64_t)gridDim.x * blockDim.x) {
@@ -1066,6 +1075,11 @@
                                tc, te, tf, b->d_obs[0], b->d_obs[1]);
             GM_HIP(hipGetLastError());
             b->d_fwd_tab[0] = tc; b->d_fwd_tab[1] = te; b->d_fwd_tab_feat = tf;
+        }
+        if (b->d_tiles && b->n_tiles > 0) {
+            GM_TRY(gm_balloc(b, &b->d_tile_live[0], (size_t)b->n_tiles, s)); GM_TRY(gm_balloc(b, &b->d_tile_live[1], (size_t)b->n_tiles, s));
+            hipLaunchKernelGGL(k_tile_live, dim3(b->n_tiles), dim3(GM_GEMM_BM), 0, s, b->d_tiles, b->n_tiles, b->d_norm_c, b->d_norm_e1, b->d_tile_live[0], b->d_tile_live[1]);
+            GM_HIP(hipGetLastError());
         }
         if (gm_knob().agg_mid_list && h_cnt[0] <= cap && h_cnt[1] <= cap) {
             const int64_t walked_fwd = b->d_mid ? b->n_mid : b->rows;
diff --git a/g-meta_amd/csrc/gemm.hip b/g-meta_amd/csrc/gemm.hip
--- a/g-meta_amd/csrc/gemm.hip
+++ b/g-meta_amd/csrc/gemm.hip
@@ -455,7 +455,8 @@
             k.f2 = reinterpret_cast<const int4*>(a.fuse2); k.zside = a.zside; k.ldz = a.ldz; k.zrow = gm_zero_row(s);
             GM_REQUIRE(k.zrow, GM_EHIP, "gemm: zero row allocation failed");
             const int mult_f = a.n_tiles >= 16 * grid_cap ? 2 : 3;
-            const int grid = std::min(a.n_tiles, mult_f * grid_cap);
+            const int grid = std::min(a.n_tiles, a.grid_test > 0 ? a.grid_test : mult_f * grid_cap);
+            if (a.tile_live && a.row_scale_keep && !a.relu_bits && !a.zero_out && !f16) k.tile_live = a.tile_live;
             GM_TRY(f16 ? (launch_gemm_split<true, 2>(a, k, grid, false, s)) : (launch_gemm_split<true, 3>(a, k, grid, false, s)));
         } else {
             const int grid = std::min(a.n_tiles, grid_cap);
diff --git a/g-meta_amd/csrc/gemm_split.h b/g-meta_amd/csrc/gemm_split.h
--- a/g-meta_amd/csrc/gemm_split.h
+++ b/g-meta_amd/csrc/gemm_split.h
@@ -37,7 +37,7 @@
     const float* row_scale; const float* bias; int64_t bias_stride; const float* mask_h; int relu;
     const uint8_t* mask_b; uint8_t* relu_bits;
     const int32_t* tiles; int n_tiles; int n_col_tiles; int nt_store;
-    unsigned long long* dbg;
+    const int32_t* tile_live;
     int dephase;
     float* zero_out;
     const int4* f2; const float* zside; int64_t ldz; const float* zrow;
@@ -181,7 +181,10 @@
     constexpr int A_PER = (BM * BK / 4) / 256;
     constexpr int B_PPW = (NP * 2 * (BN / 64)) / 4;
     constexpr int OFF_MAX = OFF_BIAS + 2 * BN * 4;
-    __shared__ __attribute__((aligned(16))) char smem[OFF_MAX + 16];
+    constexpr bool LIVE = GATHER && NP == 3;
+    constexpr int LIVE_CAP = LIVE ? 1024 : 0, OFF_LIVE = OFF_MAX + 16;
+    static_assert(!LIVE || SPLIT == 1, "one flag per tile of `tiles`");
+    __shared__ __attribute__((aligned(16))) char smem[OFF_LIVE + (LIVE ? (LIVE_CAP + 4) * 4 : 0)];
     const int tid = threadIdx.x, lane = tid & 63, wave = __builtin_amdgcn_readfirstlane(tid >> 6);
     const int nchunks = g.K / BK;
     const int G = gridDim.x, b = blockIdx.x;
@@ -201,11 +204,73 @@
         if constexpr (NP == 3) return 1.f;
         else return gs_bound_scale(g.b_bound, set);
     };
-    const int total = ntb * nchunks;
+    int nt = ntb; bool listed = false;
+    const int* live_idx = reinterpret_cast<const int*>(smem + OFF_LIVE);
+    if constexpr (LIVE) {
+        if (g.tile_live && g.keep_signed && !g.relu_bits && !g.zero_out && ntb > 0 && ntb <= LIVE_CAP) {
+            int* lw = reinterpret_cast<int*>(smem + OFF_LIVE);
+            if (wave == 0) {
+                int n = 0;
+                for (int t0 = 0; t0 < ntb; t0 += 64) {
+                    const int ti = t0 + lane;
+                    const bool lv = ti < ntb && g.tile_live[logical(b + ti * G)] != 0;
+                    const unsigned long long m = __ballot(lv);
+                    if (lv) lw[n + __popcll(m & ((1ull << lane) - 1ull))] = ti;
+                    n += __popcll(m);
+                }
+                if (lane == 0) lw[LIVE_CAP] = n;
+            }
+            __syncthreads();
+            nt = __builtin_amdgcn_readfirstlane(live_idx[LIVE_CAP]); listed = true;
+        }
+    }
+    auto ord = [&](int i) -> int {
+        if constexpr (LIVE) { if (listed) return __builtin_amdgcn_readfirstlane(live_idx[i]); }
+        return i;
+    };
+    auto dead_chunks = [&](int n) {
+        if constexpr (LIVE) {
+            if (n <= 0) return;
+            gm_f32x16 d[MI][2];
+#pragma unroll
+            for (int i = 0; i < MI; ++i)
+#pragma unroll
+                for (int j = 0; j < 2; ++j)
+#pragma unroll
+                    for (int e = 0; e < 16; ++e) d[i][j][e] = 0.f;
+            gm_bf16x8 za, zb;
+            {
+                typedef unsigned u4 __attribute__((ext_vector_type(4)));
+                u4 ua, ub;
+                asm volatile("v_mov_b32 %0, 0\n\tv_mov_b32 %1, 0\n\tv_mov_b32 %2, 0\n\tv_mov_b32 %3, 0" : "=v"(ua.x), "=v"(ua.y), "=v"(ua.z), "=v"(ua.w));
+                asm volatile("v_mov_b32 %0, 0\n\tv_mov_b32 %1, 0\n\tv_mov_b32 %2, 0\n\tv_mov_b32 %3, 0" : "=v"(ub.x), "=v"(ub.y), "=v"(ub.z), "=v"(ub.w));
+                za = __builtin_bit_cast(gm_bf16x8, ua); zb = __builtin_bit_cast(gm_bf16x8, ub);
+            }
+            asm volatile("s_nop 7" ::: "memory");
+#define GS_M(D) "v_mfma_f32_32x32x16_bf16 " D ", %[a], %[b], " D "\n\t"
+            for (; n > 0; --n) {
+                if constexpr (MI == 2) {
+#define GS_P GS_M("%[d0]") GS_M("%[d1]") GS_M("%[d2]") GS_M("%[d3]")
+                    asm volatile("s_nop 1\n\t" GS_P GS_P GS_P GS_P GS_P GS_P : [d0] "+v"(d[0][0]), [d1] "+v"(d[0][1]), [d2] "+v"(d[MI - 1][0]), [d3] "+v"(d[MI - 1][1]) : [a] "v"(za), [b] "v"(zb));
+#undef GS_P
+                } else {
+#define GS_P GS_M("%[d0]") GS_M("%[d1]")
+                    asm volatile("s_nop 1\n\t" GS_P GS_P GS_P GS_P GS_P GS_P : [d0] "+v"(d[0][0]), [d1] "+v"(d[0][1]) : [a] "v"(za), [b] "v"(zb));
+#undef GS_P
+                }
+            }
+#undef GS_M
+            asm volatile("s_nop 15\n\ts_nop 15" ::: "memory");
+        }
+    };
+    const int total = nt * nchunks;
     const unsigned lds_base = (unsigned)(uintptr_t)((__attribute__((address_space(3))) char*)smem);
     float* scales = reinterpret_cast<float*>(smem + OFF_SC);
     float* biasl = reinterpret_cast<float*>(smem + OFF_BIAS);
-    if (total == 0) return;
+    if (total == 0) {
+        if (listed && wave < 8) dead_chunks(ntb * nchunks);
+        return;
+    }
     if (NP == 2 && tid < 2) reinterpret_cast<unsigned*>(smem + OFF_MAX)[tid] = 0u;
     if (wave >= 12) {
         __builtin_amdgcn_s_setprio(2);
@@ -219,10 +284,10 @@
         }
         const int64_t b_chunk_bytes = (int64_t)BK * g.N * 2;
         int ib_c = 0, ib_ti = 0;
-        uint64_t ib_base = (uint64_t)(uintptr_t)(g.Bt + (int64_t)tile_of(b).set * g.bt_stride);
+        uint64_t ib_base = (uint64_t)(uintptr_t)(g.Bt + (int64_t)tile_of(b + ord(0) * G).set * g.bt_stride);
         int ib_st = 0;
         auto issue_b = [&](int gc) {
-            if (ib_c == nchunks) { ib_c = 0; ++ib_ti; ib_base = (uint64_t)(uintptr_t)(g.Bt + (int64_t)tile_of(b + ib_ti * G).set * g.bt_stride); }
+            if (ib_c == nchunks) { ib_c = 0; ++ib_ti; ib_base = (uint64_t)(uintptr_t)(g.Bt + (int64_t)tile_of(b + ord(ib_ti) * G).set * g.bt_stride); }
             const uint64_t base = ib_base + (uint64_t)(ib_c * b_chunk_bytes);
             ++ib_c;
             const unsigned blo = __builtin_amdgcn_readfirstlane((unsigned)base), bhi = __builtin_amdgcn_readfirstlane((unsigned)(base >> 32));
@@ -270,8 +335,8 @@
         float rc_sc = 1.f, rc_b = 0.f;
         float as_next = 1.f, as_cur = 1.f, inv_next = 1.f, inv_cur = 1.f;
         auto fq_prefetch = [&](int ti) {
-            if (ti >= ntb) return;
-            const GsTile t = tile_of(b + ti * G);
+            if (ti >= nt) return;
+            const GsTile t = tile_of(b + ord(ti) * G);
 #pragma unroll
             for (int p = 0; p < A_PER; ++p) {
                 const int4* q = g.f2 + t.row0 + min(rr[p], t.nrows - 1);
@@ -279,7 +344,7 @@
             }
         };
         auto la_tile = [&](int ti, bool consts) {
-            const GsTile t = tile_of(b + ti * G);
+            const GsTile t = tile_of(b + ord(ti) * G);
             if constexpr (NP == 2) { as_next = a_scale_of(t.set); inv_next = (1.f / as_next) * (1.f / b_scale_of(t.set)); }
             if constexpr (GATHER) {
                 if constexpr (A_PER == 2) asm volatile("" : "+v"(fq[0]), "+v"(fq[A_PER - 1]) :: "memory");
@@ -331,7 +396,7 @@
             if (sa_c == nchunks) {
                 sa_c = 0; ++sa_ti;
                 as_cur = as_next; inv_cur = inv_next;
-                if constexpr (NP == 2) { if (!fast_consts) as_cur = a_scale_of(tile_of(b + sa_ti * G).set); }
+                if constexpr (NP == 2) { if (!fast_consts) as_cur = a_scale_of(tile_of(b + ord(sa_ti) * G).set); }
                 if constexpr (GATHER) {
 #pragma unroll
                     for (int p = 0; p < A_PER; ++p) { w_cur[p][0] = w_next[p][0]; w_cur[p][1] = w_next[p][1]; }
@@ -367,7 +432,7 @@
             }
         };
         auto stage_tile_consts = [&](int ti) {
-            const GsTile t = tile_of(b + ti * G);
+            const GsTile t = tile_of(b + ord(ti) * G);
             const int set = t.set, row0 = t.row0, nrows = t.nrows;
             float sc = 1.f;
             if (g.row_scale) sc = g.row_scale[row0 + min(ft & (BM - 1), nrows - 1)];
@@ -446,7 +511,9 @@
             for (int o = 32; o >= 1; o >>= 1) vmax = fmaxf(vmax, __shfl_xor(vmax, o));
             if (lane == 0) vmax_note(__float_as_uint(vmax));
         };
-        for (int ti = 0; ti < ntb; ++ti) {
+        int walked = 0;
+        for (int ti = 0; ti < nt; ++ti) {
+            if constexpr (LIVE) { if (listed) { const int o = ord(ti); dead_chunks((o - walked) * nchunks); walked = o + 1; } }
             gm_f32x16 acc[MI][2];
 #pragma unroll
             for (int i = 0; i < MI; ++i)
@@ -491,7 +558,7 @@
                 }
                 GS_BARRIER();
             }
-            const GsTile tl = tile_of(b + ti * G);
+            const GsTile tl = tile_of(b + ord(ti) * G);
             const int row0 = tl.row0, nrows = tl.nrows;
             const float* sc_t = scales + (ti & 1) * GS_BM;
             const int t4 = li & 3, q4 = li >> 2;
@@ -541,6 +608,7 @@
                 }
             }
         }
+        if constexpr (LIVE) { if (listed) dead_chunks((ntb - walked) * nchunks); }
         if constexpr (NP == 2) { if (g.amax_out && vmax_set >= 0) vmax_flush_last(); }
     }
 }
diff --git a/g-meta_amd/csrc/gm_internal.h b/g-meta_amd/csrc/gm_internal.h
--- a/g-meta_amd/csrc/gm_internal.h
+++ b/g-meta_amd/csrc/gm_internal.h
@@ -157,6 +157,7 @@
     void* d_fwd_tab[2] = {nullptr, nullptr};
     void* d_fwd_tab_feat = nullptr;
     float* d_obs[2] = {nullptr, nullptr};
+    int32_t* d_tile_live[2] = {nullptr, nullptr};
     struct obs_list { int32_t* rows = nullptr; int32_t* len = nullptr; int32_t cap = 0, win = 0, take = 0; int32_t* sched = nullptr; int32_t sched_len = 0; mutable int64_t n = -1; };
     obs_list obs[3];
     mutable int64_t fwd_cnt[2][3] = {{-1, -1, -1}, {-1, -1, -1}};
@@ -191,6 +192,7 @@
     int fuse_diff;
     int agg_mid_win;
     int agg_obs_list;
+    int dead_tiles;
     int agg_mid_list;
     int query_streams;
     int head_threads;
@@ -464,6 +466,8 @@
     const int32_t* tiles;
     int n_tiles;
     int64_t rows;
+    const int32_t* tile_live;
+    int grid_test;
     int* launched;
 };
 #define GM_GEMM_ID_GLDS4 1
diff --git a/g-meta_amd/csrc/model.hip b/g-meta_amd/csrc/model.hip
--- a/g-meta_amd/csrc/model.hip
+++ b/g-meta_amd/csrc/model.hip
@@ -594,8 +594,8 @@
 enum PassKind { PASS_PLAIN = 0, PASS_FWD_ONLY = 1, PASS_DIFF = 2 };
 enum RowSet { ROWS_ALL, ROWS_SRC, ROWS_E1, ROWS_CENTRE };
 enum DqFill { DQ_MEMSET, DQ_ZEROED, DQ_CENTRE };
-struct LayerPlan { bool split, fuse; RowSet formed, stored; bool relu_bits; const gm_batch::obs_list* list; };
-struct PassPlan { PassKind kind; LayerPlan layer[GM_MAX_GCN]; DqFill dq; bool t_centre, dq_e1; const gm_batch::obs_list* t_list; };
+struct LayerPlan { bool split, fuse; RowSet formed, stored; bool relu_bits; const gm_batch::obs_list* list; bool dead_tiles; };
+struct PassPlan { PassKind kind; LayerPlan layer[GM_MAX_GCN]; DqFill dq; bool t_centre, dq_e1; const gm_batch::obs_list* t_list; bool t_dead_tiles; };
 
 struct GcnCtx {
     const gm_batch* b; gm_layout L;
@@ -778,11 +778,11 @@
     return GM_OK;
 }
 
-struct RowView { const float* keep; const float* sign; const void* tab; int obs; int64_t n; };
+struct RowView { const float* keep; const float* sign; const void* tab; int obs; int64_t n; const int32_t* live; };
 static RowView row_view(const gm_batch* b, RowSet rs, bool gather) {
-    if (rs == ROWS_E1) return {b->d_norm_e1, b->d_obs[1], gather ? b->d_fwd_tab_feat : b->d_fwd_tab[1], 1, b->n_e1};
-    if (rs == ROWS_CENTRE) return {b->d_norm_c, b->d_obs[0], b->d_fwd_tab[0], 0, b->n_c};
-    return {rs == ROWS_SRC ? b->d_norm_src : nullptr, nullptr, gather ? b->d_fuse2_feat : b->d_fuse2, -1, rs == ROWS_SRC ? b->n_src : b->rows};
+    if (rs == ROWS_E1) return {b->d_norm_e1, b->d_obs[1], gather ? b->d_fwd_tab_feat : b->d_fwd_tab[1], 1, b->n_e1, b->d_tile_live[1]};
+    if (rs == ROWS_CENTRE) return {b->d_norm_c, b->d_obs[0], b->d_fwd_tab[0], 0, b->n_c, b->d_tile_live[0]};
+    return {rs == ROWS_SRC ? b->d_norm_src : nullptr, nullptr, gather ? b->d_fuse2_feat : b->d_fuse2, -1, rs == ROWS_SRC ? b->n_src : b->rows, nullptr};
 }
 static int64_t rows_kept(const gm_batch* b, RowSet rs, hipStream_t st) { return rs != ROWS_E1 ? row_view(b, rs, false).n : gm_prof_enabled() ? gm_batch_e1_rows(b, st) : std::min<int64_t>(b->n_e1, b->rows); }
 
@@ -873,6 +873,14 @@
         for (int l = 0; l < Lg; ++l)
             if (p.layer[l].fuse && p.layer[l].formed != ROWS_ALL) p.layer[l].list = taken(p.layer[l].formed == ROWS_CENTRE ? 0 : 1);
         if (p.dq_e1) p.t_list = taken(2);
+    }
+    if (gm_knob().dead_tiles) {
+        for (int l = 0; l < Lg; ++l) {
+            const LayerPlan& lp = p.layer[l];
+            p.layer[l].dead_tiles = kind == PASS_FWD_ONLY && lp.fuse && !lp.relu_bits && c.np != 2 && (lp.stored == ROWS_CENTRE || lp.stored == ROWS_E1) &&
+                                    row_view(b, lp.stored, false).live != nullptr;
+        }
+        p.t_dead_tiles = p.t_centre && c.np != 2 && b->d_tile_live[0] != nullptr;
     }
     *plan = p; return plan_check(c, p);
 }
@@ -943,6 +951,7 @@
             g.row_scale = b->d_norm; g.bias = params + L.b_off[l]; g.bias_stride = pstride; g.relu = 1; g.tiles = b->d_tiles; g.n_tiles = b->n_tiles; g.rows = b->rows;
             g.relu_bits = relu_bits;
             if (lp.stored != ROWS_ALL) { g.row_scale_keep = row_view(b, lp.stored, false).keep; g.n_keep = rows_kept(b, lp.stored, st); }
+            if (lp.dead_tiles) g.tile_live = row_view(b, lp.stored, false).live;
             if (lp.split) {
                 GM_TRY(weight_planes(c, params, pstride, l, 0, st, g));
                 GM_REQUIRE(!(l == L.n_gcn - 1 && plan.dq == DQ_CENTRE) || g.np == 3, GM_EINVAL, "forward: dQ is left to its centre rows, which needs the three-piece kernels");
@@ -1025,6 +1034,7 @@
                     g.B = params + L.w_off[l]; g.b_stride = pstride; g.transB = 1;
                     if (dq_centre && l == Lg - 1) { g.fuse2 = b->d_dq_tab; g.zside = dQ; g.ldz = fo; }
                     if (t_centre && l == Lg - 1) { g.row_scale_keep = row_view(b, ROWS_CENTRE, false).keep; g.n_keep = rows_kept(b, ROWS_CENTRE, st); }
+                    if (t_centre && l == Lg - 1 && plan.t_dead_tiles) g.tile_live = row_view(b, ROWS_CENTRE, false).live;
                 } else if (use_wt) {
                     if (!(c.wt_of[l] == params && c.wt_stride[l] == pstride)) {
                         const int nt = pstride ? b->sets : 1;
diff --git a/include/gmeta_hip.h b/include/gmeta_hip.h
--- a/include/gmeta_hip.h
+++ b/include/gmeta_hip.h
@@ -170,6 +170,10 @@
                         int64_t ldzf, const float* W, int64_t w_stride, int32_t N, float* out, int64_t ldc, const float* s, const float* s_keep,
                         const float* bias, int64_t bias_stride, int32_t relu, uint8_t* relu_bits, float* zero_out, uint32_t* amax_out, int32_t mode,
                         int32_t* launched, void* stream);
+int gm_dense_fused_gemm_rows(const gm_batch_t* b, int32_t rowset, int32_t keep, int32_t live_on, int32_t grid, int32_t table, const float* x, int64_t ldx, int32_t K,
+                             const float* zside, int64_t ldz, const float* zfull, int64_t ldzf, const float* W, int64_t w_stride, int32_t N, float* out, int64_t ldc,
+                             const float* bias, int64_t bias_stride, int32_t relu, uint8_t* relu_bits, float* zero_out, uint32_t* amax_out, int32_t mode,
+                             int32_t* launched, void* stream);
 int gm_dense_aggregate(const gm_batch_t* b, int32_t transposed, int32_t x_src, const float* x, int64_t ldx, int32_t width, int32_t scale_src,
                        const float* s_in, const float* s_out, int32_t keep_signed, const float* bias, int64_t bias_stride, int32_t relu,
                        uint8_t* relu_bits, const float* mask_h, const uint8_t* mask_b, int32_t hubs, const int32_t* rowlist, int64_t n_list,
```

After: 2020 (median of 6 runs). 4.6% higher.
